# mp3guy/ElasticFusion

Measured on AMD Instinct MI355X. Metric: frames/s per GPU, 640x480 3-level ICP+fuse, higher is better.
Workload: dtype f32

## Files before the change

elasticfusion_amd/api.py:

```python
from __future__ import annotations

import ctypes as C
import os
import re

import numpy as np

_HERE = os.path.dirname(os.path.abspath(__file__))
LIB_PATH = os.environ.get("EF_HIP_LIB") or os.path.join(_HERE, "libefusion_hip.so")
_lib = None

c_f, c_i, c_u32, P = C.c_float, C.c_int, C.c_uint32, C.c_void_p


class EFError(RuntimeError):
    pass


class ef_config(C.Structure):
    _fields_ = [("width", c_i), ("height", c_i), ("fx", c_f), ("fy", c_f), ("cx", c_f), ("cy", c_f),
                ("time_delta", c_i), ("confidence", c_f), ("depth_cut", c_f), ("icp_weight", c_f),
                ("fast_odom", c_i), ("so3", c_i), ("frame_to_frame_rgb", c_i), ("pyramid", c_i), ("rgb_only", c_i),
                ("close_loops", c_i), ("max_surfels", c_u32), ("device", c_i), ("stream", P)]


class ef_intr(C.Structure):
    _fields_ = [("fx", c_f), ("fy", c_f), ("cx", c_f), ("cy", c_f)]


class ef_cam(C.Structure):
    _fields_ = [("cols", c_i), ("rows", c_i), ("fx", c_f), ("fy", c_f), ("cx", c_f), ("cy", c_f)]


class ef_gn_state(C.Structure):
    _fields_ = [("Rcurr", c_f * 9), ("tcurr", c_f * 3), ("resultRt", C.c_double * 16), ("krkinv", c_f * 9), ("kt", c_f * 3),
                ("lastRGBErrorLevel", c_f), ("rgb_broken", c_i)]


class ef_gn_update_args(C.Structure):
    _fields_ = [("sums", c_f * 58), ("prev", ef_gn_state), ("Rprev", c_f * 9), ("tprev", c_f * 3), ("count", c_i), ("sigma", c_i),
                ("icp", c_i), ("rgb", c_i), ("rgb_only", c_i), ("icp_weight", c_f), ("knext", ef_intr), ("level_changes", c_i),
                ("split_tail", c_i)]


class ef_model_maps_op(C.Structure):
    _fields_ = [("cols", c_i), ("rows", c_i), ("pred_vertex", P), ("pred_normal", P), ("fill_vertex", P), ("fill_normal", P), ("pred_image", P),
                ("fill_image", P), ("R", c_f * 9), ("t", c_f * 3), ("max_depth_rgb", c_f), ("camera_frame", c_i), ("force_fill_image", c_i),
                ("tally", c_i), ("dense_count", C.c_uint), ("dense_samples", c_i), ("vmap", P * 3), ("nmap", P * 3), ("depth0", P), ("last0", P),
                ("joint", c_i), ("raw", P), ("rgb3", P), ("depth_cut", c_f), ("filtered", P), ("metric", P), ("metric_filtered", P), ("next0", P)]


class ef_track_end_out(C.Structure):
    _fields_ = [("q", C.c_double * 4), ("t", C.c_double * 3), ("logged", C.c_double * 16), ("T_cw", c_f * 16), ("pose_f", c_f * 16),
                ("R_wc_f", c_f * 9), ("t_wc_f", c_f * 3), ("weighting", c_f)]


class ef_timing(C.Structure):
    _fields_ = [("name", C.c_char_p), ("ms", c_f)]


class ef_kernel_time(C.Structure):
    _fields_ = [("name", C.c_char_p), ("avg_us", c_f), ("launches", c_i), ("bytes_per_launch", C.c_double), ("bytes_per_launch_survey", C.c_double)]


class ef_tracker_plan(C.Structure):
    _fields_ = [("script", c_i), ("n_small", c_i), ("n_iter", c_i), ("levels", C.c_ulonglong), ("res_bytes", C.c_uint), ("res_budget", C.c_uint)]


class ef_render_params(C.Structure):
    _fields_ = [("width", c_i), ("height", c_i), ("fx", c_f), ("fy", c_f), ("cx", c_f), ("cy", c_f), ("T_wc", C.c_double * 16),
                ("max_depth", c_f), ("threshold", c_f), ("draw_unstable", c_i), ("color_type", c_i), ("draw_window", c_i),
                ("time", c_i), ("time_delta", c_i)]


class ef_register_params(C.Structure):
    _fields_ = [("max_dist", c_f), ("min_conf", c_f), ("min_normal_cos", c_f), ("max_iterations", c_i), ("min_pairs", c_i),
                ("stop_translation", C.c_double), ("stop_rotation", C.c_double)]


class ef_register_sums(C.Structure):
    _fields_ = [("A", C.c_double * 36), ("b", C.c_double * 6), ("e", C.c_double), ("pairs", c_u32), ("points", c_u32)]


class ef_register_result(C.Structure):
    _fields_ = [("status", c_i), ("iterations", c_i), ("pairs", c_u32), ("rms_first", C.c_double), ("rms_last", C.c_double),
                ("A", C.c_double * 36)]


class ef_map_selection(C.Structure):
    _fields_ = [("tests", c_u32), ("T_bw", C.c_double * 16), ("box_min", c_f * 3), ("box_max", c_f * 3), ("conf_min", c_f), ("conf_max", c_f),
                ("init_time_min", c_i), ("init_time_max", c_i), ("last_time_min", c_i), ("last_time_max", c_i), ("radius_min", c_f),
                ("radius_max", c_f), ("id_min", c_u32), ("id_max", c_u32), ("label_class", c_i), ("label_min_prob", c_f)]


class ef_insert_params(C.Structure):
    _fields_ = [("gate", c_i), ("min_separation", c_f), ("min_conf", c_f), ("min_normal_cos", c_f), ("init_time", c_i), ("last_time", c_i)]


class ef_insert_result(C.Structure):
    _fields_ = [("inserted", c_u32), ("duplicates", c_u32), ("skipped", c_u32), ("count_after", c_u32)]


class ef_fuse_params(C.Structure):
    _fields_ = [("min_separation", c_f), ("min_conf", c_f), ("min_normal_cos", c_f), ("append", c_i), ("init_time", c_i), ("last_time", c_i)]


class ef_fuse_result(C.Structure):
    _fields_ = [("fused", c_u32), ("absorbed", c_u32), ("weightless", c_u32), ("novel", c_u32), ("skipped", c_u32), ("inserted", c_u32),
                ("count_after", c_u32)]


class ef_thin_params(C.Structure):
    _fields_ = [("cell", c_f), ("keep", c_i)]


class ef_thin_result(C.Structure):
    _fields_ = [("participants", c_u32), ("cells", c_u32), ("removed", c_u32), ("count_after", c_u32)]


class ef_carve_params(C.Structure):
    _fields_ = [("width", c_i), ("height", c_i), ("fx", c_f), ("fy", c_f), ("cx", c_f), ("cy", c_f), ("min_depth", c_f), ("max_depth", c_f),
                ("margin", c_f), ("margin_quad", c_f), ("window", c_i), ("min_views", c_i), ("protect", c_i)]


class ef_carve_views(C.Structure):
    _fields_ = [("n", c_i), ("T_wc16", C.c_void_p), ("depth", C.c_void_p)]


class ef_carve_result(C.Structure):
    _fields_ = [("participants", c_u32), ("observed", c_u32), ("free_space", c_u32), ("protected_", c_u32), ("removed", c_u32),
                ("count_after", c_u32)]


class ef_outlier_params(C.Structure):
    _fields_ = [("mode", c_i), ("radius", c_f), ("cell", c_f), ("min_conf", c_f), ("min_neighbors", c_i), ("k", c_i), ("std_ratio", c_f),
                ("max_mean_dist", c_f), ("flag_sparse", c_i)]


class ef_outlier_result(C.Structure):
    _fields_ = [("sum", C.c_double), ("sum_sq", C.c_double), ("participants", c_u32), ("measured", c_u32), ("sparse", c_u32),
                ("outliers", c_u32), ("count_after", c_u32), ("threshold", c_f)]


class ef_component_params(C.Structure):
    _fields_ = [("radius", c_f), ("cell", c_f), ("min_conf", c_f), ("min_size", c_u32), ("max_size", c_u32)]


class ef_component_result(C.Structure):
    _fields_ = [("nodes", c_u32), ("components", c_u32), ("largest", c_u32), ("rejected_rows", c_u32), ("rejected_components", c_u32),
                ("count_after", c_u32), ("status", c_u32)]


CARVE_MAX_VIEWS = 32
COMPONENT_NONE = 0xFFFFFFFF
COMPONENTS_REJECTED, COMPONENTS_ACCEPTED = 0, 1
OUTLIER_RADIUS, OUTLIER_STATISTICAL = 0, 1
OUTLIER_SUM_LANES = 4096
THIN_KEEP_MAX_CONF, THIN_KEEP_NEWEST, THIN_KEEP_FIRST = 0, 1, 2
THIN_ROWS_REMOVED, THIN_ROWS_REPRESENTATIVES = 0, 1
INSERT_KEEP = -1
FUSE_SKIPPED, FUSE_NOVEL, FUSE_WEIGHTLESS, FUSE_ABSORBED, FUSE_FUSED, FUSE_INSERTED = 0, 1, 2, 3, 4, 5
ROW_NONE = 0xFFFFFFFF

SEL_BOX, SEL_CONF, SEL_INIT_TIME, SEL_LAST_TIME, SEL_RADIUS, SEL_ID, SEL_LABEL, SEL_INVERT = 0x01, 0x02, 0x04, 0x08, 0x10, 0x20, 0x40, 0x100

REG_CONVERGED, REG_MAX_ITERATIONS, REG_TOO_FEW_PAIRS, REG_DEGENERATE = 0, 1, 2, 3
REG_STATUS = {REG_CONVERGED: "CONVERGED", REG_MAX_ITERATIONS: "MAX_ITERATIONS", REG_TOO_FEW_PAIRS: "TOO_FEW_PAIRS", REG_DEGENERATE: "DEGENERATE"}


def _sums_dict(s: ef_register_sums) -> dict:
    return {"A": np.array(s.A, np.float64).reshape(6, 6), "b": np.array(s.b, np.float64), "e": float(s.e), "pairs": int(s.pairs),
            "points": int(s.points)}


def _sums_struct(sums) -> ef_register_sums:
    if isinstance(sums, ef_register_sums):
        return sums
    s = ef_register_sums()
    s.A[:] = np.ascontiguousarray(sums["A"], np.float64).reshape(36).tolist()
    s.b[:] = np.ascontiguousarray(sums["b"], np.float64).reshape(6).tolist()
    s.e = float(sums.get("e", 0.0))
    s.pairs = int(sums.get("pairs", 0))
    s.points = int(sums.get("points", 0))
    return s


def _pose16(T):
    if T is None:
        return None, None
    a = np.ascontiguousarray(T, np.float64).reshape(16)
    return a, _ptr(a)


def register_update(sums, T=None):
    s = _sums_struct(sums)
    keep, pT = _pose16(T)
    out = np.zeros(16, np.float64)
    xi = np.zeros(6, np.float64)
    rc = lib().ef_register_update(C.byref(s), pT, _ptr(out), _ptr(xi))
    if rc not in (0, REG_DEGENERATE):
        _chk(rc)
    return out.reshape(4, 4), xi, rc == REG_DEGENERATE
# ... 1189 lines not shown
        out = np.zeros((H, W, ch) if ch > 1 else (H, W), dt)
        _chk(lib().ef_get_image(self.h, which, _ptr(out), out.nbytes), self.h)
        return out

    def trackerBuffer(self, name: str, level: int = 0, tracker: int = 0) -> np.ndarray:
        which, dt, planes = self.TRACKER[name]
        w, h = self.cfg.width >> level, self.cfg.height >> level
        out = np.zeros((h * planes, w), dt)
        _chk(lib().ef_get_tracker_buffer_of(self.h, tracker, which, level, _ptr(out), out.nbytes), self.h)
        return out

    def enableTiming(self, on=True):
        _chk(lib().ef_enable_timing(self.h, int(on)), self.h)

    def timings(self) -> dict:
        arr = (ef_timing * 32)()
        n = c_i(0)
        _chk(lib().ef_get_timings(self.h, arr, 32, C.byref(n)), self.h)
        return {arr[i].name.decode(): arr[i].ms for i in range(n.value)}


class ops:
    @staticmethod
    def _f32(a):
        return np.ascontiguousarray(a, np.float32)

    @staticmethod
    def _image_op(name, src, dtype, scale, *scalars):
        h, w = src.shape[:2]
        shape = (h // scale, w // scale)
        s, d = DevBuf.from_array(src), DevBuf(shape[0] * shape[1] * np.dtype(dtype).itemsize)
        _chk(getattr(lib(), "ef_op_" + name)(s.p, w, h, *scalars, d.p, None))
        return d.to_array(dtype, shape)

    @staticmethod
    def pyr_down(src):
        return ops._image_op("pyr_down", src, np.uint16, 2)

    @staticmethod
    def create_vmap(depth, fx, fy, cx, cy, cutoff, init=None):
        h, w = depth.shape
        d = DevBuf.from_array(depth)
        v = DevBuf.from_array(np.zeros((3 * h, w), np.float32) if init is None else init)
        k = ef_intr(fx, fy, cx, cy)
        _chk(lib().ef_op_create_vmap(C.byref(k), d.p, w, h, cutoff, v.p, None))
        return v.to_array(np.float32, (3 * h, w))

    @staticmethod
    def create_nmap(vmap, init=None):
        h3, w = vmap.shape
        v = DevBuf.from_array(vmap)
        n = DevBuf.from_array(np.zeros((h3, w), np.float32) if init is None else init)
        _chk(lib().ef_op_create_nmap(v.p, w, h3 // 3, n.p, None))
        return n.to_array(np.float32, (h3, w))

    @staticmethod
    def transform_maps(vmap, nmap, R, t):
        h3, w = vmap.shape
        v, n = DevBuf.from_array(vmap), DevBuf.from_array(nmap)
        R9, t3 = ops._f32(R).reshape(9), ops._f32(t).reshape(3)
        _chk(lib().ef_op_transform_maps(v.p, n.p, w, h3 // 3, _ptr(R9), _ptr(t3), v.p, n.p, None))
        return v.to_array(np.float32, (h3, w)), n.to_array(np.float32, (h3, w))

    @staticmethod
    def copy_maps(vtex, ntex):
        h, w, _ = vtex.shape
        v4, n4 = DevBuf.from_array(ops._f32(vtex)), DevBuf.from_array(ops._f32(ntex))
        tmp, vm, nm = DevBuf(h * w * 16), DevBuf(h * w * 12), DevBuf(h * w * 12)
        _chk(lib().ef_op_copy_maps(v4.p, n4.p, w, h, tmp.p, vm.p, nm.p, None))
        return tmp.to_array(np.float32, (h, w, 4)), vm.to_array(np.float32, (3 * h, w)), nm.to_array(np.float32, (3 * h, w))

    @staticmethod
    def resize_map(src, normalize, init=None):
        h3, w = src.shape
        s = DevBuf.from_array(src)
        o = DevBuf.from_array(np.zeros((h3 // 2, w // 2), np.float32) if init is None else init)
        fn = lib().ef_op_resize_nmap if normalize else lib().ef_op_resize_vmap
        _chk(fn(s.p, w, h3 // 3, o.p, None))
        return o.to_array(np.float32, (h3 // 2, w // 2))

    @staticmethod
    def pyr_down_gauss_f(src):
        return ops._image_op("pyr_down_gauss_f", src, np.float32, 2)

    @staticmethod
    def pyr_down_uchar_gauss(src):
        return ops._image_op("pyr_down_uchar_gauss", src, np.uint8, 2)

    @staticmethod
    def vertices_to_depth(vmaps_tmp, cutoff):
        return ops._image_op("vertices_to_depth", ops._f32(vmaps_tmp), np.float32, 1, cutoff)

    @staticmethod
    def bgr_to_intensity(rgba):
        return ops._image_op("image_bgr_to_intensity", rgba, np.uint8, 1)

    @staticmethod
    def derivative_images(img):
        h, w = img.shape
        s, dx, dy = DevBuf.from_array(img), DevBuf(h * w * 2), DevBuf(h * w * 2)
        _chk(lib().ef_op_compute_derivative_images(s.p, w, h, dx.p, dy.p, None))
        return dx.to_array(np.int16, (h, w)), dy.to_array(np.int16, (h, w))

    @staticmethod
    def project_to_point_cloud(depth, fx, fy, cx, cy, level=0):
        h, w = depth.shape
        s, d = DevBuf.from_array(depth), DevBuf(h * w * 12)
        k = ef_intr(fx, fy, cx, cy)
        _chk(lib().ef_op_project_to_point_cloud(s.p, w, h, C.byref(k), level, d.p, None))
        return d.to_array(np.float32, (h, w, 3))

    @staticmethod
    def icp_step(Rcurr, tcurr, vmap_curr, nmap_curr, Rprev_inv, tprev, intr, vmap_g_prev, nmap_g_prev, distThres, angleThres):
        h3, w = vmap_curr.shape
        bufs = [DevBuf.from_array(a) for a in (vmap_curr, nmap_curr, vmap_g_prev, nmap_g_prev)]
        A, b, res = np.zeros((6, 6), np.float32), np.zeros(6, np.float32), np.zeros(2, np.float32)
        k = ef_intr(*intr)
        _chk(lib().ef_op_icp_step(_ptr(ops._f32(Rcurr).reshape(9)), _ptr(ops._f32(tcurr)), bufs[0].p, bufs[1].p,
                                  _ptr(ops._f32(Rprev_inv).reshape(9)), _ptr(ops._f32(tprev)), C.byref(k), bufs[2].p, bufs[3].p,
                                  distThres, angleThres, w, h3 // 3, _ptr(A), _ptr(b), _ptr(res), None))
        return A, b, res

    @staticmethod
    def rgb_residual(minScale, dIdx, dIdy, lastDepth, nextDepth, lastImage, nextImage, maxDepthDelta, kt, krkinv):
        h, w = nextImage.shape
        bufs = [DevBuf.from_array(a) for a in (dIdx, dIdy, lastDepth, nextDepth, lastImage, nextImage)]
        corres = DevBuf(h * w * 16)
        sigma, count = c_i(0), c_i(0)
        _chk(lib().ef_op_compute_rgb_residual(minScale, bufs[0].p, bufs[1].p, bufs[2].p, bufs[3].p, bufs[4].p, bufs[5].p, corres.p,
                                              maxDepthDelta, _ptr(ops._f32(kt)), _ptr(ops._f32(krkinv).reshape(9)), w, h,
                                              C.byref(sigma), C.byref(count), None))
        return corres.to_array(DATATERM, (h, w)), sigma.value, count.value

    @staticmethod
    def rgb_step(corres, sigma, cloud, fx, fy, dIdx, dIdy, sobelScale):
        h, w = corres.shape
        bufs = [DevBuf.from_array(a) for a in (corres, ops._f32(cloud), dIdx, dIdy)]
        A, b = np.zeros((6, 6), np.float32), np.zeros(6, np.float32)
        _chk(lib().ef_op_rgb_step(bufs[0].p, sigma, bufs[1].p, fx, fy, bufs[2].p, bufs[3].p, sobelScale, w, h,
                                  _ptr(A), _ptr(b), None))
        return A, b

    @staticmethod
    def so3_step(lastImage, nextImage, imageBasis, kinv, krlr):
        h, w = nextImage.shape
        li, ni = DevBuf.from_array(lastImage), DevBuf.from_array(nextImage)
        A, b, res = np.zeros((3, 3), np.float32), np.zeros(3, np.float32), np.zeros(2, np.float32)
        _chk(lib().ef_op_so3_step(li.p, ni.p, _ptr(ops._f32(imageBasis).reshape(9)), _ptr(ops._f32(kinv).reshape(9)),
                                  _ptr(ops._f32(krlr).reshape(9)), w, h, _ptr(A), _ptr(b), _ptr(res), None))
        return A, b, res

    @staticmethod
    def model_maps(pred_vertex, pred_normal, fill_vertex, fill_normal, R, t, maxDepthRGB=6.0, pred_image=None, fill_image=None, camera_frame=False,
                   force_fill_image=False, tally=False, dense_count=0, dense_samples=1, joint=False, raw=None, rgb=None, depth_cut=3.0, init=None):
        h, w, _ = pred_vertex.shape
        init = init or {}
        keep = [DevBuf.from_array(ops._f32(a)) for a in (pred_vertex, pred_normal, fill_vertex, fill_normal)]
        a = ef_model_maps_op()
        a.cols, a.rows = w, h
        a.pred_vertex, a.pred_normal, a.fill_vertex, a.fill_normal = (b.p for b in keep)
        if pred_image is not None:
            imgs = [DevBuf.from_array(np.ascontiguousarray(i, np.uint8)) for i in (pred_image, fill_image)]
            keep += imgs
            a.pred_image, a.fill_image = imgs[0].p, imgs[1].p
        a.R[:] = [float(v) for v in ops._f32(R).reshape(9)]
        a.t[:] = [float(v) for v in ops._f32(t).reshape(3)]
        a.max_depth_rgb = float(maxDepthRGB)
        a.camera_frame, a.force_fill_image, a.tally = int(camera_frame), int(force_fill_image), int(tally)
        a.dense_count, a.dense_samples = int(dense_count), int(dense_samples)
        spec = {}
        for l in range(3):
            spec[f"vmap{l}"] = spec[f"nmap{l}"] = (np.float32, (3 * (h >> l), w >> l))
        spec["depth0"], spec["last0"] = (np.float32, (h, w)), (np.uint8, (h, w))
        if joint:
            spec.update(filtered=(np.uint16, (h, w)), metric=(np.float32, (h, w)), metric_filtered=(np.float32, (h, w)), next0=(np.uint8, (h, w)))
        out = {}
        for name, (dt, shp) in spec.items():
            start = np.zeros(shp, dt) if name not in init else np.ascontiguousarray(init[name], dt)
            assert start.shape == shp, (name, start.shape, shp)
            out[name] = DevBuf.from_array(start)
        for l in range(3):
            a.vmap[l], a.nmap[l] = out[f"vmap{l}"].p, out[f"nmap{l}"].p
        a.depth0, a.last0 = out["depth0"].p, out["last0"].p
        if joint:
            fr = [DevBuf.from_array(np.ascontiguousarray(raw, np.uint16)), DevBuf.from_array(np.ascontiguousarray(rgb, np.uint8))]
            assert raw.shape == (h, w) and rgb.shape == (h, w, 3)
            keep += fr
            a.joint, a.raw, a.rgb3, a.depth_cut = 1, fr[0].p, fr[1].p, float(depth_cut)
            a.filtered, a.metric, a.metric_filtered, a.next0 = (out[n].p for n in ("filtered", "metric", "metric_filtered", "next0"))
        left = C.c_uint(0)
        _chk(lib().ef_op_model_maps(C.byref(a), C.byref(left), None))
        res = {name: out[name].to_array(*spec[name]) for name in spec}
        res["dense_count"] = int(left.value)
        return res

    @staticmethod
    def sobel_mask(nextImage, nextDepth):
        h, w = nextImage[0].shape
        img = [DevBuf.from_array(np.ascontiguousarray(a, np.uint8)) for a in nextImage]
        dep = [DevBuf.from_array(ops._f32(a)) for a in nextDepth]
        for l in range(3):
            assert nextImage[l].shape == nextDepth[l].shape == (h >> l, w >> l), (l, nextImage[l].shape, nextDepth[l].shape)
        outs = [[DevBuf((h >> l) * (w >> l) * sz, fill=0xA5) for l in range(3)] for sz in (2, 2, 1, 4)]
        arr = lambda bufs: (P * 3)(*[b.p for b in bufs])
        _chk(lib().ef_op_sobel_mask(arr(img), arr(dep), w, h, arr(outs[0]), arr(outs[1]), arr(outs[2]), arr(outs[3]), None))
        return tuple([b.to_array(dt, (h >> l, w >> l)) for l, b in enumerate(bufs)] for bufs, dt in zip(outs, (np.int16, np.int16, np.uint8, np.uint32)))

    @staticmethod
    def clean_deform(cam, T_wc, time, idx, vc, ct, nr, confThreshold, timeDelta, maxDepth, surfels, newUnstable, graph, depth, isFern=0):
        s = ops._f32(surfels).reshape(-1, 12)
        nu = ops._f32(newUnstable).reshape(-1, 12)
        g = ops._f32(graph).reshape(-1, 16)
        bufs = [DevBuf.from_array(a) for a in (idx, ops._f32(vc), ops._f32(ct), ops._f32(nr), g, ops._f32(depth))]
        sb, nb = DevBuf.from_array(s), DevBuf.from_array(nu if len(nu) else np.zeros((1, 12), np.float32))
        out = DevBuf((len(s) + len(nu) + 1) * 48)
        n = c_u32(0)
        _chk(lib().ef_op_clean_deform(C.byref(cam), _ptr(ops._T(T_wc)), time, bufs[0].p, bufs[1].p, bufs[2].p, bufs[3].p,
                                      confThreshold, timeDelta, maxDepth, sb.p, len(s), nb.p, len(nu),
                                      bufs[4].p, len(g), bufs[5].p, int(isFern), out.p, C.byref(n), None))
        return out.to_array(np.float32, (n.value, 12))

    LINALG = dict(ldlt6=0, ldlt3f=1, polar3=2, rodrigues=3, se3_inverse=4, se3_log_norm=5, scalar=6, ldlt6_wave=7, ldlt6_every_lane=8,
                  mat_to_quat=9, se3_mul=10, se3_castf=11, se3_inverse_f=12, m4_affine_inverse=13, ldlt_pivots=14, lu_inverse6=15)

    @staticmethod
    def linalg(which, vec, n_out):
        v = np.ascontiguousarray(np.asarray(vec, np.float64).reshape(-1))
        out = np.zeros(n_out, np.float64)
        _chk(lib().ef_op_linalg(ops.LINALG[which], _ptr(v), v.size, _ptr(out), n_out))
        return out

    GN_STATE = ("Rcurr", "tcurr", "resultRt", "krkinv", "kt", "lastRGBErrorLevel", "rgb_broken")

    @staticmethod
    def gn_update(sums, prev, Rprev, tprev, count, sigma, icp, rgb, rgbOnly, icpWeight, knext, level_changes, split_tail, lastA, lastb, stats):
        a = ef_gn_update_args()
        a.sums[:] = [float(v) for v in ops._f32(sums).reshape(58)]
        for name in ("Rcurr", "tcurr", "krkinv", "kt"):
            getattr(a.prev, name)[:] = [float(v) for v in ops._f32(prev[name]).reshape(-1)]
        a.prev.resultRt[:] = [float(v) for v in np.asarray(prev["resultRt"], np.float64).reshape(16)]
        a.prev.lastRGBErrorLevel, a.prev.rgb_broken = float(np.float32(prev["lastRGBErrorLevel"])), int(prev["rgb_broken"])
        a.Rprev[:] = [float(v) for v in ops._f32(Rprev).reshape(9)]
        a.tprev[:] = [float(v) for v in ops._f32(tprev).reshape(3)]
        a.count, a.sigma, a.icp, a.rgb, a.rgb_only = int(count), int(sigma), int(icp), int(rgb), int(rgbOnly)
        a.icp_weight, a.knext, a.level_changes, a.split_tail = float(icpWeight), ef_intr(*[float(v) for v in knext]), int(level_changes), int(split_tail)
        nxt = ef_gn_state()
        A = np.ascontiguousarray(np.asarray(lastA, np.float64).reshape(36)).copy()
        b = np.ascontiguousarray(np.asarray(lastb, np.float64).reshape(6)).copy()
        st = ops._f32(stats).reshape(4).copy()
        _chk(lib().ef_op_gn_update(C.byref(a), C.byref(nxt), _ptr(A), _ptr(b), _ptr(st)))
        out = {n: np.array(getattr(nxt, n)) for n in ("Rcurr", "tcurr", "resultRt", "krkinv", "kt")}
        out["lastRGBErrorLevel"], out["rgb_broken"] = np.float32(nxt.lastRGBErrorLevel), int(nxt.rgb_broken)
        return out, A, b, st

    @staticmethod
    def track_end_tail(Rcurr, tcurr, Rprev, tprev, q_prev, t_prev, rgb, weightMultiplier):
        o = ef_track_end_out()
        qp = np.ascontiguousarray(np.asarray(q_prev, np.float64).reshape(4))
        tp = np.ascontiguousarray(np.asarray(t_prev, np.float64).reshape(3))
        _chk(lib().ef_op_track_end_tail(_ptr(ops._f32(Rcurr).reshape(9)), _ptr(ops._f32(tcurr).reshape(3)), _ptr(ops._f32(Rprev).reshape(9)),
                                        _ptr(ops._f32(tprev).reshape(3)), _ptr(qp), _ptr(tp), int(rgb), weightMultiplier, C.byref(o)))
        out = {n: np.array(getattr(o, n)) for n in ("q", "t", "logged", "T_cw", "pose_f", "R_wc_f", "t_wc_f")}
        out["weighting"] = np.float32(o.weighting)
        return out

    @staticmethod
    def filter_depth(raw, maxD):
        return ops._image_op("filter_depth", raw, np.uint16, 1, maxD)

    @staticmethod
    def metricise_depth(d_in, maxD):
        return ops._image_op("metricise_depth", d_in, np.float32, 1, maxD)

    @staticmethod
    def seed_map(cam, rgb, dm, dmf, time, maxDepth):
        Pn = cam.cols * cam.rows
        bufs = [DevBuf.from_array(a) for a in (rgb, dm, dmf)]
        out = DevBuf(Pn * 48)
        n = c_u32(0)
        _chk(lib().ef_op_seed_map(C.byref(cam), bufs[0].p, bufs[1].p, bufs[2].p, time, maxDepth, out.p, C.byref(n), None))
        return out.to_array(np.float32, (n.value, 12))

    @staticmethod
    def _T(T):
        return np.ascontiguousarray(T, np.float64).reshape(16)

    @staticmethod
    def predict_indices(cam, T_wc, time, surfels, maxDepth, timeDelta):
        s = ops._f32(surfels).reshape(-1, 12)
        Pn = cam.cols * cam.rows
        sb = DevBuf.from_array(s)
        idx, vc, ct, nr = DevBuf(Pn * 4), DevBuf(Pn * 16), DevBuf(Pn * 16), DevBuf(Pn * 16)
        _chk(lib().ef_op_predict_indices(C.byref(cam), _ptr(ops._T(T_wc)), time, sb.p, len(s), maxDepth, timeDelta,
                                         idx.p, vc.p, ct.p, nr.p, None))
        shp = (cam.rows, cam.cols)
        return (idx.to_array(np.uint32, shp), vc.to_array(np.float32, shp + (4,)), ct.to_array(np.float32, shp + (4,)),
                nr.to_array(np.float32, shp + (4,)))

    @staticmethod
    def combined_predict(cam, T_wc, surfels, maxDepth, confThreshold, time, maxTime, timeDelta):
        s = ops._f32(surfels).reshape(-1, 12)
        Pn = cam.cols * cam.rows
        sb = DevBuf.from_array(s)
        img, vt, nm, tm = DevBuf(Pn * 4), DevBuf(Pn * 16), DevBuf(Pn * 16), DevBuf(Pn * 2)
        _chk(lib().ef_op_combined_predict(C.byref(cam), _ptr(ops._T(T_wc)), sb.p, len(s), maxDepth, confThreshold,
                                          time, maxTime, timeDelta, img.p, vt.p, nm.p, tm.p, None))
        shp = (cam.rows, cam.cols)
        return (img.to_array(np.uint8, shp + (4,)), vt.to_array(np.float32, shp + (4,)), nm.to_array(np.float32, shp + (4,)),
                tm.to_array(np.uint16, shp))

    @staticmethod
    def synthesize_depth(cam, T_wc, surfels, maxDepth, confThreshold, time, maxTime, timeDelta):
        s = ops._f32(surfels).reshape(-1, 12)
        Pn = cam.cols * cam.rows
        sb, d = DevBuf.from_array(s), DevBuf(Pn * 4)
        _chk(lib().ef_op_synthesize_depth(C.byref(cam), _ptr(ops._T(T_wc)), sb.p, len(s), maxDepth, confThreshold,
                                          time, maxTime, timeDelta, d.p, None))
        return d.to_array(np.float32, (cam.rows, cam.cols))

    @staticmethod
    def fill_in(cam, image, vertex, normal, depthFiltered, rgb, passthrough=0, passthroughImage=0):
        bufs = [DevBuf.from_array(a) for a in (image, ops._f32(vertex), ops._f32(normal), depthFiltered, rgb)]
        Pn = cam.cols * cam.rows
        fi, fv, fn = DevBuf(Pn * 4), DevBuf(Pn * 16), DevBuf(Pn * 16)
        _chk(lib().ef_op_fill_in(C.byref(cam), bufs[0].p, bufs[1].p, bufs[2].p, bufs[3].p, bufs[4].p, passthrough, passthroughImage,
                                 fi.p, fv.p, fn.p, None))
        shp = (cam.rows, cam.cols)
        return fi.to_array(np.uint8, shp + (4,)), fv.to_array(np.float32, shp + (4,)), fn.to_array(np.float32, shp + (4,))

    @staticmethod
    def dense_enough(cam, image):
        b = DevBuf.from_array(image)
        d = c_i(0)
        _chk(lib().ef_op_dense_enough(C.byref(cam), b.p, C.byref(d), None))
        return bool(d.value)

    @staticmethod
    def fuse(cam, T_wc, time, rgb, dm, dmf, idx, vc, ct, nr, maxDepth, weighting, surfels):
        s = ops._f32(surfels).reshape(-1, 12)
        bufs = [DevBuf.from_array(a) for a in (rgb, dm, dmf, idx, ops._f32(vc), ops._f32(ct), ops._f32(nr))]
        sb = DevBuf.from_array(s)
        nu = DevBuf((cam.cols // 2) * (cam.rows // 2) * 48)
# ... 17 lines not shown
```

elasticfusion_amd/csrc/ef_context.hip:

```cpp
#include <hip/hip_runtime.h>
#include <math.h>
#include <cmath>
#include <stdio.h>
#include <string.h>
#include <limits>
#include <string>
#include <thread>
#include <vector>

#include "../../include/ef_hip.h"
#include "ef_linalg_dev.hpp"
#include "ef_solve_dev.hpp"
#include "ef_map.hpp"
#include "ef_deform_solver.hpp"
#include "ef_track.hpp"

template void std::vector<int64_t>::push_back(const int64_t&);

namespace {

thread_local std::string g_create_error;

struct StageTimer {
  const char* name;
  hipEvent_t a, b;
  bool used;
};

struct DevBuf {
  uint8_t* p = nullptr;
  size_t bytes = 0;
  int reserve(ef_ctx* c, size_t need, const char* what, bool* grew = nullptr);
  void release() {
    if (p) (void)hipFree(p);
    p = nullptr;
    bytes = 0;
  }
  template <class T>
  T* as() const { return (T*)p; }
};
struct Carver {
  uint8_t* at;
  explicit Carver(const DevBuf& b) : at(b.p) {}
  template <class T>
  T* take(size_t count, size_t align = alignof(T)) {
    at = (uint8_t*)(((uintptr_t)at + align - 1) & ~(uintptr_t)(align - 1));
    T* r = (T*)at;
    at += count * sizeof(T);
    return r;
  }
  static size_t chunks(size_t rows) { return (size_t)efm::select_chunks((unsigned)rows) + 1; }
  static size_t scan_bytes(size_t rows) { return (2 * chunks(rows) + 4) * sizeof(uint32_t); }
  uint32_t* scan_words(size_t rows, efm::SelectScratch* sc, size_t align = alignof(uint32_t)) {
    const size_t k = chunks(rows);
    sc->chunk_count = take<uint32_t>(k, align);
    sc->chunk_offset = take<uint32_t>(k);
    return take<uint32_t>(4);
  }
};

struct FrameImages {
  uint8_t* rgb = nullptr;
  uint16_t *depth_raw = nullptr, *depth_filtered = nullptr;
  float *depth_metric = nullptr, *depth_metric_filtered = nullptr;
};
struct RingSlot {
  uint8_t *h_rgb = nullptr, *d_rgb = nullptr;
  uint16_t *h_depth = nullptr, *d_depth = nullptr;
  hipEvent_t ev_h2d = nullptr;
};
struct KernelSampler {
  std::vector<hipEvent_t> start, stop;
  eft::KernelProbe probe{nullptr, nullptr, 0, 0};
  int create(ef_ctx* c, int capacity);
  int average_us(ef_ctx* c, float* us) const;
  void release() {
    for (auto e : start) (void)hipEventDestroy(e);
    for (auto e : stop) (void)hipEventDestroy(e);
    *this = KernelSampler{};
  }
};

}

struct ef_ctx {
  ef_config cfg;
  hipStream_t stream = nullptr;
  bool own_stream = false;
  std::string err;
  efm::Cam cam;
  eft::Intr intr;
  const float maxDepthProcessed = 20.0f;
  FrameImages img, img_alt;
  hipStream_t in_stream = nullptr;
  hipEvent_t ev_input_done = nullptr, ev_track_done = nullptr;
  hipEvent_t ev_frame_done[2] = {nullptr, nullptr};
  int frame_parity = 0;
  int overlap_mode = 1;
  bool overlap = false;
  bool events_live = false;
  static constexpr int RING = 3;
  RingSlot ring[RING];
  hipStream_t copy_stream = nullptr;
  unsigned host_seq = 0;
  unsigned mark_value = 0;
  unsigned* h_consumed = nullptr;
  unsigned* d_consumed = nullptr;
  unsigned* h_abort = nullptr;
  unsigned* d_abort = nullptr;
  eft::Pyramid pyr{};
  eft::TrackState* st = nullptr;
  efm::IndexMaps im{};
  efm::PredictMaps pm{};
  efm::FillMaps fm{};
  unsigned long long* zbuf = nullptr;
  unsigned long long* zbuf_assoc = nullptr;
  unsigned long long* zbuf_clean = nullptr;
  float* im_T16 = nullptr;
  bool im_pending = false;
  int im_map = 0;
  efm::SurfelSoA maps[2]{};
  int cur = 0;
  efm::SurfelSoA shadow{};
  bool reference_download = false;
  uint32_t capacity = 0;
  uint32_t* winner = nullptr;
  efm::Candidates cand{};
  efm::CompactScratch cs{};
  int* overflow = nullptr;
  double* traj = nullptr;
  int traj_cap = 0;
  std::vector<int64_t> stamps;
  int tick = 1;
  std::vector<void*> allocs;
  bool tally_by_consumer = false;
  bool tally_pending = false;
  bool timing = false;
  std::vector<StageTimer> timers;
  float* graph_dev = nullptr;
  int graph_nodes = 0, graph_is_fern = 0;
  float* synth_depth = nullptr;
  float* rays = nullptr;
  int icp_count_thresh = 35000;
  float icp_err_thresh = 5e-05f, cov_thresh = 1e-05f;
  int deforms = 0;
  const float* bil_table = nullptr;
  eft::Pyramid pyr2{};
  eft::TrackState* st2 = nullptr;
  efm::PredictMaps old{};
  float* cons_dev = nullptr;
  float* h_cons = nullptr;
  eft::TrackState* h_states = nullptr;
  ef_loop_solver solver = nullptr;
  void* solver_user = nullptr;
  bool builtin_solver = false;
  int64_t last_deform_time = 0;
  float* nodes_dev = nullptr;
  std::vector<float> h_nodes;
  ef_local_loop loop{};
  std::vector<double> loop_constraints;
  std::vector<float> loop_graph;
  ef_closure* closure = nullptr;
  ef_global_loop gloop{};
  std::string fern_tracker_error;
  int fern_w = 0, fern_h = 0;
  uchar4* view_img_dev = nullptr;
  float4* view_vert_dev = nullptr;
  float4* view_norm_dev = nullptr;
  uint8_t* h_view = nullptr;
  eft::Pyramid pyr3{};
  eft::TrackState* st3 = nullptr;
  eft::Intr intr3{};
  float4* fern_maps_dev = nullptr;
  float* h_nodes_pinned = nullptr;
  int* fern_table_dev = nullptr;
  int fern_num = 0, fern_table_version = -1;
  uint8_t* fern_codes_dev = nullptr;
  uint8_t* h_codes = nullptr;
  uint8_t* h_codes_end = nullptr;
  uint8_t* h_view_end = nullptr;
  hipEvent_t ev_end_record = nullptr;
  bool end_pending = false, end_lost = false;
  int end_tick = 0;
  int n_nodes_host = 0;
  double h_pose[16] = {1, 0, 0, 0, 0, 1, 0, 0, 0, 0, 1, 0, 0, 0, 0, 1};
  bool reloc = false, lost = false, last_frame_recovery = false, tracking_ok = true;
  int tracking_count = 0;
  eft::TrackState h_reloc{};
  bool use_graph = false;
  bool track_only = false;
  bool no_resident = false;
  bool fused_step = false;
  int persistent = 1;
  struct TrackGraph { hipGraphExec_t exec = nullptr; const void* key = nullptr; eft::TrackParams tp{}; eft::TrackTail tail{}; eft::TrackerPlan plan{}; };
  TrackGraph tgraph[2];
  int ktime_every = 0;
  KernelSampler sample_step, sample_splat, sample_all;
  hipStream_t debug_stream = nullptr;
  DevBuf stage;
  struct RenderState { DevBuf zbuf; } render;
  struct LabelState {
    bool ids_on = false, ids_bad = false;
    unsigned* ids_state = nullptr;
    int C = 0, cur = 0;
    float* tab[2] = {};
    uint32_t* ids[2] = {};
    size_t rows = 0, bound = 0;
    size_t known = 0, known_frames = 0, ev_frames = 0;
    unsigned* count_h = nullptr;
    hipEvent_t ev = nullptr;
    bool ev_pending = false;
    DevBuf index;
  } labels;
  uint64_t map_gen = 1;
  struct QueryState {
    uint64_t gen = 0;
    float cell = EF_QUERY_DEFAULT_CELL, built_cell = 0.f;
    int lanes = 0;
    DevBuf sorted, rows;
    DevBuf cells;
    uint32_t nb = 0, n = 0;
  } query;
  struct RegisterState {
    DevBuf slabs;
    double* sums_h = nullptr;
  } reg;
  struct SelectState {
    DevBuf scratch;
    size_t rows = 0;
    uint64_t gen = 0;
    uint32_t count = 0;
  } sel;
  struct InsertState {
    DevBuf scratch;
    size_t rows = 0;
  } ins;
  struct ThinState {
    DevBuf scratch;
    size_t rows = 0;
  } thin;
  struct CarveState {
    DevBuf scratch;
    size_t rows = 0;
  } carve;
  struct OutlierState {
    DevBuf scratch;
    size_t rows = 0;
  } outlier;
  struct ComponentState {
    DevBuf scratch;
    size_t rows = 0;
  } components;
  struct FuseState {
    DevBuf scratch;
  } fuse;
};

namespace {

#define EF_HIP(ctx, expr)                                                                       \
  do {                                                                                          \
    hipError_t _e = (expr);                                                                     \
    if (_e != hipSuccess) {                                                                     \
      (ctx)->err = std::string(#expr) + ": " + hipGetErrorString(_e);                           \
      return EF_EHIP;                                                                           \
    }                                                                                           \
  } while (0)
// ... 788 lines not shown
```

elasticfusion_amd/csrc/ef_device.hpp:

```cpp
#pragma once
#include <hip/hip_runtime.h>
#include <stdint.h>
#include "ef_build.hpp"

#ifdef EF_NO_FMA
#define EF_FMA(a, b, c) ((a) * (b) + (c))
#else
#define EF_FMA(a, b, c) fmaf((a), (b), (c))
#endif

namespace ef {

struct f3 { float x, y, z; };

__device__ __forceinline__ float qnan() { return __int_as_float(0x7fffffff); }
__device__ __forceinline__ f3 operator-(f3 a, f3 b) { return {a.x - b.x, a.y - b.y, a.z - b.z}; }
__device__ __forceinline__ f3 operator+(f3 a, f3 b) { return {a.x + b.x, a.y + b.y, a.z + b.z}; }
__device__ __forceinline__ float dot(f3 a, f3 b) { return EF_FMA(a.z, b.z, EF_FMA(a.y, b.y, a.x * b.x)); }
__device__ __forceinline__ f3 cross(f3 a, f3 b) {
  return {EF_FMA(a.y, b.z, -(a.z * b.y)), EF_FMA(a.z, b.x, -(a.x * b.z)), EF_FMA(a.x, b.y, -(a.y * b.x))};
}
__device__ __forceinline__ float norm(f3 a) { return sqrtf(dot(a, a)); }
__device__ __forceinline__ f3 normalized(f3 a) {
  const float rn = 1.0f / sqrtf(dot(a, a));
  return {a.x * rn, a.y * rn, a.z * rn};
}
__device__ __forceinline__ uint8_t intensity_of(float c0, float c1, float c2) {
  const int value = (int)(c0 * 0.114f + c1 * 0.299f + c2 * 0.587f);
  return (uint8_t)value;
}
struct m33 { f3 r[3]; };
__device__ __forceinline__ f3 mul(const m33& m, f3 a) { return {dot(m.r[0], a), dot(m.r[1], a), dot(m.r[2], a)}; }
__device__ __forceinline__ m33 m33_load(const float* p) {
  return m33{{{p[0], p[1], p[2]}, {p[3], p[4], p[5]}, {p[6], p[7], p[8]}}};
}
struct rt34 { m33 R; f3 t; };
__device__ __forceinline__ rt34 rt34_load16(const float* M) {
  return rt34{{{{M[0], M[1], M[2]}, {M[4], M[5], M[6]}, {M[8], M[9], M[10]}}}, {M[3], M[7], M[11]}};
}
__device__ __forceinline__ f3 xform(const rt34& T, f3 p) { return mul(T.R, p) + T.t; }

__device__ __forceinline__ int f2i_rn(float x) {
  float r = (x != x) ? 0.0f : rintf(x);
  r = fminf(fmaxf(r, -2147483648.0f), 2147483520.0f);
  return (int)r;
}

__host__ __device__ inline float ef_next_up(float a) { unsigned u; __builtin_memcpy(&u, &a, 4); ++u; __builtin_memcpy(&a, &u, 4); return a; }
__host__ __device__ inline float ef_next_down(float a) { unsigned u; __builtin_memcpy(&u, &a, 4); --u; __builtin_memcpy(&a, &u, 4); return a; }
__host__ __device__ inline float sq_le_max(float T) {
  if (!(T >= 0.0f)) return -1.0f;
  if (T > 3.4028234664e38f) return T;
  float a = T * T;
  if (a > 3.4028234664e38f) a = 3.4028234664e38f;
  for (int i = 0; i < 8 && a > 0.0f && !(__builtin_sqrtf(a) <= T); ++i) a = ef_next_down(a);
  for (int i = 0; i < 8 && a < 3.4028234664e38f && __builtin_sqrtf(ef_next_up(a)) <= T; ++i) a = ef_next_up(a);
  return a;
}
__host__ __device__ inline float sq_lt_max(float T) {
  if (!(T > 0.0f)) return -1.0f;
  float a = T > 3.4028234664e38f ? 3.4028234664e38f : T * T;
  if (a > 3.4028234664e38f) a = 3.4028234664e38f;
  for (int i = 0; i < 8 && a > 0.0f && !(__builtin_sqrtf(a) < T); ++i) a = ef_next_down(a);
  for (int i = 0; i < 8 && a < 3.4028234664e38f && __builtin_sqrtf(ef_next_up(a)) < T; ++i) a = ef_next_up(a);
  return a;
}

__device__ __forceinline__ float ef_expf(float x) {
  if (x < -87.0f) return 0.0f;
  const float n = rintf(x * 1.44269504088896341f);
  float r = fmaf(n, -0.693359375f, x);
  r = fmaf(n, 2.12194440e-4f, r);
  float p = 1.9875691500e-4f;
  p = fmaf(p, r, 1.3981999507e-3f);
  p = fmaf(p, r, 8.3334519073e-3f);
  p = fmaf(p, r, 4.1665795894e-2f);
  p = fmaf(p, r, 1.6666665459e-1f);
  p = fmaf(p, r, 5.0000001201e-1f);
  const float e = fmaf(p, r * r, r) + 1.0f;
  return ldexpf(e, (int)n);
}

__device__ __forceinline__ int clampi(int v, int lo, int hi) { return v < lo ? lo : (v > hi ? hi : v); }

struct DataTerm {
  short zero_x, zero_y;
  short one_x, one_y;
  float diff;
  unsigned char valid;
  unsigned char pad[3];
};
static_assert(sizeof(DataTerm) == 16, "DataTerm must be 16 bytes");

template <int K, int BLOCK>
__device__ __forceinline__ void block_reduce_store(const float (&acc)[K], float* lds, float* out) {
  static_assert(K <= 32 && BLOCK % 64 == 0, "shape");
  constexpr int STR = BLOCK + 1;
  constexpr int SEG = BLOCK / 32;
  const int t = threadIdx.x;
#pragma unroll
  for (int k = 0; k < K; ++k) lds[k * STR + t] = acc[k];
  __syncthreads();
  const int v = t & 31, g = t >> 5;
  float s = 0.f;
  if (v < K) {
    const float* row = lds + v * STR + g * 32;
#pragma unroll
    for (int i = 0; i < 32; ++i) s += row[i];
  }
  __syncthreads();
  lds[g * 32 + v] = s;
  __syncthreads();
  if (t < K) {
    float r = 0.f;
#pragma unroll
    for (int gg = 0; gg < SEG; ++gg) r += lds[gg * 32 + t];
    out[t] = r;
  }
}
template <int K, int BLOCK>
constexpr int block_reduce_lds_floats() { return K * (BLOCK + 1); }

template <int BLOCK>
__device__ __forceinline__ void block_reduce_atomic_int2(int a, int b, int* lds, int* out2) {
  const int t = threadIdx.x;
  for (int off = 32; off > 0; off >>= 1) {
    a += __shfl_down(a, off, 64);
    b += __shfl_down(b, off, 64);
  }
  if ((t & 63) == 0) { lds[(t >> 6) * 2] = a; lds[(t >> 6) * 2 + 1] = b; }
  __syncthreads();
  if (t == 0) {
    int sa = 0, sb = 0;
    for (int w = 0; w < BLOCK / 64; ++w) { sa += lds[w * 2]; sb += lds[w * 2 + 1]; }
    if (sa) atomicAdd(out2, sa);
    if (sb) atomicAdd(out2 + 1, sb);
  }
}

}
```

elasticfusion_amd/csrc/ef_host_frame.inc:

```
namespace {
int do_predict(ef_ctx* c, bool count_dense = true) {
  efm::combined_predict(c->cam, c->st->T_cw, c->maps[c->cur], &c->st->map_counts[c->cur], c->maxDepthProcessed, c->cfg.confidence,
                        c->last_frame_recovery ? 0 : c->tick, c->tick, c->cfg.time_delta, c->zbuf, c->pm, c->fm, c->img.depth_filtered, c->img.rgb,
                        c->cfg.frame_to_frame_rgb != 0, (count_dense && !c->tally_by_consumer) ? &c->st->dense_count : nullptr, c->stream, nullptr, 0u,
                        (count_dense && c->mark_value) ? c->d_consumed : nullptr, c->mark_value, c->rays);
  if (count_dense) c->mark_value = 0;
  if (count_dense && c->tally_by_consumer) c->tally_pending = true;
  if (c->lost) efm::fill_in(c->cam, c->pm, c->img.depth_filtered, c->img.rgb, true, true, c->fm, c->stream);
  return EF_OK;
}
bool reloc_covariance_ok(const eft::TrackState& h) {
  double cov[36];
  efl::lu_inverse<double, 6>(h.lastA, cov);
  for (int i = 0; i < 6; ++i)
    if (cov[i * 6 + i] > 1e-04) return false;
  return true;
}
struct FramePlan {
  const ef_ctx* c; hipMemcpyKind kind; bool pose_given;
  bool overlap = c->overlap && !c->timing && c->in_stream != nullptr;
  hipStream_t sb = overlap ? c->in_stream : c->stream;
  bool want_events = c->overlap && c->in_stream != nullptr;
  int overlap_mode = (c->overlap_mode == 2 && c->persistent == 1 && !c->use_graph) ? 1 : c->overlap_mode;
  bool frame_done_event = want_events && c->overlap_mode == 2;
  bool track_this = c->tick > 1 && !pose_given;
  bool fold_copies = kind == hipMemcpyDeviceToDevice && track_this;
  bool joint_inputs = track_this && !overlap && !c->timing;
  bool sample = c->ktime_every > 0 && (c->tick % c->ktime_every) == 0;
  bool replay = c->use_graph && !sample && !c->timing;
#ifdef EF_KEEP_INDEX_RESOLVE
  bool keyed = false;
#else
  bool keyed = !c->timing && !c->reference_download && !c->cfg.close_loops;
#endif
  bool defer_merge = !c->timing;
};
int input_stage(ef_ctx* c, const FramePlan& f, const uint8_t* rgb_src, const uint16_t* depth_src, hipEvent_t images_ready, eft::FramePreprocess* fp) {
  const int W = c->cam.cols, H = c->cam.rows;
  hipStream_t sb = f.sb;
  if (f.overlap && !c->events_live) EF_HIP(c, hipStreamSynchronize(c->stream));
  std::swap(c->img, c->img_alt);
  c->frame_parity ^= 1;
  if (f.overlap) EF_HIP(c, hipStreamWaitEvent(sb, f.overlap_mode == 2 ? c->ev_frame_done[c->frame_parity] : c->ev_track_done, 0));
  if (images_ready) EF_HIP(c, hipStreamWaitEvent(sb, images_ready, 0));
  if (!f.fold_copies) {
    EF_HIP(c, hipMemcpyAsync(c->img.rgb, rgb_src, (size_t)W * H * 3, f.kind, sb));
    EF_HIP(c, hipMemcpyAsync(c->img.depth_raw, depth_src, (size_t)W * H * 2, f.kind, sb));
  }
  *fp = eft::FramePreprocess{f.fold_copies ? depth_src : c->img.depth_raw, c->cfg.depth_cut, c->bil_table, c->img.depth_filtered, c->img.depth_metric,
                             c->img.depth_metric_filtered, f.fold_copies ? rgb_src : c->img.rgb, f.fold_copies ? c->img.rgb : nullptr};
  timer_begin(c, "Preprocess");
  if (!f.joint_inputs && !efm::preprocess_depth(fp->raw, W, H, fp->maxD, fp->filtered, fp->metric, fp->metric_filtered, sb, 0u,
                                                f.track_this ? fp->rgb3 : nullptr, c->pyr.nextImage[0], fp->rgb_keep, fp->table)) {
    c->err = "bilateral weight table missing on this device";
    return EF_EHIP;
  }
  timer_end(c, "Preprocess");
  if (f.overlap && f.overlap_mode == 2) EF_HIP(c, hipStreamWaitEvent(sb, c->ev_track_done, 0));
  if (f.track_this && f.overlap)
    eft::build_pyramids_frame_side(c->pyr, c->img.depth_filtered, c->intr, c->maxDepthProcessed, sb);
  if (f.overlap) EF_HIP(c, hipEventRecord(c->ev_input_done, sb));
  return EF_OK;
}
int first_frame(ef_ctx* c, const FramePlan& f, int log_slot) {
  hipStream_t s = c->stream;
  if (f.overlap) EF_HIP(c, hipStreamWaitEvent(s, c->ev_input_done, 0));
  timer_begin(c, "feedbackBuffers");
  efm::seed_map(c->cam, c->img.rgb, c->img.depth_metric, c->img.depth_metric_filtered, c->tick, c->maxDepthProcessed, c->maps[c->cur],
                &c->st->map_counts[c->cur], c->cs, s);
  eft::init_first_rgb(c->pyr, c->img.rgb, s);
  if (log_slot >= 0) eft::log_pose(c->st, c->traj, log_slot, s);
  if (f.want_events) EF_HIP(c, hipEventRecord(c->ev_track_done, s));
  timer_end(c, "feedbackBuffers");
  return EF_OK;
}
int track_replayed(ef_ctx* c, const eft::TrackParams& tp, eft::TrackTail* tail) {
  hipStream_t s = c->stream;
  const void* key = c->pyr.nextImage[0];
  ef_ctx::TrackGraph* g = nullptr;
  for (auto& cand : c->tgraph)
    if (cand.exec && cand.key == key && !memcmp(&cand.tp, &tp, sizeof(tp))) g = &cand;
  if (!g) {
    g = (c->tgraph[0].exec && c->tgraph[0].key != key) ? &c->tgraph[1] : &c->tgraph[0];
    if (g->exec) { (void)hipGraphExecDestroy(g->exec); g->exec = nullptr; }
    eft::track_prepare(c->pyr, tp, s);
    eft::Pyramid pyr_copy = c->pyr;
    hipGraph_t graph = nullptr;
    EF_HIP(c, hipStreamBeginCapture(s, hipStreamCaptureModeThreadLocal));
    g->tail = eft::track(pyr_copy, c->st, c->intr, tp, s, nullptr);
    g->plan = pyr_copy.plan;
    hipError_t ce = hipStreamEndCapture(s, &graph);
    if (ce == hipSuccess) ce = hipGraphInstantiate(&g->exec, graph, nullptr, nullptr, 0);
    if (graph) (void)hipGraphDestroy(graph);
    if (ce != hipSuccess) {
      g->exec = nullptr;
      c->err = std::string("hipGraph capture of the tracker: ") + hipGetErrorString(ce);
      return EF_EHIP;
    }
    g->key = key;
    memcpy(&g->tp, &tp, sizeof(tp));
  }
  EF_HIP(c, hipGraphLaunch(g->exec, s));
  eft::track_swap(c->pyr, tp);
  c->pyr.plan = g->plan;
  *tail = g->tail;
  return EF_OK;
}
int track_frame(ef_ctx* c, const FramePlan& f, const eft::FramePreprocess& fp, float weightMultiplier, int log_slot) {
  hipStream_t s = c->stream;
  eft::TrackParams tp = track_params(c);
  tp.rgbOnly = c->cfg.rgb_only != 0; tp.pyramid = c->cfg.pyramid != 0; tp.fastOdom = c->cfg.fast_odom != 0; tp.so3 = c->cfg.so3 != 0;
  tp.icpWeight = c->cfg.icp_weight;
  const bool rgb = tp.rgbOnly || tp.icpWeight < 100;
  timer_begin(c, "odomInit");
  eft::init_icp_model(c->pyr, (const float*)c->pm.vertex, (const float*)c->pm.normal, (const float*)c->fm.vertex,
                      (const float*)c->fm.normal, c->st, 6.0f , s, (const uint8_t*)c->pm.image,
                      (const uint8_t*)c->fm.image, c->cfg.frame_to_frame_rgb != 0, f.joint_inputs ? &fp : nullptr, c->tally_pending);
  c->tally_pending = false;
  if (f.overlap) {
    eft::build_pyramids_model_side(c->pyr, s);
    EF_HIP(c, hipStreamWaitEvent(s, c->ev_input_done, 0));
  } else {
    eft::build_pyramids(c->pyr, c->img.depth_filtered, c->intr, c->maxDepthProcessed, s, rgb);
  }
  if (rgb && f.overlap) eft::init_rgb_sobel(c->pyr, s);
  timer_end(c, "odomInit");
  timer_begin(c, "odom");
  eft::TrackTail tail{};
  if (f.replay) {
    tp.persistent = 0;
    EF_TRY(track_replayed(c, tp, &tail));
  } else {
    tail = eft::track(c->pyr, c->st, c->intr, tp, s, f.sample ? &c->sample_step.probe : nullptr,
                      f.sample && c->sample_all.probe.start ? &c->sample_all.probe : nullptr);
  }
  eft::track_end(c->st, tail, rgb, weightMultiplier, log_slot >= 0 ? c->traj : nullptr, log_slot, s, eft::tracker_abort_word(c->pyr), c->d_abort);
  timer_end(c, "odom");
  return EF_OK;
}
int reloc_verdict(ef_ctx* c) {
  c->tracking_ok = true;
  if (!c->reloc) return EF_OK;
  EF_TRY(read_state(c, c->st, &c->h_reloc));
  c->tracking_ok = c->h_reloc.lastICPError < 1e-04;
  if (!c->lost) {
    if (!reloc_covariance_ok(c->h_reloc)) c->tracking_ok = false;
    if (!c->tracking_ok) {
      if (++c->tracking_count > 10) c->lost = true;
    } else {
      c->tracking_count = 0;
    }
  } else if (c->last_frame_recovery) {
    if (!reloc_covariance_ok(c->h_reloc)) c->tracking_ok = false;
    if (c->tracking_ok) {
      c->lost = false;
      c->tracking_count = 0;
    }
    c->last_frame_recovery = false;
  }
  return EF_OK;
}
int close_loops(ef_ctx* c, int log_slot) {
  int fern_graph = 0;
  if (c->closure) {
    timer_begin(c, "globalLoop");
    do_predict(c, false);
    c->last_frame_recovery = false;
    const int r = global_loop_closure(c, log_slot, &fern_graph);
    timer_end(c, "globalLoop");
    if (r != EF_OK) return r;
  }
  if (c->lost || fern_graph) {
    memset(&c->loop, 0, sizeof(c->loop));
    return EF_OK;
  }
  timer_begin(c, "localLoop");
  const int r = local_loop_closure(c, log_slot, c->closure != nullptr);
  timer_end(c, "localLoop");
  return r;
  return EF_OK;
}
void fuse_frame(ef_ctx* c, const FramePlan& f) {
  hipStream_t s = c->stream;
  const bool keyed = f.keyed, sample_splat = f.sample && c->sample_splat.probe.start;
  timer_begin(c, "indexMap");
  efm::IndexMaps im_assoc = c->im;
  im_assoc.color_time = nullptr;
  const efm::KeyedIndex key_assoc{c->zbuf_assoc, c->st->T_cw, c->maps[c->cur]}, key_clean{c->zbuf_clean, c->st->T_cw, c->maps[c->cur]};
  efm::predict_indices(c->cam, c->st->T_cw, c->tick, c->maps[c->cur], &c->st->map_counts[c->cur], c->maxDepthProcessed, c->cfg.time_delta,
                       keyed ? c->zbuf_assoc : c->zbuf, im_assoc, s, sample_splat ? &c->sample_splat.probe : nullptr, nullptr, nullptr, !keyed);
  timer_end(c, "indexMap");
  timer_begin(c, "Fuse::Data+Update");
  efm::fuse(c->cam, c->st->pose_f, c->tick, c->img.rgb, c->img.depth_metric, c->img.depth_metric_filtered, c->im, c->maxDepthProcessed,
            &c->st->weighting, c->maps[c->cur], &c->st->map_counts[c->cur], c->cand, c->winner, s, f.defer_merge,
            keyed ? &key_assoc : nullptr, keyed ? c->zbuf_clean : nullptr);
  if (c->reference_download && !f.defer_merge) efm::copy_map(c->maps[c->cur], &c->st->map_counts[c->cur], c->shadow, s);
  timer_end(c, "Fuse::Data+Update");
  timer_begin(c, "indexMap2");
  efm::predict_indices(c->cam, c->st->T_cw, c->tick, c->maps[c->cur], &c->st->map_counts[c->cur], c->maxDepthProcessed, c->cfg.time_delta,
                       keyed ? c->zbuf_clean : c->zbuf, c->im, s, nullptr, f.defer_merge ? &c->cand : nullptr, c->winner, !keyed);
  c->im_pending = keyed;
  c->im_map = c->cur;
  if (c->reference_download && f.defer_merge) efm::copy_map(c->maps[c->cur], &c->st->map_counts[c->cur], c->shadow, s);
  timer_end(c, "indexMap2");
  efm::Deformation def{c->graph_dev, c->graph_nodes, c->synth_depth, c->graph_is_fern, c->maxDepthProcessed};
  if (c->graph_nodes > 0 && !c->graph_is_fern)
    efm::synthesize_depth(c->cam, c->st->T_cw, c->maps[c->cur], &c->st->map_counts[c->cur], c->maxDepthProcessed, c->cfg.confidence, c->tick,
                          c->tick - c->cfg.time_delta, 65535, c->zbuf, c->synth_depth, s, c->rays);
  timer_begin(c, "Fuse::Copy");
  efm::clean(c->cam, c->st->T_cw, c->tick, c->im, c->cfg.confidence, c->cfg.time_delta, c->maps[c->cur], &c->st->map_counts[c->cur], c->cand,
             c->winner, c->maps[c->cur ^ 1], &c->st->map_counts[c->cur ^ 1], c->capacity, c->cs, c->overflow, s,
             c->graph_nodes > 0 ? &def : nullptr, keyed ? &key_clean : nullptr, keyed ? c->zbuf_assoc : nullptr, keyed ? c->im_T16 : nullptr);
  c->cur ^= 1;
  timer_end(c, "Fuse::Copy");
}
int end_of_frame(ef_ctx* c, const FramePlan& f) {
  timer_begin(c, "IndexMap::ACTIVE");
  do_predict(c);
  timer_end(c, "IndexMap::ACTIVE");
  if (c->closure) {
    timer_begin(c, "ferns");
    int r = flush_end_record(c);
    if (r == EF_OK) r = enqueue_end_record(c);
    timer_end(c, "ferns");
    if (r != EF_OK) return r;
  }
  if (f.frame_done_event) EF_HIP(c, hipEventRecord(c->ev_frame_done[c->frame_parity], c->stream));
  c->events_live = f.want_events;
  if (!c->lost) c->tick++;
  EF_HIP(c, hipGetLastError());
  return EF_OK;
}
int process_frame(ef_ctx* c, const uint8_t* rgb_src, const uint16_t* depth_src, hipMemcpyKind kind, int64_t timestamp,
                  float weightMultiplier, const double* in_T_wc, hipEvent_t images_ready = nullptr) {
  ++c->map_gen;
  if ((c->h_abort && (c->h_abort[0] | c->h_abort[1] | c->h_abort[2])) || c->pyr.sticky_abort || c->pyr2.sticky_abort || c->pyr3.sticky_abort) {
    c->err = "a persistent tracker launch of an earlier frame timed out waiting for another workgroup after its whole grid had reported in (a protocol "
             "failure, not a busy chip: that case runs on one workgroup, ef_get_tracker_fallbacks): the poses and the map since then are invalid; "
             "recreate the context (ef_set_persistent_tracker(ctx, 0) selects the launch-per-step script)";
    return EF_EHIP;
  }
  const FramePlan f{c, kind, in_T_wc != nullptr};
  eft::FramePreprocess fp;
  EF_TRY(input_stage(c, f, rgb_src, depth_src, images_ready, &fp));
  if ((int)c->stamps.size() >= c->traj_cap) EF_TRY(grow_trajectory(c));
  const int log_slot = (int)c->stamps.size();
  c->stamps.push_back(timestamp);
  if (c->tick == 1) {
    EF_TRY(first_frame(c, f, log_slot));
  } else {
    if (!in_T_wc) {
      EF_TRY(track_frame(c, f, fp, weightMultiplier, log_slot));
      EF_TRY(reloc_verdict(c));
    } else {
      c->tracking_ok = true;
      if (f.overlap) EF_HIP(c, hipStreamWaitEvent(c->stream, c->ev_input_done, 0));
      eft::pose_injected(c->st, in_T_wc, true, weightMultiplier, true, log_slot >= 0 ? c->traj : nullptr, log_slot, c->stream);
    }
    if (f.want_events) EF_HIP(c, hipEventRecord(c->ev_track_done, c->stream));
    if (c->cfg.close_loops) EF_TRY(close_loops(c, log_slot));
    if (!c->cfg.rgb_only && c->tracking_ok && !c->lost && !c->track_only) fuse_frame(c, f);
    c->graph_nodes = 0;
  }
  return end_of_frame(c, f);
}
}

extern "C" {

int ef_process_frame(ef_ctx* c, const uint8_t* rgb, const uint16_t* depth, int64_t timestamp, float wm, const double* T) {
  if (!c || !rgb || !depth) return EF_EINVAL;
  DeviceGuard dg_(c);
  const size_t P = (size_t)c->cam.cols * c->cam.rows;
  const RingSlot& slot = c->ring[c->host_seq % ef_ctx::RING];
  if (c->host_seq >= (unsigned)ef_ctx::RING) {
    const unsigned need = c->host_seq - ef_ctx::RING + 1u;
    volatile unsigned* seen = c->h_consumed;
    int spins = 0;
    while ((int)(*seen - need) < 0) {
      if (++spins > 20000) {
        EF_HIP(c, hipStreamSynchronize(c->stream));
        break;
      }
      if (spins > 64) std::this_thread::yield();
    }
  }
  memcpy(slot.h_rgb, rgb, P * 3);
  memcpy(slot.h_depth, depth, P * 2);
  EF_HIP(c, hipMemcpyAsync(slot.d_depth, slot.h_depth, P * 2, hipMemcpyHostToDevice, c->copy_stream));
  EF_HIP(c, hipMemcpyAsync(slot.d_rgb, slot.h_rgb, P * 3, hipMemcpyHostToDevice, c->copy_stream));
  EF_HIP(c, hipEventRecord(slot.ev_h2d, c->copy_stream));
  c->mark_value = c->host_seq + 1u;
  c->host_seq++;
  return process_frame(c, slot.d_rgb, slot.d_depth, hipMemcpyDeviceToDevice, timestamp, wm, T, slot.ev_h2d);
}
int ef_process_frame_dev(ef_ctx* c, const uint8_t* rgb_dev, const uint16_t* depth_dev, int64_t timestamp, float wm, const double* T) {
  if (!c || !rgb_dev || !depth_dev) return EF_EINVAL;
  DeviceGuard dg_(c);
  return process_frame(c, rgb_dev, depth_dev, hipMemcpyDeviceToDevice, timestamp, wm, T);
}
int ef_predict(ef_ctx* c) {
  if (!c) return EF_EINVAL;
  DeviceGuard dg_(c);
  EF_HIP(c, hipMemsetAsync(&c->st->dense_count, 0, sizeof(unsigned), c->stream));
  return do_predict(c);
}

}
```

elasticfusion_amd/csrc/ef_host_inspect.inc:

```
namespace {
struct ImageRef { const void* src; int elem; bool resizable; };
ImageRef image_ref(const ef_ctx* c, int which) {
  switch (which) {
    case EF_IMG_DEPTH_FILTERED: return {c->img.depth_filtered, 2, false};
    case EF_IMG_DEPTH_METRIC: return {c->img.depth_metric, 4, false};
    case EF_IMG_DEPTH_METRIC_FILTERED: return {c->img.depth_metric_filtered, 4, false};
    case EF_IMG_PREDICT_IMAGE: return {c->pm.image, 4, true};
    case EF_IMG_PREDICT_VERTEX: return {c->pm.vertex, 16, true};
    case EF_IMG_PREDICT_NORMAL: return {c->pm.normal, 16, true};
    case EF_IMG_PREDICT_TIME: return {c->pm.time, 2, true};
    case EF_IMG_FILL_IMAGE: return {c->fm.image, 4, true};
    case EF_IMG_FILL_VERTEX: return {c->fm.vertex, 16, true};
    case EF_IMG_FILL_NORMAL: return {c->fm.normal, 16, true};
    case EF_IMG_INDEX: return {c->im.index, 4, false};
    case EF_IMG_VERT_CONF: return {c->im.vert_conf, 16, false};
    case EF_IMG_COLOR_TIME: return {c->im.color_time, 16, false};
    case EF_IMG_NORM_RAD: return {c->im.norm_rad, 16, false};
    case EF_IMG_OLD_IMAGE: return {c->old.image, 4, true};
    case EF_IMG_OLD_VERTEX: return {c->old.vertex, 16, true};
    case EF_IMG_OLD_NORMAL: return {c->old.normal, 16, true};
    case EF_IMG_OLD_TIME: return {c->old.time, 2, true};
    default: return {nullptr, 0, false};
  }
}
// ... 89 lines not shown
      }
    }
  }
  if (stamps) for (int i = 0; i < n; ++i) stamps[i] = c->stamps[i];
  *n_frames = n;
  return EF_OK;
}
int ef_get_pose_qt(ef_ctx* c, double* q4_t3) {
  if (!c || !q4_t3) return EF_EINVAL;
  DeviceGuard dg_(c);
  eft::TrackState h;
  EF_TRY(read_state(c, c->st, &h));
  for (int i = 0; i < 4; ++i) q4_t3[i] = h.q[i];
  for (int i = 0; i < 3; ++i) q4_t3[4 + i] = h.t[i];
  return EF_OK;
}
int ef_get_relocalisation(ef_ctx* c, ef_reloc_state* out) {
  if (!c || !out) return EF_EINVAL;
  out->lost = c->lost; out->tracking_ok = c->tracking_ok; out->tracking_count = c->tracking_count; out->last_frame_recovery = c->last_frame_recovery;
  return EF_OK;
}
int ef_get_global_loop(ef_ctx* c, ef_global_loop* info) {
  if (!c || !info) return EF_EINVAL;
  *info = c->gloop;
  return EF_OK;
}
ef_closure* ef_get_closure(ef_ctx* c) {
  if (!c) return nullptr;
  DeviceGuard dg_(c);
  (void)flush_end_record(c);
  return c->closure;
}
int ef_get_local_loop(ef_ctx* c, ef_local_loop* info, double* constraints, int max_constraints, int* n_out) {
  if (!c || !info) return EF_EINVAL;
  *info = c->loop;
  int n = c->loop.n_constraints < max_constraints ? c->loop.n_constraints : max_constraints;
  if (!constraints) n = 0;
  if (n > 0) memcpy(constraints, c->loop_constraints.data(), (size_t)n * 8 * sizeof(double));
  if (n_out) *n_out = n;
  return EF_OK;
}
int ef_sample_graph(ef_ctx* c, float* nodes4, int max_nodes, int* n_out) {
  if (!c || !nodes4 || !n_out || max_nodes <= 0) return EF_EINVAL;
  DeviceGuard dg_(c);
  float* dev = nullptr;
  EF_HIP(c, hipMalloc((void**)&dev, ((size_t)max_nodes * 4 + 4) * sizeof(float)));
  unsigned* n_dev = (unsigned*)(dev + (size_t)max_nodes * 4);
  efm::sample_graph(c->maps[c->cur], &c->st->map_counts[c->cur], 5000, max_nodes, dev, n_dev, c->stream);
  unsigned n = 0;
  hipError_t e = hipMemcpyAsync(&n, n_dev, sizeof(n), hipMemcpyDeviceToHost, c->stream);
  if (e == hipSuccess) e = hipStreamSynchronize(c->stream);
  if (e == hipSuccess && n > 0) e = hipMemcpy(nodes4, dev, (size_t)n * 4 * sizeof(float), hipMemcpyDeviceToHost);
  (void)hipFree(dev);
  EF_HIP(c, e);
  *n_out = (int)n;
  return EF_OK;
}
int ef_map_count(ef_ctx* c, uint32_t* count) {
  if (!c || !count) return EF_EINVAL;
  DeviceGuard dg_(c);
  return read_count(c, count);
}
int ef_map_download(ef_ctx* c, float* surfels, uint32_t max_surfels, uint32_t* count) {
  if (!c || !count) return EF_EINVAL;
  DeviceGuard dg_(c);
  if (c->labels.ids_on) {
    const int ri = ids_prepare(c, "ef_map_download");
    if (ri != EF_OK) return ri;
  }
  uint32_t n = 0;
  int r = ef_map_count(c, &n);
  if (r != EF_OK) return r;
  if (n > max_surfels) n = max_surfels;
  *count = n;
  if (!surfels || !n) return EF_OK;
  float* tmp = nullptr;
  EF_HIP(c, hipMalloc((void**)&tmp, (size_t)n * 48));
  efm::soa_to_aos(c->reference_download ? c->shadow : c->maps[c->cur], n, tmp, c->stream);
  hipError_t e = hipMemcpyAsync(surfels, tmp, (size_t)n * 48, hipMemcpyDeviceToHost, c->stream);
  if (e == hipSuccess) e = hipStreamSynchronize(c->stream);
  (void)hipFree(tmp);
  EF_HIP(c, e);
  return EF_OK;
}
int ef_write_freiburg(const char* path, const double* T_wc16_array, const int64_t* timestamps, int n) {
  if (!path || (n > 0 && (!T_wc16_array || !timestamps))) return EF_EINVAL;
  FILE* f = fopen(path, "w");
  if (!f) return EF_EINVAL;
  for (int i = 0; i < n; ++i) {
    const efl::SE3 S = efl::se3_from_matrix(T_wc16_array + (size_t)i * 16);
    fprintf(f, "%.6f %g %g %g %g %g %g %g\n", (double)timestamps[i] / 1000000.0, S.t[0], S.t[1], S.t[2], S.q[0], S.q[1], S.q[2], S.q[3]);
  }
  fclose(f);
  return EF_OK;
}
int ef_write_ply(const char* path, const float* surfels, uint32_t count, float confidence_threshold) {
  if (!path || (count > 0 && !surfels)) return EF_EINVAL;
  uint32_t valid = 0;
  for (uint32_t i = 0; i < count; ++i) valid += surfels[(size_t)i * 12 + 3] > confidence_threshold;
  FILE* f = fopen(path, "wb");
  if (!f) return EF_EINVAL;
  fprintf(f, "ply\nformat binary_little_endian 1.0\nelement vertex %u\nproperty float x\nproperty float y\nproperty float z\n"
             "property uchar red\nproperty uchar green\nproperty uchar blue\nproperty float nx\nproperty float ny\nproperty float nz\n"
             "property float radius\nend_header\n", valid);
  for (uint32_t i = 0; i < count; ++i) {
    const float* s = surfels + (size_t)i * 12;
    if (!(s[3] > confidence_threshold)) continue;
    const int col = (int)s[4];
    const unsigned char rgbc[3] = {(unsigned char)((col >> 16) & 0xFF), (unsigned char)((col >> 8) & 0xFF), (unsigned char)(col & 0xFF)};
    const float nr[4] = {s[8] * -1, s[9] * -1, s[10] * -1, s[11]};
    fwrite(s, sizeof(float), 3, f);
    fwrite(rgbc, 1, 3, f);
    fwrite(nr, sizeof(float), 4, f);
  }
  fclose(f);
  return EF_OK;
}
int ef_save_freiburg(ef_ctx* c, const char* path) {
  if (!c || !path) return EF_EINVAL;
  DeviceGuard dg_(c);
  const int n = (int)c->stamps.size();
  std::vector<double> T((size_t)n * 16);
  int got = 0;
  int r = ef_get_trajectory(c, T.data(), nullptr, n, &got);
  if (r != EF_OK) return r;
  r = ef_write_freiburg(path, T.data(), c->stamps.data(), got);
  if (r != EF_OK) c->err = std::string("cannot open ") + path;
  return r;
}
int ef_save_ply(ef_ctx* c, const char* path) {
  if (!c || !path) return EF_EINVAL;
  DeviceGuard dg_(c);
  uint32_t n = 0;
  int r = ef_map_count(c, &n);
  if (r != EF_OK) return r;
  std::vector<float> m((size_t)n * 12);
  r = ef_map_download(c, m.data(), n, &n);
  if (r != EF_OK) return r;
  r = ef_write_ply(path, m.data(), n, c->cfg.confidence);
  if (r != EF_OK) c->err = std::string("cannot open ") + path;
  return r;
}

static void im_materialise(ef_ctx* c) {
  if (!c->im_pending) return;
  efm::resolve_indices(c->cam, c->im_T16, c->maps[c->im_map], c->zbuf_clean, c->im, c->stream);
  c->im_pending = false;
}
int ef_get_image(ef_ctx* c, int which, void* dst, size_t bytes) {
  if (!c || !dst) return EF_EINVAL;
  DeviceGuard dg_(c);
  const size_t P = (size_t)c->cam.cols * c->cam.rows;
  if (which >= EF_IMG_INDEX && which <= EF_IMG_NORM_RAD) im_materialise(c);
  const ImageRef im = image_ref(c, which);
  if (!im.elem) { c->err = "ef_get_image: unknown image"; return EF_EINVAL; }
  const void* src = im.src;
  const size_t need = P * (size_t)im.elem;
  if (!src) { c->err = "ef_get_image: this image only exists in a close_loops context"; return EF_ESTATE; }
  if (bytes < need) { c->err = "ef_get_image: destination too small"; return EF_EINVAL; }
  void* tmp = nullptr;
  if (c->im.colmajor && which >= EF_IMG_INDEX && which <= EF_IMG_NORM_RAD) {
    EF_HIP(c, hipMalloc(&tmp, need));
    const int W = c->cam.cols, H = c->cam.rows;
    const dim3 g((unsigned)((P + 255) / 256));
    if (which == EF_IMG_INDEX) hipLaunchKernelGGL(k_to_rowmajor<uint32_t>, g, dim3(256), 0, c->stream, (const uint32_t*)src, W, H, (uint32_t*)tmp);
    else hipLaunchKernelGGL(k_to_rowmajor<float4>, g, dim3(256), 0, c->stream, (const float4*)src, W, H, (float4*)tmp);
    src = tmp;
  }
  hipError_t e = hipMemcpyAsync(dst, src, need, hipMemcpyDeviceToHost, c->stream);
  if (e == hipSuccess) e = hipStreamSynchronize(c->stream);
  if (tmp) (void)hipFree(tmp);
  EF_HIP(c, e);
  return EF_OK;
}
int ef_get_image_resized(ef_ctx* c, int which, int factor, void* dst, size_t bytes) {
  if (!c || !dst || factor < 1) return EF_EINVAL;
  DeviceGuard dg_(c);
  const int W = c->cam.cols, H = c->cam.rows, dw = W / factor, dh = H / factor;
  const ImageRef im = image_ref(c, which);
  if (!im.resizable) { c->err = "ef_get_image_resized: a predicted, fill-in or inactive-prediction image"; return EF_EINVAL; }
  const void* src = im.src;
  const int elem = im.elem;
  if (!src) { c->err = "ef_get_image_resized: this image only exists in a close_loops context"; return EF_ESTATE; }
  const size_t need = (size_t)dw * dh * elem;
  if (dw == 0 || dh == 0 || bytes < need) { c->err = "ef_get_image_resized: destination too small"; return EF_EINVAL; }
  void* tmp = nullptr;
  EF_HIP(c, hipMalloc(&tmp, need));
  const dim3 g((unsigned)((dw * dh + 255) / 256));
  if (elem == 16) hipLaunchKernelGGL(k_resize_nearest<float4>, g, dim3(256), 0, c->stream, (const float4*)src, W, dw, dh, factor, (float4*)tmp);
  else if (elem == 4) hipLaunchKernelGGL(k_resize_nearest<uint32_t>, g, dim3(256), 0, c->stream, (const uint32_t*)src, W, dw, dh, factor, (uint32_t*)tmp);
  else hipLaunchKernelGGL(k_resize_nearest<uint16_t>, g, dim3(256), 0, c->stream, (const uint16_t*)src, W, dw, dh, factor, (uint16_t*)tmp);
  hipError_t e = hipMemcpyAsync(dst, tmp, need, hipMemcpyDeviceToHost, c->stream);
  if (e == hipSuccess) e = hipStreamSynchronize(c->stream);
  (void)hipFree(tmp);
  EF_HIP(c, e);
  return EF_OK;
}
int ef_get_tracker_buffer(ef_ctx* c, int which, int level, void* dst, size_t bytes) { return ef_get_tracker_buffer_of(c, 0, which, level, dst, bytes); }
int ef_get_tracker_buffer_of(ef_ctx* c, int tracker, int which, int level, void* dst, size_t bytes) {
  if (!c || !dst || level < 0 || level >= eft::NUM_PYRS || tracker < 0 || tracker > 1) return EF_EINVAL;
  DeviceGuard dg_(c);
  const size_t n = (size_t)(c->cam.cols >> level) * (c->cam.rows >> level);
  const void* src = nullptr;
  size_t need = 0;
  const eft::Pyramid& p = tracker == 0 ? c->pyr : c->pyr2;
  if (!p.partials) { c->err = "ef_get_tracker_buffer_of: the model-to-model tracker only exists in a close_loops context"; return EF_ESTATE; }
  switch (which) {
    case 0: src = p.vmap_curr[level]; need = n * 12; break;
    case 1: src = p.nmap_curr[level]; need = n * 12; break;
    case 2: src = p.vmap_g_prev[level]; need = n * 12; break;
    case 3: src = p.nmap_g_prev[level]; need = n * 12; break;
    case 4: src = p.lastDepth[level]; need = n * 4; break;
    case 5: src = p.nextDepth[level]; need = n * 4; break;
    case 6: src = p.lastImage[level]; need = n; break;
    case 7: src = p.nextImage[level]; need = n; break;
    case 8: src = p.lastNextImage[level]; need = n; break;
    case 9: src = p.dIdx[level]; need = n * 2; break;
    case 10: src = p.dIdy[level]; need = n * 2; break;
    case 11: src = (level == 0 && tracker == 0) ? c->img.depth_filtered : p.depth_tmp[level]; need = n * 2; break;
    case 12: src = p.rgbMask[level]; need = n; break;
    case 13: src = p.corres[level]; need = n * 4; break;
    default: c->err = "ef_get_tracker_buffer: unknown buffer"; return EF_EINVAL;
  }
  if (bytes < need) { c->err = "ef_get_tracker_buffer: destination too small"; return EF_EINVAL; }
  EF_HIP(c, hipMemcpyAsync(dst, src, need, hipMemcpyDeviceToHost, c->stream));
  EF_HIP(c, hipStreamSynchronize(c->stream));
  return EF_OK;
}

int ef_enable_timing(ef_ctx* c, int on) { if (!c) return EF_EINVAL; c->timing = on != 0; return EF_OK; }
int ef_get_timings(ef_ctx* c, ef_timing* out, int max, int* n) {
  if (!c || !n) return EF_EINVAL;
  DeviceGuard dg_(c);
  EF_HIP(c, hipStreamSynchronize(c->stream));
  int k = 0;
  for (auto& t : c->timers) {
    if (!t.used || k >= max) continue;
    float ms = 0.f;
    if (hipEventElapsedTime(&ms, t.a, t.b) != hipSuccess) ms = -1.f;
    if (out) { out[k].name = t.name; out[k].ms = ms; }
    ++k;
  }
  *n = k;
  return EF_OK;
}

int ef_kernel_timing(ef_ctx* c, int every_n_frames) {
  if (!c || every_n_frames < 0) return EF_EINVAL;
  DeviceGuard dg_(c);
  EF_HIP(c, hipStreamSynchronize(c->stream));
  c->ktime_every = every_n_frames;
  KernelSampler* const all[3] = {&c->sample_all, &c->sample_splat, &c->sample_step};
  const int capacity[3] = {1024, 1024, 4096};
  for (int i = 0; i < 3; ++i) {
    all[i]->probe.used = 0;
    if (every_n_frames > 0) EF_TRY(all[i]->create(c, capacity[i]));
  }
  return EF_OK;
}
int ef_get_kernel_timing(ef_ctx* c, ef_kernel_time* out) {
  if (!c || !out) return EF_EINVAL;
  DeviceGuard dg_(c);
  EF_TRY(c->sample_step.average_us(c, &out->avg_us));
  const bool icp = !c->cfg.rgb_only && c->cfg.icp_weight > 0, rgb = c->cfg.rgb_only || c->cfg.icp_weight < 100;
#ifdef EF_FAST_ORDER
  out->name = "k_se3_accum_fast (level 0 of the launch-per-step script: icpStep + rgbStep Jacobian rows + fast-order sums)";
#else
  out->name = "k_se3_accum (level 0: icpStep + rgbStep Jacobian rows + reference-order sums)";
#endif
  out->launches = c->sample_step.probe.used;
  out->bytes_per_launch = (double)c->cam.cols * c->cam.rows * ((icp ? 48.0 : 0.0) + (rgb ? 4.0 : 0.0));
  out->bytes_per_launch_survey = (double)c->cam.cols * c->cam.rows * (icp ? 48.0 : 0.0);
  return EF_OK;
}

int ef_get_tracker_timing(ef_ctx* c, ef_kernel_time* out) {
  if (!c || !out) return EF_EINVAL;
  DeviceGuard dg_(c);
  EF_TRY(c->sample_all.average_us(c, &out->avg_us));
  const bool icp = !c->cfg.rgb_only && c->cfg.icp_weight > 0, rgb = c->cfg.rgb_only || c->cfg.icp_weight < 100;
#ifdef EF_FAST_ORDER
  out->name = "k_track_fast (the whole tracker as one persistent launch: SO(3) loop + every ICP+RGB iteration of every level + the update steps)";
#else
  out->name = "k_track_ref (the whole tracker as one persistent launch, reference summation order: SO(3) loop + every ICP+RGB iteration of every level + the update steps)";
#endif
  out->launches = c->sample_all.probe.used;
  const int its[3] = {c->cfg.fast_odom ? 3 : 10, c->cfg.pyramid ? 5 : 0, c->cfg.pyramid ? 4 : 0};
  double visits = 0;
  for (int l = 0; l < 3; ++l) visits += (double)its[l] * (double)(c->cam.cols >> l) * (double)(c->cam.rows >> l);
  out->bytes_per_launch = visits * ((icp ? 48.0 : 0.0) + (rgb ? 4.0 : 0.0));
  out->bytes_per_launch_survey = visits * (icp ? 48.0 : 0.0);
  return EF_OK;
}

int ef_get_splat_timing(ef_ctx* c, ef_kernel_time* out) {
  if (!c || !out) return EF_EINVAL;
  DeviceGuard dg_(c);
  EF_TRY(c->sample_splat.average_us(c, &out->avg_us));
  unsigned count = 0;
  EF_HIP(c, hipMemcpy(&count, &c->st->map_counts[c->cur], sizeof(count), hipMemcpyDeviceToHost));
  out->name = "k_index_splat (IndexMap::predictIndices: per-surfel transform + project + 64-bit atomicMin z-buffer)";
  out->launches = c->sample_splat.probe.used;
  out->bytes_per_launch = 40.0 * (double)count;
  out->bytes_per_launch_survey = 48.0 * (double)count;
  return EF_OK;
}
// ... 3 lines not shown
```

elasticfusion_amd/csrc/ef_host_ops.inc:

```
extern "C" {

__global__ void k_calib_empty() {}
__global__ void __launch_bounds__(256) k_calib_stream(const float4* __restrict__ src, float4* __restrict__ dst, int n) {
  for (int i = blockIdx.x * blockDim.x + threadIdx.x; i < n; i += gridDim.x * blockDim.x) dst[i] = src[i];
}
int ef_dev_calibrate(void* stream, float* empty_us, float* stream16mb_us) {
  if (!empty_us || !stream16mb_us) return EF_EINVAL;
  hipStream_t s = (hipStream_t)stream;
  const int n = 1 << 20, reps = 200;
  float4 *a = nullptr, *b = nullptr;
  hipEvent_t e0 = nullptr, e1 = nullptr;
  int rc = EF_EHIP;
  float ms = 0;
  if (hipMalloc((void**)&a, (size_t)n * sizeof(float4)) != hipSuccess || hipMalloc((void**)&b, (size_t)n * sizeof(float4)) != hipSuccess) { rc = EF_ENOMEM; goto done; }
  if (hipMemsetAsync(a, 0, (size_t)n * sizeof(float4), s) != hipSuccess) goto done;
  if (hipEventCreate(&e0) != hipSuccess || hipEventCreate(&e1) != hipSuccess) goto done;
  for (int pass = 0; pass < 2; ++pass) {
    if (hipEventRecord(e0, s) != hipSuccess) goto done;
    for (int i = 0; i < reps; ++i) hipLaunchKernelGGL(k_calib_empty, dim3(256), dim3(256), 0, s);
    if (hipEventRecord(e1, s) != hipSuccess || hipEventSynchronize(e1) != hipSuccess || hipEventElapsedTime(&ms, e0, e1) != hipSuccess) goto done;
    *empty_us = 1e3f * ms / reps;
    if (hipEventRecord(e0, s) != hipSuccess) goto done;
    for (int i = 0; i < reps; ++i) hipLaunchKernelGGL(k_calib_stream, dim3(2048), dim3(256), 0, s, (const float4*)a, b, n);
    if (hipEventRecord(e1, s) != hipSuccess || hipEventSynchronize(e1) != hipSuccess || hipEventElapsedTime(&ms, e0, e1) != hipSuccess) goto done;
// ... 23 lines not shown
    if (_e != hipSuccess) { g_create_error = hipGetErrorString(_e); return EF_EHIP; } \
    return EF_OK;                                                          \
  } while (0)
#define OP_SYNC(s)                                                         \
  do {                                                                     \
    hipError_t _e = hipStreamSynchronize((hipStream_t)(s));                \
    if (_e == hipSuccess) _e = hipGetLastError();                          \
    if (_e != hipSuccess) { g_create_error = hipGetErrorString(_e); return EF_EHIP; } \
  } while (0)

int ef_op_pyr_down(const uint16_t* src, int sc, int sr, uint16_t* dst, void* s) { eft::pyr_down_u16(src, sc, sr, dst, (hipStream_t)s); OP_TAIL(s); }
int ef_op_create_vmap(const ef_intr* k, const uint16_t* depth, int cols, int rows, float cutoff, float* vmap, void* s) {
  eft::create_vmap(depth, cols, rows, eft::Intr{k->fx, k->fy, k->cx, k->cy}, cutoff, vmap, (hipStream_t)s);
  OP_TAIL(s);
}
int ef_op_create_nmap(const float* vmap, int cols, int rows, float* nmap, void* s) { eft::create_nmap(vmap, cols, rows, nmap, (hipStream_t)s); OP_TAIL(s); }
int ef_op_transform_maps(const float* vs, const float* ns, int cols, int rows, const float* R9, const float* t3, float* vd, float* nd, void* s) {
  float* rt = nullptr;
  if (hipMalloc((void**)&rt, 12 * sizeof(float)) != hipSuccess) return EF_ENOMEM;
  float h[12];
  memcpy(h, R9, 36);
  memcpy(h + 9, t3, 12);
  (void)hipMemcpyAsync(rt, h, sizeof(h), hipMemcpyHostToDevice, (hipStream_t)s);
  eft::transform_maps(vs, ns, cols, rows, rt, rt + 9, vd, nd, (hipStream_t)s);
  (void)hipStreamSynchronize((hipStream_t)s);
  (void)hipFree(rt);
  OP_TAIL(s);
}
int ef_op_copy_maps(const float* v4, const float* n4, int cols, int rows, float* tmp, float* vd, float* nd, void* s) {
  eft::copy_maps(v4, n4, cols, rows, tmp, vd, nd, (hipStream_t)s);
  OP_TAIL(s);
}
int ef_op_resize_vmap(const float* in, int sc, int sr, float* out, void* s) { eft::resize_map(in, sc, sr, out, false, (hipStream_t)s); OP_TAIL(s); }
int ef_op_resize_nmap(const float* in, int sc, int sr, float* out, void* s) { eft::resize_map(in, sc, sr, out, true, (hipStream_t)s); OP_TAIL(s); }
int ef_op_pyr_down_gauss_f(const float* src, int sc, int sr, float* dst, void* s) { eft::pyr_down_gauss_f(src, sc, sr, dst, (hipStream_t)s); OP_TAIL(s); }
int ef_op_pyr_down_uchar_gauss(const uint8_t* src, int sc, int sr, uint8_t* dst, void* s) { eft::pyr_down_uchar_gauss(src, sc, sr, dst, (hipStream_t)s); OP_TAIL(s); }
int ef_op_vertices_to_depth(const float* tmp, int cols, int rows, float cutoff, float* dst, void* s) { eft::vertices_to_depth(tmp, cols, rows, cutoff, dst, (hipStream_t)s); OP_TAIL(s); }
int ef_op_image_bgr_to_intensity(const uint8_t* rgba, int cols, int rows, uint8_t* dst, void* s) { eft::bgr_to_intensity(rgba, 4, cols, rows, dst, (hipStream_t)s); OP_TAIL(s); }
int ef_op_compute_derivative_images(const uint8_t* src, int cols, int rows, int16_t* dx, int16_t* dy, void* s) {
  eft::derivative_images(src, cols, rows, dx, dy, (hipStream_t)s);
  OP_TAIL(s);
}
int ef_op_project_to_point_cloud(const float* depth, int cols, int rows, const ef_intr* k0, int level, float* cloud, void* s) {
  eft::project_to_point_cloud(depth, cols, rows, eft::intr_level(eft::Intr{k0->fx, k0->fy, k0->cx, k0->cy}, level), cloud, (hipStream_t)s);
  OP_TAIL(s);
}

static int op_scratch(float** partials, float** out, int nfloats_out) {
  if (hipMalloc((void**)partials, (size_t)eft::OP_SCRATCH_FLOATS * sizeof(float)) != hipSuccess) return EF_ENOMEM;
  if (hipMalloc((void**)out, nfloats_out * sizeof(float)) != hipSuccess) { (void)hipFree(*partials); return EF_ENOMEM; }
  return EF_OK;
}
static void unpack29_host(const float* h, float* A, float* b) {
  int shift = 0;
  for (int i = 0; i < 6; ++i)
    for (int j = i; j < 7; ++j) {
      const float v = h[shift++];
      if (j == 6) b[i] = v;
      else A[j * 6 + i] = A[i * 6 + j] = v;
    }
}
int ef_op_icp_step(const float* Rc, const float* tc, const float* vc, const float* nc, const float* Rpi, const float* tp, const ef_intr* k,
                   const float* vg, const float* ng, float dist, float ang, int cols, int rows, float* A, float* b, float* res, void* s) {
  if (cols <= 0 || rows <= 0 || cols > 2048 || rows > 2048) return EF_EINVAL;
  eft::IcpArgs a;
  memcpy(a.Rcurr, Rc, 36); memcpy(a.tcurr, tc, 12); memcpy(a.Rprev_inv, Rpi, 36); memcpy(a.tprev, tp, 12);
  a.k = eft::Intr{k->fx, k->fy, k->cx, k->cy};
  a.distThres = dist; a.angleThres = ang;
  float *partials, *out;
  int r = op_scratch(&partials, &out, 32);
  if (r != EF_OK) return r;
  eft::icp_step_op(a, vc, nc, vg, ng, cols, rows, partials, out, (hipStream_t)s);
  float h[32];
  (void)hipMemcpyAsync(h, out, 29 * sizeof(float), hipMemcpyDeviceToHost, (hipStream_t)s);
  hipError_t e = hipStreamSynchronize((hipStream_t)s);
  (void)hipFree(partials); (void)hipFree(out);
  if (e != hipSuccess) { g_create_error = hipGetErrorString(e); return EF_EHIP; }
  unpack29_host(h, A, b);
  res[0] = h[27]; res[1] = h[28];
  return EF_OK;
}
int ef_op_compute_rgb_residual(float minScale, const int16_t* dIdx, const int16_t* dIdy, const float* lastDepth, const float* nextDepth,
                               const uint8_t* lastImage, const uint8_t* nextImage, void* corres, float maxDepthDelta, const float* kt,
                               const float* krkinv, int cols, int rows, int* sigma, int* count, void* s) {
  eft::RgbResidualArgs a;
  a.minScale = minScale; a.maxDepthDelta = maxDepthDelta;
  memcpy(a.kt, kt, 12); memcpy(a.krkinv, krkinv, 36);
  int* out;
  if (hipMalloc((void**)&out, 2 * sizeof(int)) != hipSuccess) return EF_ENOMEM;
  eft::rgb_residual_op(a, dIdx, dIdy, lastDepth, nextDepth, lastImage, nextImage, corres, cols, rows, out, (hipStream_t)s);
  int h[2] = {0, 0};
  hipError_t e = hipMemcpy(h, out, sizeof(h), hipMemcpyDeviceToHost);
  (void)hipFree(out);
  if (e != hipSuccess) { g_create_error = hipGetErrorString(e); return EF_EHIP; }
  *count = h[0];
  *sigma = h[1];
  return EF_OK;
}
int ef_op_rgb_step(const void* corres, float sigma, const float* cloud, float fx, float fy, const int16_t* dIdx, const int16_t* dIdy,
                   float sobelScale, int cols, int rows, float* A, float* b, void* s) {
  float *partials, *out;
  int r = op_scratch(&partials, &out, 32);
  if (r != EF_OK) return r;
  eft::rgb_step_op(corres, sigma, cloud, fx, fy, dIdx, dIdy, sobelScale, cols, rows, partials, out, (hipStream_t)s);
  float h[32];
  (void)hipMemcpyAsync(h, out, 29 * sizeof(float), hipMemcpyDeviceToHost, (hipStream_t)s);
  hipError_t e = hipStreamSynchronize((hipStream_t)s);
  (void)hipFree(partials); (void)hipFree(out);
  if (e != hipSuccess) { g_create_error = hipGetErrorString(e); return EF_EHIP; }
  unpack29_host(h, A, b);
  return EF_OK;
}
int ef_op_so3_step(const uint8_t* lastImage, const uint8_t* nextImage, const float* ib, const float* kinv, const float* krlr, int cols,
                   int rows, float* A, float* b, float* res, void* s) {
  eft::So3Args a;
  memcpy(a.imageBasis, ib, 36); memcpy(a.kinv, kinv, 36); memcpy(a.krlr, krlr, 36);
  float *partials, *out;
  int r = op_scratch(&partials, &out, 16);
  if (r != EF_OK) return r;
  eft::so3_step_op(a, lastImage, nextImage, cols, rows, partials, out, (hipStream_t)s);
  float h[11];
  (void)hipMemcpyAsync(h, out, sizeof(h), hipMemcpyDeviceToHost, (hipStream_t)s);
  hipError_t e = hipStreamSynchronize((hipStream_t)s);
  (void)hipFree(partials); (void)hipFree(out);
  if (e != hipSuccess) { g_create_error = hipGetErrorString(e); return EF_EHIP; }
  int shift = 0;
  for (int i = 0; i < 3; ++i)
    for (int j = i; j < 4; ++j) {
      const float v = h[shift++];
      if (j == 3) b[i] = v;
      else A[j * 3 + i] = A[i * 3 + j] = v;
    }
  res[0] = h[9]; res[1] = h[10];
  return EF_OK;
}

int ef_op_model_maps(const ef_model_maps_op* a, unsigned* dense_count_left, void* s) {
  if (!a || !dense_count_left || a->cols <= 0 || a->rows <= 0 || a->cols > 2048 || a->rows > 2048 || (a->cols & 3) || (a->rows & 3)) return EF_EINVAL;
  if (!a->pred_vertex || !a->pred_normal || !a->fill_vertex || !a->fill_normal || !a->depth0) return EF_EINVAL;
  if ((a->pred_image == nullptr) != (a->fill_image == nullptr) || (a->pred_image && !a->last0)) return EF_EINVAL;
  for (int i = 0; i < eft::NUM_PYRS; ++i)
    if (!a->vmap[i] || !a->nmap[i]) return EF_EINVAL;
  if (a->joint && (!a->raw || !a->rgb3 || !a->filtered || !a->metric || !a->metric_filtered || !a->next0)) return EF_EINVAL;
  eft::ModelMapsOp o{};
  o.cols = a->cols; o.rows = a->rows;
  o.pred_vertex = a->pred_vertex; o.pred_normal = a->pred_normal; o.fill_vertex = a->fill_vertex; o.fill_normal = a->fill_normal;
  o.pred_image = a->pred_image; o.fill_image = a->fill_image;
  memcpy(o.R, a->R, 36); memcpy(o.t, a->t, 12);
  o.maxDepthRGB = a->max_depth_rgb;
  o.camera_frame = a->camera_frame != 0; o.force_fill_image = a->force_fill_image != 0; o.tally = a->tally != 0;
  o.dense_count = a->dense_count; o.dense_samples = a->dense_samples;
  for (int i = 0; i < eft::NUM_PYRS; ++i) { o.vmap[i] = a->vmap[i]; o.nmap[i] = a->nmap[i]; }
  o.depth0 = a->depth0; o.last0 = a->last0;
  eft::FramePreprocess fp{};
  if (a->joint) {
    fp = eft::FramePreprocess{a->raw, a->depth_cut, efm::bilateral_table(), a->filtered, a->metric, a->metric_filtered, a->rgb3, nullptr};
    if (!fp.table) { g_create_error = "bilateral weight table missing on this device"; return EF_EHIP; }
    o.with = &fp; o.next0 = a->next0;
  }
  const hipError_t e = (hipError_t)eft::model_maps_op(o, dense_count_left, (hipStream_t)s);
  if (e != hipSuccess) { g_create_error = hipGetErrorString(e); return e == hipErrorOutOfMemory ? EF_ENOMEM : EF_EHIP; }
  return EF_OK;
}
int ef_op_sobel_mask(const uint8_t* const* nextImage, const float* const* nextDepth, int cols, int rows, int16_t* const* dIdx, int16_t* const* dIdy,
                     uint8_t* const* mask, uint32_t* const* corres, void* s) {
  if (!nextImage || !nextDepth || !dIdx || !dIdy || !mask || !corres || cols <= 0 || rows <= 0 || cols > 2048 || rows > 2048) return EF_EINVAL;
  eft::SobelMaskOp o{};
  o.cols = cols; o.rows = rows;
  for (int i = 0; i < eft::NUM_PYRS; ++i) {
    if (!nextImage[i] || !nextDepth[i] || !dIdx[i] || !dIdy[i] || !mask[i] || !corres[i]) return EF_EINVAL;
    o.nextImage[i] = nextImage[i]; o.nextDepth[i] = nextDepth[i]; o.dIdx[i] = dIdx[i]; o.dIdy[i] = dIdy[i]; o.mask[i] = mask[i]; o.corres[i] = corres[i];
  }
  eft::sobel_mask_op(o, (hipStream_t)s);
  const hipError_t le = hipGetLastError();
  if (le != hipSuccess) { g_create_error = hipGetErrorString(le); return EF_EHIP; }
  OP_SYNC(s);
  return EF_OK;
}

}
namespace {
__global__ void k_linalg_probe(int which, const double* __restrict__ in, double* __restrict__ out) {
  if (which == EF_LINALG_LDLT6_WAVE || which == EF_LINALG_LDLT6_EVERY_LANE) {
    __shared__ efs::SolveScratch S;
    const int lane = threadIdx.x;
    if (lane < 6) S.b[lane] = in[36 + lane];
    efs::wave_sync();
    if (which == EF_LINALG_LDLT6_WAVE) efs::ldlt6_wave(in[lane < 36 ? lane : 0], S);
    else efs::ldlt6_every_lane(in[lane < 36 ? lane : 0], S);
    if (lane < 6) out[lane] = S.x[lane];
    return;
  }
  if (threadIdx.x != 0) return;
  switch (which) {
    case EF_LINALG_LDLT6: efl::ldlt_solve<double, 6>(in, in + 36, out); break;
    case EF_LINALG_LDLT3F: {
      float A[9], b[3], x[3];
      for (int i = 0; i < 9; ++i) A[i] = (float)in[i];
      for (int i = 0; i < 3; ++i) b[i] = (float)in[9 + i];
      efl::ldlt_solve<float, 3>(A, b, x);
      for (int i = 0; i < 3; ++i) out[i] = (double)x[i];
      break;
    }
    case EF_LINALG_POLAR3: efl::polar3(in, out); break;
    case EF_LINALG_RODRIGUES: efl::rodrigues(in, out); break;
    case EF_LINALG_SE3_INVERSE: efl::se3_matrix(efl::se3_inverse(efl::se3_from_matrix(in)), out); break;
    case EF_LINALG_SE3_LOG_NORM: out[0] = efl::se3_log_norm(efl::se3_from_matrix(in)); break;
    case EF_LINALG_SCALAR:
      out[0] = sqrt(in[0]); out[1] = in[0] / in[1]; out[2] = sin(in[0]); out[3] = cos(in[0]); out[4] = atan2(in[0], in[1]);
      break;
    case EF_LINALG_MAT_TO_QUAT: {
      efl::mat_to_quat(in, out);
      efl::SE3 T;
      efl::se3_set_rotation(T, in);
      for (int i = 0; i < 4; ++i) out[4 + i] = T.q[i];
      break;
    }
    case EF_LINALG_SE3_MUL: {
      const efl::SE3 T = efl::se3_mul(efl::se3_from_matrix(in), efl::se3_from_matrix(in + 16));
      for (int i = 0; i < 4; ++i) out[i] = T.q[i];
      for (int i = 0; i < 3; ++i) out[4 + i] = T.t[i];
      break;
    }
    case EF_LINALG_SE3_CASTF:
    case EF_LINALG_SE3_INVERSE_F: {
      float M[16];
      if (which == EF_LINALG_SE3_CASTF) efl::se3_castf_matrix(efl::se3_from_matrix(in), M);
      else efl::se3_inverse_matrix_f(efl::se3_from_matrix(in), M);
      for (int i = 0; i < 16; ++i) out[i] = (double)M[i];
      break;
    }
    case EF_LINALG_M4_AFFINE_INVERSE: efl::m4_affine_inverse(in, out); break;
    case EF_LINALG_LDLT_PIVOTS: efl::ldlt_pivots<double, 6>(in, out); break;
    case EF_LINALG_LU_INVERSE6: efl::lu_inverse<double, 6>(in, out); break;
    default: break;
  }
}
}
extern "C" {
int ef_op_linalg(int which, const double* in, int n_in, double* out, int n_out) {
  if (!in || !out || n_in <= 0 || n_out <= 0 || n_in > 64 || n_out > 64 || which < 0 || which > EF_LINALG_LU_INVERSE6) return EF_EINVAL;
  double* d;
  if (hipMalloc((void**)&d, 128 * sizeof(double)) != hipSuccess) return EF_ENOMEM;
  (void)hipMemset(d, 0, 128 * sizeof(double));
  (void)hipMemcpy(d, in, n_in * sizeof(double), hipMemcpyHostToDevice);
  hipLaunchKernelGGL(k_linalg_probe, dim3(1), dim3(64), 0, 0, which, (const double*)d, d + 64);
  hipError_t e = hipMemcpy(out, d + 64, n_out * sizeof(double), hipMemcpyDeviceToHost);
  (void)hipFree(d);
  if (e != hipSuccess) { g_create_error = hipGetErrorString(e); return EF_EHIP; }
  return EF_OK;
}

static_assert(sizeof(ef_gn_state) == sizeof(eft::GNState), "ef_gn_state is eft::GNState");
int ef_op_gn_update(const ef_gn_update_args* in, ef_gn_state* next, double* lastA36, double* lastb6, float* stats4) {
  if (!in || !next || !lastA36 || !lastb6 || !stats4 || !(in->icp || in->rgb)) return EF_EINVAL;
  eft::GnUpdateProbe p;
  memcpy(p.sums, in->sums, sizeof(p.sums));
  memcpy(&p.prev, &in->prev, sizeof(p.prev));
  memcpy(p.Rprev, in->Rprev, 36); memcpy(p.tprev, in->tprev, 12);
  p.count = in->count; p.sigma = in->sigma;
  p.icp = in->icp != 0; p.rgb = in->rgb != 0; p.rgbOnly = in->rgb_only != 0;
  p.icpWeight = in->icp_weight;
  p.knext = eft::Intr{in->knext.fx, in->knext.fy, in->knext.cx, in->knext.cy};
  p.level_changes = in->level_changes != 0;
  p.split_tail = in->split_tail != 0;
  const hipError_t e = (hipError_t)eft::gn_update_op(p, (eft::GNState*)next, lastA36, lastb6, stats4);
  if (e != hipSuccess) { g_create_error = hipGetErrorString(e); return e == hipErrorOutOfMemory ? EF_ENOMEM : EF_EHIP; }
  return EF_OK;
}
int ef_op_track_end_tail(const float* Rcurr9, const float* tcurr3, const float* Rprev9, const float* tprev3, const double* q_prev4,
                         const double* t_prev3, int rgb, float weight_multiplier, ef_track_end_out* out) {
  if (!Rcurr9 || !tcurr3 || !Rprev9 || !tprev3 || !q_prev4 || !t_prev3 || !out) return EF_EINVAL;
  eft::TrackState* st = new eft::TrackState();
  memcpy(st->Rprev, Rprev9, 36); memcpy(st->tprev, tprev3, 12);
  memcpy(st->q_prev, q_prev4, 32); memcpy(st->t_prev, t_prev3, 24);
  float pose[12];
  memcpy(pose, Rcurr9, 36); memcpy(pose + 9, tcurr3, 12);
  const hipError_t e = (hipError_t)eft::track_end_tail_op(st, pose, rgb != 0, weight_multiplier, out->logged);
  if (e == hipSuccess) {
    memcpy(out->q, st->q, 32); memcpy(out->t, st->t, 24);
    memcpy(out->T_cw, st->T_cw, 64); memcpy(out->pose_f, st->pose_f, 64);
    memcpy(out->R_wc_f, st->R_wc_f, 36); memcpy(out->t_wc_f, st->t_wc_f, 12);
    out->weighting = st->weighting;
  }
  delete st;
  if (e != hipSuccess) { g_create_error = hipGetErrorString(e); return e == hipErrorOutOfMemory ? EF_ENOMEM : EF_EHIP; }
  return EF_OK;
}

int ef_op_filter_depth(const uint16_t* raw, int cols, int rows, float maxD, uint16_t* filtered, void* s) {
  if (!efm::filter_depth(raw, cols, rows, maxD, filtered, (hipStream_t)s)) return EF_EHIP;
  OP_TAIL(s);
}
int ef_op_metricise_depth(const uint16_t* in, int cols, int rows, float maxD, float* out, void* s) {
  efm::metricise_depth(in, cols, rows, maxD, out, (hipStream_t)s);
  OP_TAIL(s);
}

}
namespace {
struct OpMap {
  std::vector<void*> allocs;
  template <typename T>
  T* alloc(size_t n, int fill = 0) {
    void* p = nullptr;
    if (hipMalloc(&p, (n ? n : 1) * sizeof(T)) != hipSuccess) return nullptr;
// ... 220 lines not shown
```

elasticfusion_amd/csrc/ef_map_kernels.hip:

```cpp
#include "ef_device.hpp"
#include <stdlib.h>
#include <mutex>
#include <hip/hip_ext.h>
#include "ef_map.hpp"
#include "ef_zkey.hpp"
#include "ef_unionfind.hpp"

using namespace ef;

namespace efm {

namespace {

inline int ceil_div(int a, int b) { return (a + b - 1) / b; }
constexpr int SURFEL_GRID = 1024;
constexpr int BLK = 256;
constexpr int CLEAN_GRID = 4096;
static_assert(CLEAN_ROW == BLK, "clean kernels run one element per thread");
static_assert(CLEAN_GRID % 8 == 0, "xcd_row");

__device__ __forceinline__ unsigned long long zkey(float z, uint32_t id) { return ((unsigned long long)depth_key(z) << 32) | id; }
__device__ __forceinline__ unsigned xcd_block() {
  const unsigned g = gridDim.x, x = blockIdx.x & 7u, slot = blockIdx.x >> 3;
  return x * (g >> 3) + (x < (g & 7u) ? x : (g & 7u)) + slot;
// ... 272 lines not shown
                                                      unsigned long long* zbuf, int colmajor, Candidates cand, const uint32_t* __restrict__ winner) {
  const rt34 T = rt34_load16(T16);
  const unsigned count = *count_dev;
  const float ftime = (float)time, ftd = (float)timeDelta;
  for (unsigned id = blockIdx.x * blockDim.x + threadIdx.x; id < count; id += gridDim.x * blockDim.x) {
    float4 pc = map.pos_conf[id];
    float4 ct = map.col_time[id];
    if (MERGE) {
      const uint32_t r = winner[id];
      if (r != WINNER_EMPTY) merge_surfel(cand, (int)r, id, map, time, pc, ct);
    }
    const f3 p = xform(T, f3{pc.x, pc.y, pc.z});
    if (p.z > maxDepth || p.z < 0 || ftime - ct.w > ftd) continue;
    const float u = ((cam.fx * p.x) / p.z) + cam.cx;
    const float v = ((cam.fy * p.y) / p.z) + cam.cy;
    const float xn = (u - (float)cam.cols * 0.5f) / ((float)cam.cols * 0.5f), yn = (v - (float)cam.rows * 0.5f) / ((float)cam.rows * 0.5f);
    const double xw = ((double)xn + 1.0) * 0.5 * (double)cam.cols, yw = ((double)yn + 1.0) * 0.5 * (double)cam.rows;
    if (!(xw >= 0 && xw < cam.cols && yw >= 0 && yw < cam.rows)) continue;
    const int px = (int)floor(xw), py = (int)floor(yw);
    atomicMin(&zbuf[colmajor ? px * cam.rows + py : py * cam.cols + px], zkey(p.z, id));
  }
}
__device__ __forceinline__ float4 index_texel_vert_conf(const rt34& T, float4 pc) {
  const f3 p = xform(T, f3{pc.x, pc.y, pc.z});
  return make_float4(p.x, p.y, p.z, pc.w);
}
__device__ __forceinline__ float4 index_texel_norm_rad(const rt34& T, float4 nr) {
  const f3 n = normalized(mul(T.R, f3{nr.x, nr.y, nr.z}));
  return make_float4(n.x, n.y, n.z, nr.w);
}
template <bool CLEAR>
__global__ void __launch_bounds__(BLK) k_index_resolve(const Cam cam, const float* __restrict__ T16, SurfelSoA map,
                                                        unsigned long long* zbuf, IndexMaps out) {
  const int pi = blockIdx.x * blockDim.x + threadIdx.x;
  if (pi >= cam.cols * cam.rows) return;
  const unsigned long long key = zbuf[pi];
  if (key == ZBUF_EMPTY) {
    out.index[pi] = 0u;
    out.vert_conf[pi] = make_float4(0, 0, 0, 0);
    if (out.color_time) out.color_time[pi] = make_float4(0, 0, 0, 0);
    out.norm_rad[pi] = make_float4(0, 0, 0, 0);
    return;
  }
  if (CLEAR) zbuf[pi] = ZBUF_EMPTY;
  const uint32_t id = (uint32_t)key;
  const rt34 T = rt34_load16(T16);
  const float4 pc = map.pos_conf[id];
  const float4 nr = map.nrm_rad[id];
  out.index[pi] = id;
  out.vert_conf[pi] = index_texel_vert_conf(T, pc);
  if (out.color_time) out.color_time[pi] = map.col_time[id];
  out.norm_rad[pi] = index_texel_norm_rad(T, nr);
}

struct Sprite {
  f3 p, n;
  float rad, conf;
  float u, v, hs;
  bool ok;
};
__device__ __forceinline__ float glmin(float x, float y) { return y < x ? y : x; }
__device__ __forceinline__ float glmax(float x, float y) { return x < y ? y : x; }
__device__ __forceinline__ Sprite make_sprite(const Cam& cam, const rt34& T, float4 pc, float4 ct, float4 nr, float maxDepth,
                                              float confThreshold, float ftime, float fmaxTime, float ftd) {
  Sprite S;
  S.ok = false;
  S.p = xform(T, f3{pc.x, pc.y, pc.z});
  if (S.p.z > maxDepth || S.p.z < 0 || pc.w < confThreshold || ftime - ct.w > ftd || ct.w > fmaxTime) return S;
  S.n = normalized(mul(T.R, f3{nr.x, nr.y, nr.z}));
  S.rad = nr.w;
  S.conf = pc.w;
  const f3 t1 = normalized(f3{S.n.y - S.n.z, -S.n.x, S.n.x});
  const f3 x1{(t1.x * S.rad) * 1.41421356f, (t1.y * S.rad) * 1.41421356f, (t1.z * S.rad) * 1.41421356f};
  const f3 y1 = cross(S.n, x1);
  const float fx = cam.fx, fy = cam.fy, cx = cam.cx, cy = cam.cy;
  const f3 a = S.p + x1, b = S.p + y1, c = S.p - y1, d = S.p - x1;
  const float q1x = ((fx * a.x) / a.z) + cx, q1y = ((fy * a.y) / a.z) + cy;
  const float q2x = ((fx * b.x) / b.z) + cx, q2y = ((fy * b.y) / b.z) + cy;
  const float q3x = ((fx * c.x) / c.z) + cx, q3y = ((fy * c.y) / c.z) + cy;
  const float q4x = ((fx * d.x) / d.z) + cx, q4y = ((fy * d.y) / d.z) + cy;
  const float xmin = glmin(q1x, glmin(q2x, glmin(q3x, q4x))), xmax = glmax(q1x, glmax(q2x, glmax(q3x, q4x)));
  const float ymin = glmin(q1y, glmin(q2y, glmin(q3y, q4y))), ymax = glmax(q1y, glmax(q2y, glmax(q3y, q4y)));
  float size = glmax(0.f, glmax(fabsf(xmax - xmin), fabsf(ymax - ymin)));
  size = fminf(fmaxf(size, 1.0f), 2047.0f);
  S.u = ((fx * S.p.x) / S.p.z) + cx;
  S.v = ((fy * S.p.y) / S.p.z) + cy;
  if (!(S.u >= 0 && S.u < (float)cam.cols && S.v >= 0 && S.v < (float)cam.rows)) return S;
  S.hs = size * 0.5f;
  S.ok = true;
  return S;
}
__device__ __forceinline__ f3 pixel_ray(const Cam& cam, int px, int py) {
  const float fcx = (float)px + 0.5f, fcy = (float)py + 0.5f;
  return normalized(f3{(fcx - cam.cx) / cam.fx, (fcy - cam.cy) / cam.fy, 1.0f});
}
__device__ __forceinline__ bool sprite_fragment_ray(const f3& Sp, const f3& Sn, float rad, float psn, const f3& l, float& z) {
  const float k = psn / dot(l, Sn);
  const f3 cp{k * l.x, k * l.y, k * l.z};
  const f3 diff = cp - Sp;
  if (!(dot(diff, diff) <= rad * rad)) return false;
  z = cp.z;
  return true;
}
__device__ __forceinline__ bool sprite_fragment(const Cam& cam, const Sprite& S, int px, int py, float& z) {
  return sprite_fragment_ray(S.p, S.n, S.rad, dot(S.p, S.n), pixel_ray(cam, px, py), z);
}
__global__ void k_ray_table(const Cam cam, float4* __restrict__ rays) {
  const int i = blockIdx.x * blockDim.x + threadIdx.x;
  if (i >= cam.cols * cam.rows) return;
  const int px = i / cam.rows, py = i - px * cam.rows;
  const f3 l = pixel_ray(cam, px, py);
  rays[i] = make_float4(l.x, l.y, l.z, 0.f);
}
constexpr int SPLAT_LANES = 4;
constexpr int SPLAT_GRID = SURFEL_GRID * SPLAT_LANES;
template <bool LUT>
__global__ void __launch_bounds__(BLK) k_surface_splat(const Cam cam, const float* __restrict__ T16, SurfelSoA map,
                                                        const unsigned* __restrict__ count_dev, float maxDepth, float confThreshold,
                                                        int time, int maxTime, int timeDelta, unsigned long long* zbuf,
                                                        unsigned* consumed_mark, unsigned consumed_value, const float4* __restrict__ rays) {
  if (consumed_mark && blockIdx.x == 0 && threadIdx.x == 0)
    __hip_atomic_store(consumed_mark, consumed_value, __ATOMIC_RELAXED, __HIP_MEMORY_SCOPE_SYSTEM);
  const rt34 T = rt34_load16(T16);
  const unsigned count = *count_dev;
  const unsigned sub = threadIdx.x % SPLAT_LANES;
  const unsigned stride = gridDim.x * blockDim.x / SPLAT_LANES;
  for (unsigned id = (blockIdx.x * blockDim.x + threadIdx.x) / SPLAT_LANES; id < count; id += stride) {
    const float4 pc = map.pos_conf[id];
    if (pc.w < confThreshold) continue;
    const float4 ct = map.col_time[id];
    const float4 nr = map.nrm_rad[id];
    const Sprite S = make_sprite(cam, T, pc, ct, nr, maxDepth, confThreshold, (float)time, (float)maxTime, (float)timeDelta);
    if (!S.ok) continue;
    const int px0 = max(0, (int)ceilf(S.u - S.hs - 0.5f)), px1 = min(cam.cols - 1, (int)ceilf(S.u + S.hs - 0.5f) - 1);
    const int py0 = max(0, (int)ceilf(S.v - S.hs - 0.5f)), py1 = min(cam.rows - 1, (int)ceilf(S.v + S.hs - 0.5f) - 1);
    const int hgt = py1 - py0 + 1, nfrag = (px1 - px0 + 1) * hgt;
    const float psn = dot(S.p, S.n);
    for (int f = (int)sub; f < nfrag; f += SPLAT_LANES) {
      const int fx = f / hgt, py = py0 + (f - fx * hgt), px = px0 + fx;
      const int zi = px * cam.rows + py;
      f3 l;
      if (LUT) { const float4 r = rays[zi]; l = f3{r.x, r.y, r.z}; }
      else l = pixel_ray(cam, px, py);
      float z;
      if (!sprite_fragment_ray(S.p, S.n, S.rad, psn, l, z)) continue;
      if (z != z) continue;
      unsigned long long* cell = &zbuf[zi];
      const unsigned long long key = zkey(z, id);
      atomicMin(cell, key);
    }
  }
}

__device__ __forceinline__ f3 fill_vertex_at(const uint16_t* __restrict__ d, const Cam& cam, int sx, int sy, int x, int y, float inv_fx,
                                             float inv_fy) {
  const float z = (float)d[clampi(sy, 0, cam.rows - 1) * cam.cols + clampi(sx, 0, cam.cols - 1)] / 1000.0f;
  return {((float)x - cam.cx) * z * inv_fx, ((float)y - cam.cy) * z * inv_fy, z};
}
__device__ __forceinline__ void fill_in_px(const Cam& cam, int x, int y, uchar4 si, float4 sv, float4 sn,
                                           const uint16_t* __restrict__ depth_filtered, const uint8_t* __restrict__ rgb3, bool passthrough,
                                           bool passthroughImage, FillMaps out) {
  const int pi = y * cam.cols + x;
  const float inv_fx = 1.0f / cam.fx, inv_fy = 1.0f / cam.fy;
  if (sv.z == 0 || passthrough) {
    const f3 v = fill_vertex_at(depth_filtered, cam, x, y, x, y, inv_fx, inv_fy);
    out.vertex[pi] = make_float4(v.x, v.y, v.z, 1.f);
  } else {
    out.vertex[pi] = sv;
  }
  if (sn.z == 0 || passthrough) {
    const f3 v = fill_vertex_at(depth_filtered, cam, x, y, x, y, inv_fx, inv_fy);
    const f3 vx = fill_vertex_at(depth_filtered, cam, x + 1, y, x + 1, y, inv_fx, inv_fy);
    const f3 vy = fill_vertex_at(depth_filtered, cam, x, y + 1, x, y + 1, inv_fx, inv_fy);
    const f3 nn = normalized(cross(vx - v, vy - v));
    out.normal[pi] = make_float4(nn.x, nn.y, nn.z, 1.f);
  } else {
    out.normal[pi] = sn;
  }
  if ((si.x == 0 && si.y == 0 && si.z == 0) || passthroughImage) {
    out.image[pi] = make_uchar4(rgb3[(size_t)pi * 3], rgb3[(size_t)pi * 3 + 1], rgb3[(size_t)pi * 3 + 2], 255);
  } else {
    out.image[pi] = si;
  }
}
__device__ __forceinline__ void dense_sample(const Cam& cam, int x, int y, uchar4 si, unsigned* counter) {
  if (counter && x % 20 == 10 && y % 20 == 10 && x / 20 < cam.cols / 20 && y / 20 < cam.rows / 20)
    if (si.x > 0 && si.y > 0 && si.z > 0) atomicAdd(counter, 1u);
}

template <bool FUSE_FILL>
__global__ void __launch_bounds__(BLK) k_surface_resolve(const Cam cam, const float* __restrict__ T16, SurfelSoA map, float maxDepth,
                                                          float confThreshold, int time, int maxTime, int timeDelta,
                                                          unsigned long long* zbuf, PredictMaps out, FillMaps fill,
                                                          const uint16_t* __restrict__ depth_filtered, const uint8_t* __restrict__ rgb3,
                                                          bool passthroughImage, unsigned* dense_counter, unsigned* nonempty_flag,
                                                          unsigned nonempty_value) {
  const int lane = threadIdx.x & 63, wave = threadIdx.x >> 6;
  const int px = blockIdx.x * 16 + (wave & 1) * 8 + (lane >> 3), py = blockIdx.y * 16 + (wave >> 1) * 8 + (lane & 7);
  if (px >= cam.cols || py >= cam.rows) return;
  const int pi = py * cam.cols + px, zi = px * cam.rows + py;
  const unsigned long long key = zbuf[zi];
  uchar4 im = make_uchar4(0, 0, 0, 0);
  float4 vt = make_float4(0, 0, 0, 0), nm = make_float4(0, 0, 0, 0);
  uint16_t tm = 0;
  if (key != ZBUF_EMPTY) {
    if (nonempty_flag) *nonempty_flag = nonempty_value;
    zbuf[zi] = ZBUF_EMPTY;
    const uint32_t id = (uint32_t)key;
    const rt34 T = rt34_load16(T16);
    const float4 pc = map.pos_conf[id], ct = map.col_time[id], nr = map.nrm_rad[id];
    const Sprite S = make_sprite(cam, T, pc, ct, nr, maxDepth, confThreshold, (float)time, (float)maxTime, (float)timeDelta);
    float z = 0.f;
    sprite_fragment(cam, S, px, py, z);
    const f3 col = decodeColor(ct.x);
    im = make_uchar4((uint8_t)roundf(col.x * 255.0f), (uint8_t)roundf(col.y * 255.0f), (uint8_t)roundf(col.z * 255.0f), 255);
    const float fcx = (float)px + 0.5f, fcy = (float)py + 0.5f;
    vt = make_float4((fcx - cam.cx) * z * (1.f / cam.fx), (fcy - cam.cy) * z * (1.f / cam.fy), z, pc.w);
    nm = make_float4(S.n.x, S.n.y, S.n.z, nr.w);
    tm = (uint16_t)(unsigned)ct.z;
  }
  out.image[pi] = im;
  out.vertex[pi] = vt;
  out.normal[pi] = nm;
  out.time[pi] = tm;
  if (FUSE_FILL) {
    fill_in_px(cam, px, py, im, vt, nm, depth_filtered, rgb3, false, passthroughImage, fill);
    dense_sample(cam, px, py, im, dense_counter);
  }
}
__global__ void __launch_bounds__(BLK) k_depth_resolve(const Cam cam, const float* __restrict__ T16, SurfelSoA map, float maxDepth,
                                                        float confThreshold, int time, int maxTime, int timeDelta, unsigned long long* zbuf,
                                                        float* __restrict__ depth) {
  const int cols = cam.cols, rows = cam.rows;
  const int pi = blockIdx.x * blockDim.x + threadIdx.x;
  if (pi >= cols * rows) return;
  const int py = pi / cols, px = pi - py * cols, zi = px * rows + py;
  const unsigned long long key = zbuf[zi];
  float z = 0.f;
  if (key != ZBUF_EMPTY) {
    zbuf[zi] = ZBUF_EMPTY;
    z = depth_of_key((uint32_t)(key >> 32));
    if (z == 0.f) {
      const uint32_t id = (uint32_t)key;
      const rt34 T = rt34_load16(T16);
      const Sprite S = make_sprite(cam, T, map.pos_conf[id], map.col_time[id], map.nrm_rad[id], maxDepth, confThreshold, (float)time,
                                   (float)maxTime, (float)timeDelta);
      sprite_fragment(cam, S, px, py, z);
    }
  }
  depth[pi] = z;
}
__global__ void __launch_bounds__(BLK) k_fill_in(const Cam cam, PredictMaps pred, const uint16_t* __restrict__ depth_filtered,
                                                  const uint8_t* __restrict__ rgb3, bool passthrough, bool passthroughImage, FillMaps out) {
  const int pi = blockIdx.x * blockDim.x + threadIdx.x;
  if (pi >= cam.cols * cam.rows) return;
  const int py = pi / cam.cols, px = pi - py * cam.cols;
  fill_in_px(cam, px, py, pred.image[pi], pred.vertex[pi], pred.normal[pi], depth_filtered, rgb3, passthrough, passthroughImage, out);
}
__global__ void k_dense_count(const Cam cam, const uchar4* __restrict__ image, unsigned* counter) {
  const int dc = cam.cols / 20, dr = cam.rows / 20;
  const int i = blockIdx.x * blockDim.x + threadIdx.x;
  if (i >= dc * dr) return;
  const int b = i / dc, a = i - b * dc;
  const uchar4 t = image[(20 * b + 10) * cam.cols + (20 * a + 10)];
  if (t.x > 0 && t.y > 0 && t.z > 0) atomicAdd(counter, 1u);
}

struct FuseArgs {
  Cam cam;
  const float* pose16;
  int time;
  const uint8_t* rgb3;
  const float* dm;
  const float* dmf;
  IndexMaps im;
  float maxDepth;
  const float* weighting;
  KeyedIndex key;
  unsigned long long* zclear;
};
constexpr int ASSOC_LANES = 4;
constexpr int ASSOC_SLOTS = (9 + ASSOC_LANES - 1) / ASSOC_LANES;
static_assert(ASSOC_LANES == 1 || ASSOC_LANES == 2 || ASSOC_LANES == 4 || ASSOC_LANES == 8, "a wavefront holds whole pixels; the combine knows offsets 1, 2, 4");
template <int OFF>
__device__ __forceinline__ uint32_t assoc_lane_down(uint32_t v) {
  static_assert(OFF == 1 || OFF == 2 || OFF == 4, "");
  constexpr int ctrl = OFF == 1 ? 0xF5  : OFF == 2 ? 0xEE  : 0x104 ;
  return (uint32_t)__builtin_amdgcn_update_dpp(0, (int)v, ctrl, 0xF, 0xF, true);
}
template <int OFF>
__device__ __forceinline__ void assoc_combine(float& bestDist, uint32_t& best) {
  const float d = __uint_as_float(assoc_lane_down<OFF>(__float_as_uint(bestDist)));
  const uint32_t id = assoc_lane_down<OFF>(best);
  if (d < bestDist) {
    bestDist = d;
    best = id;
  }
}
template <bool KEYED>
__global__ void __launch_bounds__(BLK) k_associate(const FuseArgs A, Candidates cand, uint32_t* winner, int colwalk) {
  const Cam cam = A.cam;
  const int qc = cam.cols / 2, qr = cam.rows / 2;
  const int t = (int)(xcd_block() * blockDim.x + threadIdx.x);
  if (KEYED && A.zclear)
    for (int i = t, P = cam.cols * cam.rows, step = (int)(gridDim.x * blockDim.x); i < P; i += step) A.zclear[i] = ZBUF_EMPTY;
  const int q = t / ASSOC_LANES, sub = t % ASSOC_LANES;
  if (q >= qc * qr) return;
  const int seg_len = 9 / ASSOC_LANES + (sub < 9 % ASSOC_LANES ? 1 : 0);
  const int seg_first = sub * (9 / ASSOC_LANES) + (sub < 9 % ASSOC_LANES ? sub : 9 % ASSOC_LANES);
  const int qy = colwalk ? q % qr : q / qc, qx = colwalk ? q / qr : q - (q / qc) * qc;
  const int par = A.time % 2;
  const int i = 2 * qx + par, j = 2 * qy + par;
  const int r = qx * qr + qy;
  float4 c_col = make_float4(0, 0, 0, 0);
  if (i < cam.cols && j < cam.rows) {
    const float cx = cam.cx, cy = cam.cy;
    const float inv_fx = (float)(1.0 / (double)cam.fx), inv_fy = (float)(1.0 / (double)cam.fy);
    const DepthF DR{A.dm, cam.cols, cam.rows}, DF{A.dmf, cam.cols, cam.rows};
    const float x = pix_coord(i, cam.cols), y = pix_coord(j, cam.rows);
    const float ftime = (float)A.time;
    const f3 vPosLocal = getVertexF(DR, i, j, x, y, cx, cy, inv_fx, inv_fy);
    const bool sel = ((int)x % 2 == (int)ftime % 2 && (int)y % 2 == (int)ftime % 2);
    const bool nb = !(DR.at(i - 1, j) == 0 || DR.at(i, j - 1) == 0 || DR.at(i + 1, j) == 0 || DR.at(i, j + 1) == 0);
    const float zf_c = DF.at(i, j), zf_xf = DF.at(i + 1, j), zf_xb = DF.at(i - 1, j), zf_yf = DF.at(i, j + 1), zf_yb = DF.at(i, j - 1);
    const uint8_t* c = A.rgb3 + (size_t)(j * cam.cols + i) * 3;
    const uint8_t c0 = c[0], c1 = c[1], c2 = c[2];
    const float weighting = *A.weighting;
    uint32_t idxs[ASSOC_SLOTS];
    float4 vcs[ASSOC_SLOTS], nrs[ASSOC_SLOTS];
    uint2 keys[ASSOC_SLOTS];
#pragma unroll
    for (int m = 0; m < ASSOC_SLOTS; ++m) {
      const int k = m < seg_len ? seg_first + m : 8;
      const int a3 = (k >= 3) + (k >= 6), b3 = k - 3 * a3;
      const int tx = clampi(i + a3 - 1, 0, cam.cols - 1), ty = clampi(j + b3 - 1, 0, cam.rows - 1);
      const int ti = im_texel(A.im, cam, tx, ty);
      if (KEYED) {
        keys[m] = reinterpret_cast<const uint2*>(A.key.keys)[ti];
      } else {
        const uint32_t id = A.im.index[ti];
        idxs[m] = m < seg_len ? id : 0U;
        vcs[m] = A.im.vert_conf[ti];
        nrs[m] = A.im.norm_rad[ti];
      }
    }
    const rt34 pose = rt34_load16(A.pose16);
    if (sel && nb && vPosLocal.z > 0 && vPosLocal.z <= A.maxDepth) {
      auto vtx = [&](float z, float xx, float yy) { return f3{(xx - cx) * z * inv_fx, (yy - cy) * z * inv_fy, z}; };
      const f3 vPosition_f = vtx(zf_c, x, y);
      const f3 xf = vtx(zf_xf, x + 1, y), xb = vtx(zf_xb, x - 1, y), yf = vtx(zf_yf, x, y + 1), yb = vtx(zf_yb, x, y - 1);
      const f3 del_x = half_sum(xb, vPosition_f) - half_sum(xf, vPosition_f);
      const f3 del_y = half_sum(yb, vPosition_f) - half_sum(yf, vPosition_f);
      const f3 vNormLocal = normalized(cross(del_x, del_y));
      uint32_t best = 0;
      float bestDist = 1000;
      const float xl = (x - cx) * inv_fx, yl = (y - cy) * inv_fy;
      const float lambda = sqrtf(xl * xl + yl * yl + 1);
      const f3 ray{xl, yl, 1};
      const float lenRay = sqrtf(dot(ray, ray));
      const float lenN = sqrtf(dot(vNormLocal, vNormLocal));
      const rt34 Tcw = rt34_load16(KEYED ? A.key.T_cw16_dev : A.pose16);
      if (KEYED) {
#pragma unroll
        for (int m = 0; m < ASSOC_SLOTS; ++m) {
          const uint32_t id = keys[m].x;
          float vcz = depth_of_key(keys[m].y);
          asm volatile("" : "+v"(vcz));
          const bool tap = m < seg_len && (id & keys[m].y) != 0xFFFFFFFFu  && id > 0U && fabsf((vcz * lambda) - (vPosLocal.z * lambda)) < 0.05f;
          idxs[m] = tap ? id : 0U;
        }
#pragma unroll
        for (int m = 0; m < ASSOC_SLOTS; ++m) {
          vcs[m] = A.key.map.pos_conf[idxs[m]];
          nrs[m] = A.key.map.nrm_rad[idxs[m]];
        }
      }
#pragma unroll
      for (int m = 0; m < ASSOC_SLOTS; ++m) {
        const uint32_t current = idxs[m];
        if (current > 0U) {
          const float4 vc = KEYED ? index_texel_vert_conf(Tcw, vcs[m]) : vcs[m];
// ... 674 lines not shown
```

elasticfusion_amd/csrc/ef_track.hpp:

```cpp
#pragma once
#include <hip/hip_runtime.h>
#include <stdint.h>

#include "ef_build.hpp"

namespace eft {

constexpr int NUM_PYRS = 3;
constexpr int REDUCE_BLOCK = 256;
constexpr int VTHREADS = 16384;
constexpr int VWARPS = VTHREADS / 32;
constexpr int RGB_SLOTS = 64;
constexpr int SE3_ACCS = 29;
constexpr int SO3_ACCS = 11;
constexpr int SE3_PAIRS = VWARPS / 2;
constexpr int PARTIAL_FLOATS = 2 * SE3_ACCS * SE3_PAIRS > SO3_ACCS * VWARPS ? 2 * SE3_ACCS * SE3_PAIRS : SO3_ACCS * VWARPS;
constexpr int PT_WGS = 128, PT_BLOCK = 512, PT_MAX_ITER = 16, PT_MAX_PIXELS = 8 * VTHREADS, PT_SYNC_FLOATS = 1024;
constexpr int PARTIAL_ALLOC_FLOATS = (2 * PARTIAL_FLOATS + PT_SYNC_FLOATS) > 196608 ? (2 * PARTIAL_FLOATS + PT_SYNC_FLOATS) : 196608;
constexpr int FT_EPOCHS = 64;

struct Intr { float fx, fy, cx, cy; };
__host__ __device__ inline Intr intr_level(const Intr& k, int level) {
  const int div = 1 << level;
  return Intr{k.fx / div, k.fy / div, k.cx / div, k.cy / div};
// ... 1 lines not shown

struct GNState {
  float Rcurr[9], tcurr[3];
  double resultRt[16];
  float krkinv[9], kt[3];
  float lastRGBErrorLevel;
  int rgb_broken;
};

struct TrackState {
  double q[4];
  double t[3];
  double q_prev[4];
  double t_prev[3];
  float Rprev[9], tprev[3], Rprev_inv[9];
  GNState gn[2];
  int rgb_slots[2][RGB_SLOTS][16];
  float lastICPError, lastICPCount, lastRGBError, lastRGBCount, lastSO3Error, lastSO3Count;
  double lastA[36], lastb[6];
  int so3_iterations;
  double so3_resultR[9], so3_lastResultR[9];
  float so3_R_lr[9];
  float so3_mats[27];
  float so3_lastError, so3_lastCount;
  int so3_done;
  unsigned so3_ticket;
  float weighting;
  unsigned dense_count;
  int dense_samples;
  int tick;
  unsigned long long step_rec[16];
  unsigned call_seq;
  unsigned step_timeout;
  unsigned long long dbg_clock[16];
  unsigned map_counts[2];
  unsigned model_view_stamp;
  float T_cw[16];
  float pose_f[16];
  float R_wc_f[9], t_wc_f[3];
};

struct TrackerPlan {
  int script = 0;
  int n_small = 0;
  int n_iter = 0;
  unsigned long long levels = 0;
  unsigned res_bytes = 0;
  unsigned res_budget = 0;
};

struct Pyramid {
  int width, height;
  uint16_t* depth_tmp[NUM_PYRS];
  float* vmap_curr[NUM_PYRS];
  float* nmap_curr[NUM_PYRS];
  float* vmap_g_prev[NUM_PYRS];
  float* nmap_g_prev[NUM_PYRS];
  float* lastDepth[NUM_PYRS];
  float* nextDepth[NUM_PYRS];
  uint8_t* lastImage[NUM_PYRS];
  uint8_t* nextImage[NUM_PYRS];
  uint8_t* lastNextImage[NUM_PYRS];
  int16_t* dIdx[NUM_PYRS];
  int16_t* dIdy[NUM_PYRS];
  uint32_t* corres[NUM_PYRS];
  uint8_t* rgbMask[NUM_PYRS];
  float* partials;
  unsigned epoch = 1;
  int last_mode = 0;
  unsigned sticky_abort = 0, fallbacks_base = 0;
  TrackerPlan plan;
  int W(int l) const { return width >> l; }
  int H(int l) const { return height >> l; }
};

struct KernelProbe {
  hipEvent_t* start;
  hipEvent_t* stop;
  int capacity;
  int used;
};

struct TrackParams {
  bool rgbOnly, pyramid, fastOdom, so3;
  float icpWeight;
  float distThres, angleThres;
  int fused_step = 0;
  int persistent = 1;
  const unsigned* empty_model_flag = nullptr;
  unsigned empty_model_value = 0;
  int no_resident = 0;
};
static_assert(sizeof(TrackParams) == 4 + 4 + 8 + 4 + 4 + 8 + 4 + 4, "TrackParams has no padding bytes (it is compared with memcmp)");

void pyr_down_u16(const uint16_t* src, int scols, int srows, uint16_t* dst, hipStream_t s);
void create_vmap(const uint16_t* depth, int cols, int rows, Intr k, float cutoff, float* vmap, hipStream_t s);
void create_nmap(const float* vmap, int cols, int rows, float* nmap, hipStream_t s);
void transform_maps(const float* vsrc, const float* nsrc, int cols, int rows, const float* R9_dev, const float* t3_dev,
                    float* vdst, float* ndst, hipStream_t s);
void copy_maps(const float* vtex, const float* ntex, int cols, int rows, float* vmaps_tmp, float* vmap, float* nmap, hipStream_t s);
void resize_map(const float* in, int scols, int srows, float* out, bool normalize, hipStream_t s);
void pyr_down_gauss_f(const float* src, int scols, int srows, float* dst, hipStream_t s);
void pyr_down_uchar_gauss(const uint8_t* src, int scols, int srows, uint8_t* dst, hipStream_t s);
void vertices_to_depth(const float* vmaps_tmp, int cols, int rows, float cutoff, float* dst, hipStream_t s);
void bgr_to_intensity(const uint8_t* src, int channels, int cols, int rows, uint8_t* dst, hipStream_t s);
void derivative_images(const uint8_t* src, int cols, int rows, int16_t* dx, int16_t* dy, hipStream_t s);
void project_to_point_cloud(const float* depth, int cols, int rows, Intr k, float* cloud, hipStream_t s);

struct IcpArgs {
  float Rcurr[9], tcurr[3], Rprev_inv[9], tprev[3];
  Intr k;
  float distThres, angleThres;
};
constexpr int OP_SCRATCH_FLOATS = SE3_ACCS * VWARPS + 64;
void icp_step_op(const IcpArgs& a, const float* vmap_curr, const float* nmap_curr, const float* vmap_g_prev,
                 const float* nmap_g_prev, int cols, int rows, float* scratch, float* out29_dev, hipStream_t s);
struct RgbResidualArgs {
  float minScale, maxDepthDelta;
  float kt[3], krkinv[9];
};
void rgb_residual_op(const RgbResidualArgs& a, const int16_t* dIdx, const int16_t* dIdy, const float* lastDepth,
                     const float* nextDepth, const uint8_t* lastImage, const uint8_t* nextImage, void* corres, int cols,
                     int rows, int* out2_dev, hipStream_t s);
void rgb_step_op(const void* corres, float sigma, const float* cloud, float fx, float fy, const int16_t* dIdx,
                 const int16_t* dIdy, float sobelScale, int cols, int rows, float* scratch, float* out29_dev, hipStream_t s);
struct So3Args { float imageBasis[9], kinv[9], krlr[9]; };
void so3_step_op(const So3Args& a, const uint8_t* lastImage, const uint8_t* nextImage, int cols, int rows, float* scratch,
                 float* out11_dev, hipStream_t s);

struct GnUpdateProbe {
  float sums[2 * SE3_ACCS];
  GNState prev;
  float Rprev[9], tprev[3];
  int count, sigma;
  bool icp, rgb, rgbOnly;
  float icpWeight;
  Intr knext;
  bool level_changes;
  bool split_tail;
};
int gn_update_op(const GnUpdateProbe& p, GNState* next_host, double* lastA36, double* lastb6, float* stats4);
int track_end_tail_op(TrackState* st_host, const float* pose12, bool rgb, float weightMultiplier, double* logged16);

struct FramePreprocess {
  const uint16_t* raw;
  float maxD;
  const float* table;
  uint16_t* filtered;
  float* metric;
  float* metric_filtered;
  const uint8_t* rgb3;
  uint8_t* rgb_keep;
};
void init_icp_model(const Pyramid& p, const float* pred_vertex, const float* pred_normal, const float* fill_vertex,
                    const float* fill_normal, const TrackState* st, float maxDepthRGB, hipStream_t s, const uint8_t* pred_image_rgba = nullptr,
                    const uint8_t* fill_image_rgba = nullptr, bool frameToFrameRGB = false, const FramePreprocess* with = nullptr,
                    bool tally = false );
void init_icp_maps(const Pyramid& p, const float* vertex4, const float* normal4, const uint8_t* image_rgba, const TrackState* st,
                   float maxDepthRGB, hipStream_t s);
void build_pyramids(const Pyramid& p, const uint16_t* depth_filtered, Intr k, float cutoff, hipStream_t s, bool with_sobel);
void build_pyramids_frame_side(const Pyramid& p, const uint16_t* depth_filtered, Intr k, float cutoff, hipStream_t s);
void build_pyramids_model_side(const Pyramid& p, hipStream_t s);
void init_rgb_sobel(const Pyramid& p, hipStream_t s);
void init_model_pair(const Pyramid& p, const float* model_vertex4, const float* model_normal4, const uint8_t* model_image_rgba,
                     const float* cur_vertex4, const float* cur_normal4, const uint8_t* cur_image_rgba, const TrackState* st, float maxDepthRGB,
                     hipStream_t s);
struct ModelMapsOp {
  int cols, rows;
  const float *pred_vertex, *pred_normal, *fill_vertex, *fill_normal;
  const uint8_t *pred_image, *fill_image;
  float R[9], t[3], maxDepthRGB;
  bool camera_frame, force_fill_image, tally;
  unsigned dense_count;
  int dense_samples;
  float* vmap[NUM_PYRS];
  float* nmap[NUM_PYRS];
  float* depth0;
  uint8_t* last0;
  const FramePreprocess* with;
  uint8_t* next0;
};
int model_maps_op(const ModelMapsOp& o, unsigned* dense_count_left, hipStream_t s);
struct SobelMaskOp {
  int cols, rows;
  const uint8_t* nextImage[NUM_PYRS];
  const float* nextDepth[NUM_PYRS];
  int16_t* dIdx[NUM_PYRS];
  int16_t* dIdy[NUM_PYRS];
  uint8_t* mask[NUM_PYRS];
  uint32_t* corres[NUM_PYRS];
};
void sobel_mask_op(const SobelMaskOp& o, hipStream_t s);
void init_first_rgb(const Pyramid& p, const uint8_t* rgb3, hipStream_t s);
struct TrackTail {
  int cur, slots;
  bool has_head, icp, rgb, rgbOnly;
  float icpWeight;
  Intr k0;
  const float* pairs;
  int ng = 0;
  bool merged_end = false;
  unsigned epoch = 0;
  float* partials = nullptr;
};
TrackTail track(Pyramid& p, TrackState* st, Intr k, const TrackParams& tp, hipStream_t s, KernelProbe* probe = nullptr,
                KernelProbe* probe_all = nullptr);
int tracker_aborted(const Pyramid& p, hipStream_t s);
void track_prepare(Pyramid& p, const TrackParams& tp, hipStream_t s);
int tracker_fallbacks(const Pyramid& p, hipStream_t s);
void persistent_chain_forget(hipStream_t s);
int tracker_small_clocks(const Pyramid& p, unsigned long long* out32, hipStream_t s);
void track_swap(Pyramid& p, const TrackParams& tp);
void track_end(TrackState* st, const TrackTail& tail, bool rgb, float weightMultiplier, double* traj, int slot, hipStream_t s,
               const unsigned* abort_word = nullptr, unsigned* abort_report = nullptr);
unsigned* tracker_abort_word(const Pyramid& p);
void pose_injected(TrackState* st, const double* T_wc16, bool save_prev, float weightMultiplier, bool with_weighting, double* traj,
                   int slot, hipStream_t s);
void log_pose(const TrackState* st, double* traj, int slot, hipStream_t s);
void pose_restored(TrackState* st, const double* q4, const double* t3, hipStream_t s);
void copy_pose(TrackState* dst, const TrackState* src, hipStream_t s);
void adopt_pose(TrackState* st, const TrackState* est, double* traj, int slot, hipStream_t s);
void sample_constraints(const float* vertex4, const uint16_t* old_time, int cols, int rows, int step, float* out4, hipStream_t s);

}
```

elasticfusion_amd/csrc/ef_track_host_inputs.inc:

```
namespace {
inline dim3 model_maps_grid(const Pyramid& p) {
  return dim3(ceil_div(p.W(0), 64), ceil_div(p.H(0) / 4, 4));
}
ModelMapsArgs model_maps_args(const Pyramid& p, bool model_side, const float* vertex, const float* normal, float maxDepthRGB) {
  ModelMapsArgs A{};
  A.pred_vertex = A.fill_vertex = (const float4*)vertex;
  A.pred_normal = A.fill_normal = (const float4*)normal;
  for (int i = 0; i < NUM_PYRS; ++i) {
    A.vmap[i] = model_side ? p.vmap_g_prev[i] : p.vmap_curr[i];
    A.nmap[i] = model_side ? p.nmap_g_prev[i] : p.nmap_curr[i];
  }
  A.depth0 = model_side ? p.lastDepth[0] : p.nextDepth[0];
  A.cols = p.W(0); A.rows = p.H(0);
  A.maxDepthRGB = maxDepthRGB;
  A.camera_frame = !model_side;
  return A;
}
struct PyrJob { const void* src; void* dst; int type; };
enum { PYR_U16 = 0, PYR_F32 = 1, PYR_U8 = 2 };
void launch_pyr_step(const Pyramid& p, int i, std::initializer_list<PyrJob> jobs, hipStream_t s) {
  PyrJobs J{};
  int n = 0;
  for (const PyrJob& j : jobs) { J.src[n] = j.src; J.dst[n] = j.dst; J.type[n] = j.type; ++n; }
  J.scols = p.W(i); J.srows = p.H(i);
  dim3 g = tile_grid(p.W(i + 1), p.H(i + 1));
  g.z = n;
  hipLaunchKernelGGL(k_pyr_down_multi, g, tile_block(), 0, s, J);
}
inline const uint16_t* frame_depth(const Pyramid& p, const uint16_t* depth_filtered, int i) { return i == 0 ? depth_filtered : p.depth_tmp[i]; }

SobelLevels sobel_levels_of(const Pyramid& p) {
  SobelLevels L;
  const float minGrad[NUM_PYRS] = {5, 3, 1};
  const float sobelScale = 1.0f / 8.0f;
  for (int i = 0; i < NUM_PYRS; ++i) {
    L.src[i] = p.nextImage[i]; L.dx[i] = p.dIdx[i]; L.dy[i] = p.dIdy[i];
    L.nextDepth[i] = p.nextDepth[i]; L.mask[i] = p.rgbMask[i]; L.corres[i] = p.corres[i];
    L.minScale[i] = (float)(pow((double)minGrad[i], 2.0) / pow((double)sobelScale, 2.0));
    L.cols[i] = p.W(i); L.rows[i] = p.H(i);
  }
  return L;
}
void build_vn_levels(const Pyramid& p, const uint16_t* depth_filtered, Intr k, float cutoff, bool with_sobel, hipStream_t s) {
  VNLevels L;
  for (int i = 0; i < NUM_PYRS; ++i) {
    L.depth[i] = frame_depth(p, depth_filtered, i);
    L.vmap[i] = p.vmap_curr[i];
    L.nmap[i] = p.nmap_curr[i];
    L.cols[i] = p.W(i);
    L.rows[i] = p.H(i);
    L.k[i] = intr_level(k, i);
  }
  L.cutoff = cutoff;
  dim3 g = tile_grid(p.W(0), p.H(0));
  if (with_sobel) {
    g.z = 2 * NUM_PYRS;
    hipLaunchKernelGGL(k_vn_sobel_levels, g, tile_block(), 0, s, L, sobel_levels_of(p));
    return;
  }
  g.z = NUM_PYRS;
  hipLaunchKernelGGL(k_vmap_nmap_levels, g, tile_block(), 0, s, L);
}
ModelMapsArgs model_maps_choice_args(const Pyramid& p, bool model_side, const float* pred_vertex, const float* pred_normal, const float* fill_vertex,
                                     const float* fill_normal, const TrackState* st, float maxDepthRGB, const uint8_t* pred_image_rgba,
                                     const uint8_t* fill_image_rgba, bool frameToFrameRGB, bool tally) {
  ModelMapsArgs A = model_maps_args(p, model_side, pred_vertex, pred_normal, maxDepthRGB);
  A.fill_vertex = (const float4*)fill_vertex; A.fill_normal = (const float4*)fill_normal;
  A.pred_image = pred_image_rgba; A.fill_image = fill_image_rgba; A.force_fill_image = frameToFrameRGB;
  A.tally_image = (tally && pred_image_rgba) ? pred_image_rgba : nullptr;
  A.tally_out = const_cast<unsigned*>(&st->dense_count);
  A.last0 = pred_image_rgba ? p.lastImage[0] : nullptr;
  return A;
}
void launch_model_maps(const Pyramid& p, const ModelMapsArgs& A, const TrackState* st, const FramePreprocess* with, hipStream_t s) {
  const dim3 mg = model_maps_grid(p);
  if (with) {
    PreArgs P{};
    P.raw = with->raw; P.cols = p.W(0); P.rows = p.H(0); P.maxv = (unsigned)(with->maxD * 1000.0f); P.table = with->table;
    P.filtered = with->filtered; P.metric = with->metric; P.metric_filtered = with->metric_filtered;
    P.rgb3 = with->rgb3; P.next0 = p.nextImage[0]; P.rgb_keep = with->rgb_keep;
    P.tiles_x = (P.cols + pre::PRE_TW - 1) / pre::PRE_TW;
    P.tiles = P.tiles_x * ((P.rows + pre::PRE_TH - 1) / pre::PRE_TH);
    P.mm_x = (int)mg.x;
    hipLaunchKernelGGL(k_frame_inputs, dim3(P.tiles + (int)(mg.x * mg.y)), dim3(64, 4), 0, s, P, A, st);
    return;
  }
  hipLaunchKernelGGL(k_model_maps, mg, dim3(64, 4), 0, s, A, st);
}
}

void init_icp_model(const Pyramid& p, const float* pred_vertex, const float* pred_normal, const float* fill_vertex,
                    const float* fill_normal, const TrackState* st, float maxDepthRGB, hipStream_t s, const uint8_t* pred_image_rgba,
                    const uint8_t* fill_image_rgba, bool frameToFrameRGB, const FramePreprocess* with, bool tally) {
  launch_model_maps(p, model_maps_choice_args(p, true, pred_vertex, pred_normal, fill_vertex, fill_normal, st, maxDepthRGB, pred_image_rgba,
                                               fill_image_rgba, frameToFrameRGB, tally), st, with, s);
}
int model_maps_op(const ModelMapsOp& o, unsigned* dense_count_left, hipStream_t s) {
  Pyramid p{};
  p.width = o.cols; p.height = o.rows;
  for (int i = 0; i < NUM_PYRS; ++i) {
    p.vmap_g_prev[i] = p.vmap_curr[i] = o.vmap[i];
    p.nmap_g_prev[i] = p.nmap_curr[i] = o.nmap[i];
  }
  p.lastDepth[0] = p.nextDepth[0] = o.depth0;
  p.lastImage[0] = o.last0;
  p.nextImage[0] = o.next0;
  TrackState* h = new TrackState();
  for (int i = 0; i < 9; ++i) h->R_wc_f[i] = o.R[i];
  for (int i = 0; i < 3; ++i) h->t_wc_f[i] = o.t[i];
  h->dense_count = o.dense_count;
  h->dense_samples = o.dense_samples;
  TrackState* st = nullptr;
  hipError_t e = hipMalloc((void**)&st, sizeof(TrackState));
  if (e == hipSuccess) e = hipMemcpy(st, h, sizeof(TrackState), hipMemcpyHostToDevice);
  if (e == hipSuccess) {
    launch_model_maps(p, model_maps_choice_args(p, !o.camera_frame, o.pred_vertex, o.pred_normal, o.fill_vertex, o.fill_normal, st, o.maxDepthRGB,
                                                 o.pred_image, o.fill_image, o.force_fill_image, o.tally), st, o.with, s);
    e = hipGetLastError();
  }
  if (e == hipSuccess) e = hipStreamSynchronize(s);
  if (e == hipSuccess) e = hipMemcpy(dense_count_left, &st->dense_count, sizeof(unsigned), hipMemcpyDeviceToHost);
  if (st) (void)hipFree(st);
  delete h;
  return (int)e;
}
void init_icp_maps(const Pyramid& p, const float* vertex, const float* normal, const uint8_t* image_rgba, const TrackState* st,
                   float maxDepthRGB, hipStream_t s) {
  hipLaunchKernelGGL(k_model_maps, model_maps_grid(p), dim3(64, 4), 0, s, model_maps_args(p, false, vertex, normal, maxDepthRGB), st);
  const int n = p.W(0) * p.H(0);
  for (int i = 0; i + 1 < NUM_PYRS; ++i) pyr_down_gauss_f(p.nextDepth[i], p.W(i), p.H(i), p.nextDepth[i + 1], s);
  hipLaunchKernelGGL(k_model_intensity, dim3(ceil_div(n, 256)), dim3(256), 0, s, image_rgba, image_rgba, true, st, n, p.nextImage[0]);
  for (int i = 0; i + 1 < NUM_PYRS; ++i) pyr_down_uchar_gauss(p.nextImage[i], p.W(i), p.H(i), p.nextImage[i + 1], s);
}
void init_model_pair(const Pyramid& p, const float* model_vertex, const float* model_normal, const uint8_t* model_image_rgba, const float* cur_vertex,
                     const float* cur_normal, const uint8_t* cur_image_rgba, const TrackState* st, float maxDepthRGB, hipStream_t s) {
  hipLaunchKernelGGL(k_model_maps, model_maps_grid(p), dim3(64, 4), 0, s, model_maps_args(p, true, model_vertex, model_normal, maxDepthRGB), st);
  hipLaunchKernelGGL(k_model_maps, model_maps_grid(p), dim3(64, 4), 0, s, model_maps_args(p, false, cur_vertex, cur_normal, maxDepthRGB), st);
  const int n = p.W(0) * p.H(0);
  hipLaunchKernelGGL(k_rgba_intensity_pair, dim3(ceil_div(n, 256), 2), dim3(256), 0, s, model_image_rgba, cur_image_rgba, n, p.lastImage[0], p.nextImage[0]);
  for (int i = 0; i + 1 < NUM_PYRS; ++i)
    launch_pyr_step(p, i, {{p.lastDepth[i], p.lastDepth[i + 1], PYR_F32}, {p.nextDepth[i], p.nextDepth[i + 1], PYR_F32},
                           {p.lastImage[i], p.lastImage[i + 1], PYR_U8}, {p.nextImage[i], p.nextImage[i + 1], PYR_U8}}, s);
}
void build_pyramids(const Pyramid& p, const uint16_t* depth_filtered, Intr k, float cutoff, hipStream_t s, bool with_sobel) {
  for (int i = 0; i + 1 < NUM_PYRS; ++i)
    launch_pyr_step(p, i, {{frame_depth(p, depth_filtered, i), p.depth_tmp[i + 1], PYR_U16}, {p.lastDepth[i], p.lastDepth[i + 1], PYR_F32},
                           {p.lastImage[i], p.lastImage[i + 1], PYR_U8}, {p.nextImage[i], p.nextImage[i + 1], PYR_U8}}, s);
  build_vn_levels(p, depth_filtered, k, cutoff, with_sobel, s);
}
void build_pyramids_frame_side(const Pyramid& p, const uint16_t* depth_filtered, Intr k, float cutoff, hipStream_t s) {
  for (int i = 0; i + 1 < NUM_PYRS; ++i)
    launch_pyr_step(p, i, {{frame_depth(p, depth_filtered, i), p.depth_tmp[i + 1], PYR_U16}, {p.nextImage[i], p.nextImage[i + 1], PYR_U8}}, s);
  build_vn_levels(p, depth_filtered, k, cutoff, false, s);
}
void build_pyramids_model_side(const Pyramid& p, hipStream_t s) {
  for (int i = 0; i + 1 < NUM_PYRS; ++i)
    launch_pyr_step(p, i, {{p.lastDepth[i], p.lastDepth[i + 1], PYR_F32}, {p.lastImage[i], p.lastImage[i + 1], PYR_U8}}, s);
}
void init_rgb_sobel(const Pyramid& p, hipStream_t s) {
  dim3 g = tile_grid(p.W(0), p.H(0));
  g.z = NUM_PYRS;
  hipLaunchKernelGGL(k_sobel_levels, g, tile_block(), 0, s, sobel_levels_of(p));
}
void sobel_mask_op(const SobelMaskOp& o, hipStream_t s) {
  Pyramid p{};
  p.width = o.cols; p.height = o.rows;
  for (int i = 0; i < NUM_PYRS; ++i) {
    p.nextImage[i] = const_cast<uint8_t*>(o.nextImage[i]); p.nextDepth[i] = const_cast<float*>(o.nextDepth[i]);
    p.dIdx[i] = o.dIdx[i]; p.dIdy[i] = o.dIdy[i]; p.rgbMask[i] = o.mask[i]; p.corres[i] = o.corres[i];
  }
  init_rgb_sobel(p, s);
}

void init_first_rgb(const Pyramid& p, const uint8_t* rgb3, hipStream_t s) {
  bgr_to_intensity(rgb3, 3, p.W(0), p.H(0), p.lastNextImage[0], s);
  for (int i = 0; i + 1 < NUM_PYRS; ++i) pyr_down_uchar_gauss(p.lastNextImage[i], p.W(i), p.H(i), p.lastNextImage[i + 1], s);
}
```

elasticfusion_amd/csrc/ef_track_kernels.hip:

```cpp
#include "ef_device.hpp"
#include "ef_linalg_dev.hpp"
#include "ef_solve_dev.hpp"
#include <stddef.h>
#include <initializer_list>
#include <mutex>
#include <type_traits>
#include <hip/hip_ext.h>
#include "ef_track.hpp"

using namespace ef;

namespace eft {

namespace {

constexpr int TILE_X = 64, TILE_Y = 4;

inline dim3 tile_grid(int cols, int rows) { return dim3((cols + TILE_X - 1) / TILE_X, (rows + TILE_Y - 1) / TILE_Y); }
inline dim3 tile_block() { return dim3(TILE_X, TILE_Y); }


__device__ __forceinline__ void pyr_down_u16_px(const uint16_t* __restrict__ src, int scols, int srows, uint16_t* __restrict__ dst, int x, int y) {
  const int dcols = scols / 2;
  const int D = 5;
// ... 286 lines not shown
__global__ void k_rgba_intensity_pair(const uint8_t* __restrict__ last_rgba, const uint8_t* __restrict__ next_rgba, int n, uint8_t* __restrict__ last0,
                                      uint8_t* __restrict__ next0) {
  const int i = blockIdx.x * blockDim.x + threadIdx.x;
  if (i >= n) return;
  const uchar4 c = ((const uchar4*)(blockIdx.y == 0 ? last_rgba : next_rgba))[i];
  (blockIdx.y == 0 ? last0 : next0)[i] = intensity_of((float)c.x, (float)c.y, (float)c.z);
}

__device__ __forceinline__ float sobel_gsx(int k) {
  const float a = 0.52201f, b = 0.79451f;
  return k == 8 ? -a : k == 7 ? 0.00000f : k == 6 ? a : k == 5 ? -b : k == 4 ? -0.00000f : k == 3 ? b : k == 2 ? -a : k == 1 ? 0.00000f : a;
}
__device__ __forceinline__ float sobel_gsy(int k) {
  const float a = 0.52201f, b = 0.79451f;
  return k == 8 ? -a : k == 7 ? -b : k == 6 ? -a : (k >= 3) ? 0.00000f : k == 2 ? a : k == 1 ? b : a;
}
__device__ __forceinline__ void sobel_taps(const float (&v)[3][3], int cols, int rows, int x, int y, int16_t& dx, int16_t& dy) {
  const float gsx[9] = {0.52201f, 0.00000f, -0.52201f, 0.79451f, -0.00000f, -0.79451f, 0.52201f, 0.00000f, -0.52201f};
  const float gsy[9] = {0.52201f, 0.79451f, 0.52201f, 0.00000f, 0.00000f, 0.00000f, -0.52201f, -0.79451f, -0.52201f};
  float dxVal = 0, dyVal = 0;
  if (x >= 1 && y >= 1 && x <= cols - 2 && y <= rows - 2) {
    int k = 8;
#pragma unroll
    for (int dj = 0; dj < 3; ++dj)
#pragma unroll
      for (int di = 0; di < 3; ++di) {
        dxVal += v[dj][di] * gsx[k];
        dyVal += v[dj][di] * gsy[k];
        --k;
      }
  } else {
    const int jlo = max(y - 1, 0), ilo = max(x - 1, 0), ni = min(x + 1, cols - 1) - ilo + 1;
#pragma unroll
    for (int dj = 0; dj < 3; ++dj)
#pragma unroll
      for (int di = 0; di < 3; ++di) {
        const int j = y - 1 + dj, i = x - 1 + di;
        if (j >= 0 && j <= rows - 1 && i >= 0 && i <= cols - 1) {
          const int k = 8 - ((j - jlo) * ni + (i - ilo));
          dxVal += v[dj][di] * sobel_gsx(k);
          dyVal += v[dj][di] * sobel_gsy(k);
        }
      }
  }
  dx = (int16_t)(int)dxVal;
  dy = (int16_t)(int)dyVal;
}
__device__ __forceinline__ void sobel_px(const uint8_t* __restrict__ src, int cols, int rows, int x, int y, int16_t* dx, int16_t* dy) {
  float v[3][3];
#pragma unroll
  for (int dj = 0; dj < 3; ++dj)
#pragma unroll
    for (int di = 0; di < 3; ++di) v[dj][di] = (float)src[min(max(y - 1 + dj, 0), rows - 1) * cols + min(max(x - 1 + di, 0), cols - 1)];
  int16_t ox, oy;
  sobel_taps(v, cols, rows, x, y, ox, oy);
  dx[y * cols + x] = ox;
  dy[y * cols + x] = oy;
}
__global__ void k_sobel(const uint8_t* __restrict__ src, int cols, int rows, int16_t* __restrict__ dx, int16_t* __restrict__ dy) {
  const int x = blockIdx.x * blockDim.x + threadIdx.x, y = blockIdx.y * blockDim.y + threadIdx.y;
  if (x >= cols || y >= rows) return;
  sobel_px(src, cols, rows, x, y, dx, dy);
}
__device__ __forceinline__ uint32_t pack_corres(int u0, int v0, int idiff) {
  return 0x80000000u | ((uint32_t)(idiff + 255) << 22) | ((uint32_t)v0 << 11) | (uint32_t)u0;
}
struct SobelLevels {
  const uint8_t* src[NUM_PYRS];
  int16_t* dx[NUM_PYRS];
  int16_t* dy[NUM_PYRS];
  const float* nextDepth[NUM_PYRS];
  uint8_t* mask[NUM_PYRS];
  uint32_t* corres[NUM_PYRS];
  float minScale[NUM_PYRS];
  int cols[NUM_PYRS], rows[NUM_PYRS];
};
__device__ __forceinline__ void sobel_mask_px(const SobelLevels& L, int l, int x, int y) {
  const int cols = L.cols[l], rows = L.rows[l];
  if (x >= cols || y >= rows) return;
  const uint8_t* __restrict__ img = L.src[l];
  const int k = y * cols + x;
  int w[4][4];
#pragma unroll
  for (int a = 0; a < 4; ++a)
#pragma unroll
    for (int b = 0; b < 4; ++b) w[a][b] = img[min(max(y - 2 + a, 0), rows - 1) * cols + min(max(x - 2 + b, 0), cols - 1)];
  const float nd = L.nextDepth[l][k];
  float v[3][3];
#pragma unroll
  for (int dj = 0; dj < 3; ++dj)
#pragma unroll
    for (int di = 0; di < 3; ++di) v[dj][di] = (float)w[dj + 1][di + 1];
  int16_t sx, sy;
  sobel_taps(v, cols, rows, x, y, sx, sy);
  L.dx[l][k] = sx;
  L.dy[l][k] = sy;
  bool ok = (x < cols - 5 && y < rows - 1);
#pragma unroll
  for (int a = 0; a < 4; ++a)
#pragma unroll
    for (int b = 0; b < 4; ++b) {
      const int u = y - 2 + a, vv = x - 2 + b;
      if (u >= 0 && u < rows && vv >= 0 && vv < cols) ok = ok && (w[a][b] > 0);
    }
  if (ok) {
    const int valx = sx, valy = sy;
    const float mTwo = (float)((valx * valx) + (valy * valy));
    ok = mTwo >= L.minScale[l] && !isnan(nd);
  }
  L.mask[l][k] = ok ? 1 : 0;
  L.corres[l][k] = 0u;
}
__global__ void k_sobel_levels(const SobelLevels L) {
  sobel_mask_px(L, blockIdx.z, blockIdx.x * blockDim.x + threadIdx.x, blockIdx.y * blockDim.y + threadIdx.y);
}
__global__ void k_vn_sobel_levels(const VNLevels V, const SobelLevels S) {
  const int z = blockIdx.z, x = blockIdx.x * blockDim.x + threadIdx.x, y = blockIdx.y * blockDim.y + threadIdx.y;
  if (z < NUM_PYRS) vmap_nmap_px(V, z, x, y);
  else sobel_mask_px(S, z - NUM_PYRS, x, y);
}

__device__ __forceinline__ f3 project_point(int x, int y, float z, float invFx, float invFy, float cx, float cy) {
  return {(float)((x - cx) * z * invFx), (float)((y - cy) * z * invFy), z};
}
__global__ void k_project_points(const float* __restrict__ depth, int cols, int rows, float invFx, float invFy, float cx,
                                 float cy, float* __restrict__ cloud) {
  const int x = blockIdx.x * blockDim.x + threadIdx.x, y = blockIdx.y * blockDim.y + threadIdx.y;
  if (x >= cols || y >= rows) return;
  const f3 p = project_point(x, y, depth[y * cols + x], invFx, invFy, cx, cy);
  float* c = cloud + (size_t)(y * cols + x) * 3;
  c[0] = p.x; c[1] = p.y; c[2] = p.z;
}

__device__ __forceinline__ bool use_fill_in(const TrackState* __restrict__ st) {
  return !((float)st->dense_count / (float)st->dense_samples > 0.75f);
}
struct ModelMapsArgs {
  const float4* pred_vertex;
  const float4* pred_normal;
  const float4* fill_vertex;
  const float4* fill_normal;
  float* vmap[NUM_PYRS];
  float* nmap[NUM_PYRS];
  float* depth0;
  int cols, rows;
  float maxDepthRGB;
  bool camera_frame;
  const uint8_t* pred_image;
  const uint8_t* fill_image;
  bool force_fill_image;
  uint8_t* last0;
  const uint8_t* tally_image;
  unsigned* tally_out;
};
__device__ __forceinline__ bool model_maps_use_fill(const ModelMapsArgs& A, const TrackState* __restrict__ st, bool first_wg) {
  if (!A.tally_image) return use_fill_in(st);
  __shared__ unsigned tally_s[4];
  const int t = (int)(threadIdx.y * blockDim.x + threadIdx.x);
  const int dc = A.cols / 20, dr = A.rows / 20;
  unsigned cnt = 0;
  for (int i = t; i < dc * dr; i += 256) {
    const int b = i / dc, a = i - b * dc;
    const uchar4 px = ((const uchar4*)A.tally_image)[(20 * b + 10) * A.cols + (20 * a + 10)];
    cnt += (px.x > 0 && px.y > 0 && px.z > 0) ? 1u : 0u;
  }
#pragma unroll
  for (int off = 32; off > 0; off >>= 1) cnt += __shfl_down(cnt, off, 64);
  if ((t & 63) == 0) tally_s[t >> 6] = cnt;
  __syncthreads();
  const unsigned total = tally_s[0] + tally_s[1] + tally_s[2] + tally_s[3];
  if (first_wg && t == 0) *A.tally_out = total;
  return !((float)total / (float)st->dense_samples > 0.75f);
}
template <bool ALL_PLANES>
__device__ __forceinline__ void store_planar(float* m, int cols, int rows, int x, int y, bool valid, f3 v) {
  if (valid) {
    m[(y + rows) * cols + x] = v.y;
    m[(y + 2 * rows) * cols + x] = v.z;
    m[y * cols + x] = v.x;
  } else {
    m[y * cols + x] = qnan();
    if (ALL_PLANES) {
      m[(y + rows) * cols + x] = qnan();
      m[(y + 2 * rows) * cols + x] = qnan();
    }
  }
}
__device__ __forceinline__ float qx1(float x) { return __int_as_float(__builtin_amdgcn_mov_dpp(__float_as_int(x), 0xB1, 0xF, 0xF, true)); }
__device__ __forceinline__ float qx2(float x) { return __int_as_float(__builtin_amdgcn_mov_dpp(__float_as_int(x), 0x4E, 0xF, 0xF, true)); }
__device__ __forceinline__ f3 qx1(f3 v) { return f3{qx1(v.x), qx1(v.y), qx1(v.z)}; }
__device__ __forceinline__ f3 qx2(f3 v) { return f3{qx2(v.x), qx2(v.y), qx2(v.z)}; }
__device__ __forceinline__ f3 box4(f3 a, f3 b, f3 c, f3 d) {
  return f3{(a.x + b.x + c.x + d.x) / 4, (a.y + b.y + c.y + d.y) / 4, (a.z + b.z + c.z + d.z) / 4};
}
__device__ __forceinline__ void model_maps_lane(const ModelMapsArgs& A, const TrackState* __restrict__ st, int gx, int by, bool fill) {
  const int cols = A.cols, rows = A.rows;
  if (gx >= cols || by * 4 >= rows) return;
  const int j = gx & 3, bx = gx >> 2;
  const bool even = (j & 1) == 0, leftpair = j < 2;
  const float4* __restrict__ vsrc = fill ? A.fill_vertex : A.pred_vertex;
  const float4* __restrict__ nsrc = fill ? A.fill_normal : A.pred_normal;
  const m33 R = m33_load(st->R_wc_f);
  const f3 t{st->t_wc_f[0], st->t_wc_f[1], st->t_wc_f[2]};
  const bool cf = A.camera_frame;
  const int c1 = cols / 2, r1 = rows / 2, c2 = cols / 4, r2 = rows / 4;
  float4 vs[4], ns[4];
#pragma unroll
  for (int r = 0; r < 4; ++r) {
    vs[r] = vsrc[(by * 4 + r) * cols + gx];
    ns[r] = nsrc[(by * 4 + r) * cols + gx];
  }
  if (A.last0) {
    const uchar4* __restrict__ isrc = (const uchar4*)((A.force_fill_image || fill) ? A.fill_image : A.pred_image);
    uchar4 cs[4];
#pragma unroll
    for (int r = 0; r < 4; ++r) cs[r] = isrc[(by * 4 + r) * cols + gx];
#pragma unroll
    for (int r = 0; r < 4; ++r) A.last0[(by * 4 + r) * cols + gx] = intensity_of((float)cs[r].x, (float)cs[r].y, (float)cs[r].z);
  }
  f3 v0[4], n0[4];
#pragma unroll
  for (int r = 0; r < 4; ++r) {
    const int y = by * 4 + r;
    const bool ok = !(vs[r].z == 0);
    v0[r] = {vs[r].x, vs[r].y, vs[r].z};
    n0[r] = {ns[r].x, ns[r].y, ns[r].z};
    A.depth0[y * cols + gx] = (vs[r].z > A.maxDepthRGB || vs[r].z <= 0) ? qnan() : vs[r].z;
    const bool nok = ok && !isnan(ns[r].x);
    if (cf) {
      store_planar<true>(A.vmap[0], cols, rows, gx, y, ok, v0[r]);
      store_planar<true>(A.nmap[0], cols, rows, gx, y, ok, n0[r]);
    } else {
      store_planar<true>(A.vmap[0], cols, rows, gx, y, ok && !isnan(vs[r].x), mul(R, v0[r]) + t);
      store_planar<true>(A.nmap[0], cols, rows, gx, y, nok, mul(R, n0[r]));
    }
  }
  f3 v1[2], n1[2];
  bool v1ok[2], n1ok[2];
#pragma unroll
  for (int qy = 0; qy < 2; ++qy) {
    const f3 pv0 = qx1(v0[2 * qy]), pv1 = qx1(v0[2 * qy + 1]), pn0 = qx1(n0[2 * qy]), pn1 = qx1(n0[2 * qy + 1]);
    const f3 va = even ? v0[2 * qy] : pv0, vb = even ? pv0 : v0[2 * qy], vc = even ? v0[2 * qy + 1] : pv1, vd = even ? pv1 : v0[2 * qy + 1];
    const f3 na_ = even ? n0[2 * qy] : pn0, nb = even ? pn0 : n0[2 * qy], nc = even ? n0[2 * qy + 1] : pn1, nd = even ? pn1 : n0[2 * qy + 1];
    const bool oka = !(va.z == 0), okb = !(vb.z == 0), okc = !(vc.z == 0), okd = !(vd.z == 0);
    const bool vok = oka && okb && okc && okd && !isnan(va.x) && !isnan(vb.x) && !isnan(vc.x) && !isnan(vd.x);
    const bool nok = oka && okb && okc && okd && !isnan(na_.x) && !isnan(nb.x) && !isnan(nc.x) && !isnan(nd.x);
    const f3 vavg = box4(va, vb, vc, vd);
    const f3 navg = normalized(box4(na_, nb, nc, nd));
    v1[qy] = vavg; n1[qy] = navg;
    v1ok[qy] = vok; n1ok[qy] = nok;
    if (even) {
      const int x1 = bx * 2 + (j >> 1), y1 = by * 2 + qy;
      if (cf) {
        store_planar<false>(A.vmap[1], c1, r1, x1, y1, vok, vavg);
        store_planar<false>(A.nmap[1], c1, r1, x1, y1, nok, navg);
      } else {
        store_planar<false>(A.vmap[1], c1, r1, x1, y1, vok && !isnan(vavg.x), mul(R, vavg) + t);
        store_planar<false>(A.nmap[1], c1, r1, x1, y1, nok && !isnan(navg.x), mul(R, navg));
      }
    }
  }
  const f3 ov0 = qx2(v1[0]), ov1 = qx2(v1[1]), on0 = qx2(n1[0]), on1 = qx2(n1[1]);
  const bool ovok0 = qx2(v1ok[0] ? 1.0f : 0.0f) != 0.0f, ovok1 = qx2(v1ok[1] ? 1.0f : 0.0f) != 0.0f;
  const bool onok0 = qx2(n1ok[0] ? 1.0f : 0.0f) != 0.0f, onok1 = qx2(n1ok[1] ? 1.0f : 0.0f) != 0.0f;
  const f3 v00 = leftpair ? v1[0] : ov0, v01 = leftpair ? ov0 : v1[0], v10 = leftpair ? v1[1] : ov1, v11 = leftpair ? ov1 : v1[1];
  const f3 n00 = leftpair ? n1[0] : on0, n01 = leftpair ? on0 : n1[0], n10 = leftpair ? n1[1] : on1, n11 = leftpair ? on1 : n1[1];
  const bool vok2 = v1ok[0] && ovok0 && v1ok[1] && ovok1 && !isnan(v00.x) && !isnan(v01.x) && !isnan(v10.x) && !isnan(v11.x);
  const bool nok2 = n1ok[0] && onok0 && n1ok[1] && onok1 && !isnan(n00.x) && !isnan(n01.x) && !isnan(n10.x) && !isnan(n11.x);
  const f3 va = box4(v00, v01, v10, v11);
  const f3 na = normalized(box4(n00, n01, n10, n11));
  if (j == 0) {
    if (cf) {
      store_planar<false>(A.vmap[2], c2, r2, bx, by, vok2, va);
      store_planar<false>(A.nmap[2], c2, r2, bx, by, nok2, na);
    } else {
      store_planar<false>(A.vmap[2], c2, r2, bx, by, vok2 && !isnan(va.x), mul(R, va) + t);
      store_planar<false>(A.nmap[2], c2, r2, bx, by, nok2 && !isnan(na.x), mul(R, na));
    }
  }
}
__global__ void __launch_bounds__(256) k_model_maps(const ModelMapsArgs A, const TrackState* __restrict__ st) {
  const bool fill = model_maps_use_fill(A, st, blockIdx.x == 0 && blockIdx.y == 0);
  model_maps_lane(A, st, (int)(blockIdx.x * blockDim.x + threadIdx.x), (int)(blockIdx.y * blockDim.y + threadIdx.y), fill);
}
struct IcpView {
  const float* vmap_curr;
  const float* nmap_curr;
  const float* vmap_g_prev;
  const float* nmap_g_prev;
  int cols, rows;
  Intr k;
  float distThres, angleThres;
  float dist2Max, sine2Max;
};
struct IcpPose { m33 Rcurr; f3 tcurr; m33 Rprev_inv; f3 tprev; };
__device__ __forceinline__ float uniform_f(float x) { return __uint_as_float(__builtin_amdgcn_readfirstlane(__float_as_uint(x))); }
__device__ __forceinline__ f3 uniform_f3(f3 a) { return f3{uniform_f(a.x), uniform_f(a.y), uniform_f(a.z)}; }
__device__ __forceinline__ m33 uniform_m33(const m33& m) { return m33{{uniform_f3(m.r[0]), uniform_f3(m.r[1]), uniform_f3(m.r[2])}}; }
__device__ __forceinline__ IcpPose icp_pose_uniform(const IcpPose& P) {
  return IcpPose{uniform_m33(P.Rcurr), uniform_f3(P.tcurr), uniform_m33(P.Rprev_inv), uniform_f3(P.tprev)};
}

__device__ __forceinline__ bool icp_row(const IcpView& V, const IcpPose& P, int x, int y, float (&row)[7]) {
  const int cols = V.cols, rows = V.rows;
  const int plane = cols * rows, idx = y * cols + x;
  const f3 vcurr{V.vmap_curr[idx], V.vmap_curr[idx + plane], V.vmap_curr[idx + 2 * plane]};
  const f3 vcurr_g = mul(P.Rcurr, vcurr) + P.tcurr;
  const f3 vcurr_cp = mul(P.Rprev_inv, vcurr_g - P.tprev);
  const int ux = f2i_rn(vcurr_cp.x * V.k.fx / vcurr_cp.z + V.k.cx);
  const int uy = f2i_rn(vcurr_cp.y * V.k.fy / vcurr_cp.z + V.k.cy);
  if (ux < 0 || uy < 0 || ux >= cols || uy >= rows || vcurr_cp.z < 0) return false;
  const int pidx = uy * cols + ux;
  const f3 vprev_g{V.vmap_g_prev[pidx], V.vmap_g_prev[pidx + plane], V.vmap_g_prev[pidx + 2 * plane]};
  const f3 ncurr{V.nmap_curr[idx], V.nmap_curr[idx + plane], V.nmap_curr[idx + 2 * plane]};
  const f3 ncurr_g = mul(P.Rcurr, ncurr);
  const f3 nprev_g{V.nmap_g_prev[pidx], V.nmap_g_prev[pidx + plane], V.nmap_g_prev[pidx + 2 * plane]};
  const float dist = norm(vprev_g - vcurr_g);
  const float sine = norm(cross(ncurr_g, nprev_g));
  if (!(sine < V.angleThres && dist <= V.distThres && !isnan(ncurr.x) && !isnan(nprev_g.x))) return false;
  const f3 s_cp = mul(P.Rprev_inv, vcurr_g - P.tprev);
  const f3 d_cp = mul(P.Rprev_inv, vprev_g - P.tprev);
  const f3 n_cp = mul(P.Rprev_inv, nprev_g);
  const f3 c = cross(s_cp, n_cp);
  row[0] = n_cp.x; row[1] = n_cp.y; row[2] = n_cp.z;
  row[3] = c.x; row[4] = c.y; row[5] = c.z;
  row[6] = dot(n_cp, s_cp - d_cp);
  return true;
}

struct RgbView {
  const void* corres;
  const float* lastDepth;
  const float* cloud;
  const int16_t* dIdx;
  const int16_t* dIdy;
  int cols, rows;
  Intr k;
  float sobelScale;
};
template <bool PACKED>
__device__ __forceinline__ bool rgb_row(const RgbView& V, float sigma, int i, float (&row)[7]) {
  int zx, zy, oi;
  float diff;
  if (PACKED) {
    const uint32_t c = ((const uint32_t*)V.corres)[i];
    if (!(c & 0x80000000u)) return false;
    zx = (int)(c & 0x7FFu); zy = (int)((c >> 11) & 0x7FFu);
    diff = (float)((int)((c >> 22) & 0x1FFu) - 255);
    oi = i;
  } else {
    const DataTerm c = ((const DataTerm*)V.corres)[i];
    if (!c.valid) return false;
    zx = c.zero_x; zy = c.zero_y;
    diff = c.diff;
    oi = c.one_y * V.cols + c.one_x;
  }
  float w = sigma + fabsf(diff);
  w = w > 1.19209290E-07F ? 1.0f / w : 1.0f;
  if (sigma == -1) w = 1;
  row[6] = -w * diff;
  f3 p;
  const int zi = zy * V.cols + zx;
  if (V.cloud) {
    p = {V.cloud[(size_t)zi * 3], V.cloud[(size_t)zi * 3 + 1], V.cloud[(size_t)zi * 3 + 2]};
  } else {
    p = project_point(zx, zy, V.lastDepth[zi], 1.0f / V.k.fx, 1.0f / V.k.fy, V.k.cx, V.k.cy);
  }
  const float invz = (float)(1.0 / (double)p.z);
  const float dI_dx_val = w * V.sobelScale * V.dIdx[oi];
// ... 1985 lines not shown
```

include/ef_hip.h:

```cpp
#ifndef EF_HIP_H_
#define EF_HIP_H_
#include <stddef.h>
#include <stdint.h>
#ifdef __cplusplus
extern "C" {
#endif

#define EF_OK 0
#define EF_EINVAL (-1)
#define EF_EHIP (-2)
#define EF_ENOMEM (-3)
#define EF_ESTATE (-4)
#define EF_ECAPACITY (-5)

typedef struct ef_ctx ef_ctx;

typedef struct ef_config {
  int width, height;
  float fx, fy, cx, cy;
  int time_delta;
  float confidence;
  float depth_cut;
  float icp_weight;
  int fast_odom;
// ... 362 lines not shown
typedef struct ef_outlier_result {
  double sum, sum_sq;
  uint32_t participants, measured, sparse, outliers, count_after;
  float threshold;
} ef_outlier_result;
int ef_default_outlier_params(ef_ctx* ctx, ef_outlier_params* params);
int ef_map_neighbor_stats(ef_ctx* ctx, const ef_outlier_params* params, const ef_map_selection* among_or_null, float* mean_dist_or_null,
                          uint32_t* count_or_null, uint32_t max_rows);
int ef_map_neighbor_stats_dev(ef_ctx* ctx, const ef_outlier_params* params, const ef_map_selection* among_or_null, float* mean_dist_dev_or_null,
                              uint32_t* count_dev_or_null, uint32_t max_rows);
int ef_map_outliers_select(ef_ctx* ctx, const ef_outlier_params* params, const ef_map_selection* among_or_null, uint32_t* rows, uint32_t max_rows,
                           uint32_t* count, ef_outlier_result* result_or_null);
int ef_map_outliers_select_dev(ef_ctx* ctx, const ef_outlier_params* params, const ef_map_selection* among_or_null, uint32_t* rows_dev,
                               uint32_t max_rows, uint32_t* count_dev, ef_outlier_result* result_dev_or_null);
int ef_map_remove_outliers(ef_ctx* ctx, const ef_outlier_params* params, const ef_map_selection* among_or_null, ef_outlier_result* result);

#define EF_COMPONENT_NONE 0xFFFFFFFFu
#define EF_COMPONENTS_REJECTED 0
#define EF_COMPONENTS_ACCEPTED 1
typedef struct ef_component_params {
  float radius; float cell; float min_conf;
  uint32_t min_size; uint32_t max_size;
} ef_component_params;
typedef struct ef_component_result {
  uint32_t nodes, components, largest, rejected_rows, rejected_components, count_after, status;
} ef_component_result;
int ef_default_component_params(ef_ctx* ctx, ef_component_params* params);
int ef_map_components(ef_ctx* ctx, const ef_component_params* params, const ef_map_selection* among_or_null, uint32_t* label_or_null,
                      uint32_t* size_or_null, uint32_t max_rows, ef_component_result* result_or_null);
int ef_map_components_dev(ef_ctx* ctx, const ef_component_params* params, const ef_map_selection* among_or_null, uint32_t* label_dev_or_null,
                          uint32_t* size_dev_or_null, uint32_t max_rows, ef_component_result* result_dev_or_null);
int ef_map_components_select(ef_ctx* ctx, const ef_component_params* params, const ef_map_selection* among_or_null, int what, uint32_t* rows,
                             uint32_t max_rows, uint32_t* count, ef_component_result* result_or_null);
int ef_map_components_select_dev(ef_ctx* ctx, const ef_component_params* params, const ef_map_selection* among_or_null, int what,
                                 uint32_t* rows_dev, uint32_t max_rows, uint32_t* count_dev, ef_component_result* result_dev_or_null);
int ef_map_remove_components(ef_ctx* ctx, const ef_component_params* params, const ef_map_selection* among_or_null, ef_component_result* result);

enum ef_image {
  EF_IMG_DEPTH_FILTERED = 0,
  EF_IMG_DEPTH_METRIC,
  EF_IMG_DEPTH_METRIC_FILTERED,
  EF_IMG_PREDICT_IMAGE,
  EF_IMG_PREDICT_VERTEX,
  EF_IMG_PREDICT_NORMAL,
  EF_IMG_PREDICT_TIME,
  EF_IMG_FILL_IMAGE,
  EF_IMG_FILL_VERTEX,
  EF_IMG_FILL_NORMAL,
  EF_IMG_INDEX,
  EF_IMG_VERT_CONF,
  EF_IMG_COLOR_TIME,
  EF_IMG_NORM_RAD,
  EF_IMG_OLD_IMAGE,
  EF_IMG_OLD_VERTEX,
  EF_IMG_OLD_NORMAL,
  EF_IMG_OLD_TIME
};
int ef_get_image(ef_ctx* ctx, int which, void* host_dst, size_t bytes);
int ef_get_image_resized(ef_ctx* ctx, int which, int factor, void* host_dst, size_t bytes);
int ef_get_tracker_buffer(ef_ctx* ctx, int which, int level, void* host_dst, size_t bytes);
int ef_get_tracker_buffer_of(ef_ctx* ctx, int tracker, int which, int level, void* host_dst, size_t bytes);

typedef struct ef_timing { const char* name; float ms; } ef_timing;
int ef_enable_timing(ef_ctx* ctx, int on);
int ef_get_timings(ef_ctx* ctx, ef_timing* out, int max, int* n);

typedef struct ef_kernel_time {
  const char* name; float avg_us; int launches; double bytes_per_launch; double bytes_per_launch_survey;
} ef_kernel_time;
int ef_kernel_timing(ef_ctx* ctx, int every_n_frames);
int ef_get_kernel_timing(ef_ctx* ctx, ef_kernel_time* out);
int ef_get_splat_timing(ef_ctx* ctx, ef_kernel_time* out);
int ef_get_tracker_timing(ef_ctx* ctx, ef_kernel_time* out);

int ef_get_tracker_fallbacks(ef_ctx* ctx, int* count);
typedef struct ef_tracker_plan {
  int script, n_small, n_iter;
  unsigned long long levels;
  unsigned res_bytes, res_budget;
} ef_tracker_plan;
int ef_get_tracker_plan(ef_ctx* ctx, ef_tracker_plan* out);
int ef_debug_occupy(ef_ctx* ctx, int workgroups, int microseconds);
int ef_debug_query_lanes(ef_ctx* ctx, int lanes);
int ef_debug_inject_tracker_abort(ef_ctx* ctx);

int ef_debug_clocks(ef_ctx* ctx, unsigned long long* out16);
int ef_debug_small_clocks(ef_ctx* ctx, unsigned long long* out32);

int ef_dev_alloc(void** dev, size_t bytes);
int ef_dev_free(void* dev);
int ef_dev_upload(void* dev, const void* host, size_t bytes);
int ef_dev_download(void* host, const void* dev, size_t bytes);
int ef_dev_memset(void* dev, int value, size_t bytes);
int ef_dev_sync(void);
int ef_dev_calibrate(void* stream, float* empty_us, float* stream16mb_us);
int ef_device_count(int* n);
int ef_set_device(int device);

typedef struct ef_intr { float fx, fy, cx, cy; } ef_intr;

int ef_op_pyr_down(const uint16_t* src, int src_cols, int src_rows, uint16_t* dst, void* stream);
int ef_op_create_vmap(const ef_intr* intr, const uint16_t* depth, int cols, int rows, float depth_cutoff,
                      float* vmap, void* stream);
int ef_op_create_nmap(const float* vmap, int cols, int rows, float* nmap, void* stream);
int ef_op_transform_maps(const float* vmap_src, const float* nmap_src, int cols, int rows, const float* R9,
                         const float* t3, float* vmap_dst, float* nmap_dst, void* stream);
int ef_op_copy_maps(const float* vmap_src_f4, const float* nmap_src_f4, int cols, int rows, float* vmaps_tmp,
                    float* vmap_dst, float* nmap_dst, void* stream);
int ef_op_resize_vmap(const float* in, int src_cols, int src_rows, float* out, void* stream);
int ef_op_resize_nmap(const float* in, int src_cols, int src_rows, float* out, void* stream);
int ef_op_pyr_down_gauss_f(const float* src, int src_cols, int src_rows, float* dst, void* stream);
int ef_op_pyr_down_uchar_gauss(const uint8_t* src, int src_cols, int src_rows, uint8_t* dst, void* stream);
int ef_op_vertices_to_depth(const float* vmaps_tmp, int cols, int rows, float cutoff, float* dst, void* stream);
int ef_op_image_bgr_to_intensity(const uint8_t* rgba, int cols, int rows, uint8_t* dst, void* stream);
int ef_op_compute_derivative_images(const uint8_t* src, int cols, int rows, int16_t* dx, int16_t* dy, void* stream);
int ef_op_project_to_point_cloud(const float* depth, int cols, int rows, const ef_intr* intr_level0, int level,
                                 float* cloud_f3, void* stream);
int ef_op_icp_step(const float* Rcurr9, const float* tcurr3, const float* vmap_curr, const float* nmap_curr,
                   const float* Rprev_inv9, const float* tprev3, const ef_intr* intr, const float* vmap_g_prev,
                   const float* nmap_g_prev, float dist_thres, float angle_thres, int cols, int rows,
                   float* A_host36, float* b_host6, float* residual_host2, void* stream);
int ef_op_compute_rgb_residual(float min_scale, const int16_t* dIdx, const int16_t* dIdy, const float* last_depth,
                               const float* next_depth, const uint8_t* last_image, const uint8_t* next_image,
                               void* corres_img, float max_depth_delta, const float* kt3, const float* krkinv9,
                               int cols, int rows, int* sigma_sum_host, int* count_host, void* stream);
int ef_op_rgb_step(const void* corres_img, float sigma, const float* cloud_f3, float fx, float fy,
                   const int16_t* dIdx, const int16_t* dIdy, float sobel_scale, int cols, int rows,
                   float* A_host36, float* b_host6, void* stream);
int ef_op_so3_step(const uint8_t* last_image, const uint8_t* next_image, const float* image_basis9,
                   const float* kinv9, const float* krlr9, int cols, int rows, float* A_host9, float* b_host3,
                   float* residual_host2, void* stream);

typedef struct ef_model_maps_op {
  int cols, rows;
  const float *pred_vertex, *pred_normal, *fill_vertex, *fill_normal;
  const uint8_t *pred_image, *fill_image;
  float R[9], t[3];
  float max_depth_rgb;
  int camera_frame, force_fill_image, tally;
  unsigned dense_count;
  int dense_samples;
  float* vmap[3];
  float* nmap[3];
  float* depth0;
  uint8_t* last0;
  int joint;
  const uint16_t* raw;
  const uint8_t* rgb3;
  float depth_cut;
  uint16_t* filtered;
  float* metric;
  float* metric_filtered;
  uint8_t* next0;
} ef_model_maps_op;
int ef_op_model_maps(const ef_model_maps_op* args, unsigned* dense_count_left, void* stream);
int ef_op_sobel_mask(const uint8_t* const* next_image3, const float* const* next_depth3, int cols, int rows, int16_t* const* dIdx3,
                     int16_t* const* dIdy3, uint8_t* const* mask3, uint32_t* const* corres3, void* stream);

enum ef_linalg_op {
  EF_LINALG_LDLT6 = 0,
  EF_LINALG_LDLT3F,
  EF_LINALG_POLAR3,
  EF_LINALG_RODRIGUES,
  EF_LINALG_SE3_INVERSE,
  EF_LINALG_SE3_LOG_NORM,
  EF_LINALG_SCALAR,
  EF_LINALG_LDLT6_WAVE,
  EF_LINALG_LDLT6_EVERY_LANE,
  EF_LINALG_MAT_TO_QUAT,
  EF_LINALG_SE3_MUL,
  EF_LINALG_SE3_CASTF,
  EF_LINALG_SE3_INVERSE_F,
  EF_LINALG_M4_AFFINE_INVERSE,
  EF_LINALG_LDLT_PIVOTS,
  EF_LINALG_LU_INVERSE6
};
int ef_op_linalg(int which, const double* in_host, int n_in, double* out_host, int n_out);

typedef struct ef_gn_state {
  float Rcurr[9], tcurr[3];
  double resultRt[16];
  float krkinv[9], kt[3];
  float lastRGBErrorLevel;
  int rgb_broken;
} ef_gn_state;
typedef struct ef_gn_update_args {
  float sums[58];
  ef_gn_state prev;
  float Rprev[9], tprev[3];
  int count, sigma;
  int icp, rgb, rgb_only;
  float icp_weight;
  ef_intr knext;
  int level_changes;
  int split_tail;
} ef_gn_update_args;
int ef_op_gn_update(const ef_gn_update_args* in, ef_gn_state* next, double* lastA36, double* lastb6, float* stats4);
typedef struct ef_track_end_out {
  double q[4], t[3];
  double logged[16];
  float T_cw[16], pose_f[16], R_wc_f[9], t_wc_f[3];
  float weighting;
} ef_track_end_out;
int ef_op_track_end_tail(const float* Rcurr9, const float* tcurr3, const float* Rprev9, const float* tprev3, const double* q_prev4,
                         const double* t_prev3, int rgb, float weight_multiplier, ef_track_end_out* out);

typedef struct ef_cam { int cols, rows; float fx, fy, cx, cy; } ef_cam;

int ef_op_filter_depth(const uint16_t* raw, int cols, int rows, float max_d, uint16_t* filtered, void* stream);
int ef_op_metricise_depth(const uint16_t* in, int cols, int rows, float max_d, float* out, void* stream);
int ef_op_seed_map(const ef_cam* cam, const uint8_t* rgb, const float* depth_metric, const float* depth_metric_filtered,
                   int time, float max_depth, float* surfels_aos, uint32_t* count_host, void* stream);
int ef_op_predict_indices(const ef_cam* cam, const double* T_wc16, int time, const float* surfels_aos, uint32_t count,
                          float max_depth, int time_delta, uint32_t* index_map, float* vert_conf, float* color_time,
                          float* norm_rad, void* stream);
int ef_op_combined_predict(const ef_cam* cam, const double* T_wc16, const float* surfels_aos, uint32_t count,
                           float max_depth, float conf_threshold, int time, int max_time, int time_delta,
                           uint8_t* image_rgba, float* vertex, float* normal, uint16_t* time_map, void* stream);
int ef_op_synthesize_depth(const ef_cam* cam, const double* T_wc16, const float* surfels_aos, uint32_t count,
                           float max_depth, float conf_threshold, int time, int max_time, int time_delta,
                           float* depth, void* stream);
int ef_op_fill_in(const ef_cam* cam, const uint8_t* image_rgba, const float* vertex, const float* normal,
                  const uint16_t* depth_filtered, const uint8_t* rgb, int passthrough, int passthrough_image,
                  uint8_t* fill_image, float* fill_vertex, float* fill_normal, void* stream);
int ef_op_dense_enough(const ef_cam* cam, const uint8_t* image_rgba, int* dense_host, void* stream);
int ef_op_fuse(const ef_cam* cam, const double* T_wc16, int time, const uint8_t* rgb, const float* depth_metric,
               const float* depth_metric_filtered, const uint32_t* index_map, const float* vert_conf,
               const float* color_time, const float* norm_rad, float max_depth, float weighting, float* surfels_aos,
               uint32_t count, float* new_unstable_aos, uint32_t* new_count_host, void* stream);
int ef_op_clean(const ef_cam* cam, const double* T_wc16, int time, const uint32_t* index_map, const float* vert_conf,
                const float* color_time, const float* norm_rad, float conf_threshold, int time_delta, float max_depth,
                const float* surfels_aos, uint32_t count, const float* new_unstable_aos, uint32_t new_count,
                float* surfels_out_aos, uint32_t* out_count_host, void* stream);
int ef_op_clean_deform(const ef_cam* cam, const double* T_wc16, int time, const uint32_t* index_map, const float* vert_conf,
                       const float* color_time, const float* norm_rad, float conf_threshold, int time_delta, float max_depth,
                       const float* surfels_aos, uint32_t count, const float* new_unstable_aos, uint32_t new_count,
                       const float* graph, int nodes, const float* depth, int is_fern, float* surfels_out_aos,
                       uint32_t* out_count_host, void* stream);

#ifdef __cplusplus
}
#endif
#endif
```

Baseline: 2172.

## Defer fill-in maps and compute them on demand inside tracking model maps

Stops the predict pass from writing the fill-in vertex/normal/image maps when tracking will consume them next. The model-maps kernel instead reconstructs fill-in texels directly from the filtered depth and RGB. Materialisation happens lazily only when something else needs the buffers, which saves a full-frame write and read of three maps. It also reuses a stored depth from the z-buffer key rather than re-rasterising each sprite, and takes the normal from a helper. The cost is extra lazy-state bookkeeping and a possible synchronisation when the image buffers swap.

```diff
diff --git a/elasticfusion_amd/api.py b/elasticfusion_amd/api.py
--- a/elasticfusion_amd/api.py
+++ b/elasticfusion_amd/api.py
@@ -47,7 +47,8 @@
     _fields_ = [("cols", c_i), ("rows", c_i), ("pred_vertex", P), ("pred_normal", P), ("fill_vertex", P), ("fill_normal", P), ("pred_image", P),
                 ("fill_image", P), ("R", c_f * 9), ("t", c_f * 3), ("max_depth_rgb", c_f), ("camera_frame", c_i), ("force_fill_image", c_i),
                 ("tally", c_i), ("dense_count", C.c_uint), ("dense_samples", c_i), ("vmap", P * 3), ("nmap", P * 3), ("depth0", P), ("last0", P),
-                ("joint", c_i), ("raw", P), ("rgb3", P), ("depth_cut", c_f), ("filtered", P), ("metric", P), ("metric_filtered", P), ("next0", P)]
+                ("joint", c_i), ("raw", P), ("rgb3", P), ("depth_cut", c_f), ("filtered", P), ("metric", P), ("metric_filtered", P), ("next0", P),
+                ("fill_depth_filtered", P), ("fill_rgb3", P), ("fill_fx", c_f), ("fill_fy", c_f), ("fill_cx", c_f), ("fill_cy", c_f)]
 
 
 class ef_track_end_out(C.Structure):
@@ -1543,7 +1544,8 @@
 
     @staticmethod
     def model_maps(pred_vertex, pred_normal, fill_vertex, fill_normal, R, t, maxDepthRGB=6.0, pred_image=None, fill_image=None, camera_frame=False,
-                   force_fill_image=False, tally=False, dense_count=0, dense_samples=1, joint=False, raw=None, rgb=None, depth_cut=3.0, init=None):
+                   force_fill_image=False, tally=False, dense_count=0, dense_samples=1, joint=False, raw=None, rgb=None, depth_cut=3.0, init=None,
+                   fill_from=None):
         h, w, _ = pred_vertex.shape
         init = init or {}
         keep = [DevBuf.from_array(ops._f32(a)) for a in (pred_vertex, pred_normal, fill_vertex, fill_normal)]
@@ -1579,6 +1581,13 @@
             keep += fr
             a.joint, a.raw, a.rgb3, a.depth_cut = 1, fr[0].p, fr[1].p, float(depth_cut)
             a.filtered, a.metric, a.metric_filtered, a.next0 = (out[n].p for n in ("filtered", "metric", "metric_filtered", "next0"))
+        if fill_from is not None:
+            fd, frgb = np.ascontiguousarray(fill_from[0], np.uint16), np.ascontiguousarray(fill_from[1], np.uint8)
+            assert fd.shape == (h, w) and frgb.shape == (h, w, 3) and not force_fill_image
+            src = [DevBuf.from_array(fd), DevBuf.from_array(frgb)]
+            keep += src
+            a.fill_depth_filtered, a.fill_rgb3 = src[0].p, src[1].p
+            a.fill_fx, a.fill_fy, a.fill_cx, a.fill_cy = (float(v) for v in fill_from[2:6])
         left = C.c_uint(0)
         _chk(lib().ef_op_model_maps(C.byref(a), C.byref(left), None))
         res = {name: out[name].to_array(*spec[name]) for name in spec}
diff --git a/elasticfusion_amd/csrc/ef_context.hip b/elasticfusion_amd/csrc/ef_context.hip
--- a/elasticfusion_amd/csrc/ef_context.hip
+++ b/elasticfusion_amd/csrc/ef_context.hip
@@ -113,6 +113,9 @@
   efm::IndexMaps im{};
   efm::PredictMaps pm{};
   efm::FillMaps fm{};
+  bool fm_pending = false;
+  const uint16_t* fm_depth = nullptr;
+  const uint8_t* fm_rgb = nullptr;
   unsigned long long* zbuf = nullptr;
   unsigned long long* zbuf_assoc = nullptr;
   unsigned long long* zbuf_clean = nullptr;
diff --git a/elasticfusion_amd/csrc/ef_device.hpp b/elasticfusion_amd/csrc/ef_device.hpp
--- a/elasticfusion_amd/csrc/ef_device.hpp
+++ b/elasticfusion_amd/csrc/ef_device.hpp
@@ -83,6 +83,38 @@
 
 __device__ __forceinline__ int clampi(int v, int lo, int hi) { return v < lo ? lo : (v > hi ? hi : v); }
 
+struct FillSource {
+  const uint16_t* depth_filtered;
+  const uint8_t* rgb3;
+  int cols, rows;
+  float cx, cy, inv_fx, inv_fy;
+};
+__device__ __forceinline__ f3 fill_vertex_at(const FillSource& F, int sx, int sy, int x, int y) {
+  const float z = (float)F.depth_filtered[clampi(sy, 0, F.rows - 1) * F.cols + clampi(sx, 0, F.cols - 1)] / 1000.0f;
+  return {((float)x - F.cx) * z * F.inv_fx, ((float)y - F.cy) * z * F.inv_fy, z};
+}
+__device__ __forceinline__ float4 fill_texel_vertex(const FillSource& F, int x, int y, float4 sv, bool passthrough) {
+  if (!(sv.z == 0 || passthrough)) return sv;
+  const f3 v = fill_vertex_at(F, x, y, x, y);
+  float4 o; o.x = v.x; o.y = v.y; o.z = v.z; o.w = 1.f;
+  return o;
+}
+__device__ __forceinline__ float4 fill_texel_normal(const FillSource& F, int x, int y, float4 sn, bool passthrough) {
+  if (!(sn.z == 0 || passthrough)) return sn;
+  const f3 v = fill_vertex_at(F, x, y, x, y);
+  const f3 vx = fill_vertex_at(F, x + 1, y, x + 1, y);
+  const f3 vy = fill_vertex_at(F, x, y + 1, x, y + 1);
+  const f3 nn = normalized(cross(vx - v, vy - v));
+  float4 o; o.x = nn.x; o.y = nn.y; o.z = nn.z; o.w = 1.f;
+  return o;
+}
+__device__ __forceinline__ uchar4 fill_texel_image(const FillSource& F, int x, int y, uchar4 si, bool passthroughImage) {
+  if (!((si.x == 0 && si.y == 0 && si.z == 0) || passthroughImage)) return si;
+  const size_t pi = (size_t)(y * F.cols + x);
+  uchar4 o; o.x = F.rgb3[pi * 3]; o.y = F.rgb3[pi * 3 + 1]; o.z = F.rgb3[pi * 3 + 2]; o.w = 255;
+  return o;
+}
+
 struct DataTerm {
   short zero_x, zero_y;
   short one_x, one_y;
diff --git a/elasticfusion_amd/csrc/ef_host_frame.inc b/elasticfusion_amd/csrc/ef_host_frame.inc
--- a/elasticfusion_amd/csrc/ef_host_frame.inc
+++ b/elasticfusion_amd/csrc/ef_host_frame.inc
@@ -1,7 +1,17 @@
 namespace {
-int do_predict(ef_ctx* c, bool count_dense = true) {
+void fm_materialise(ef_ctx* c) {
+  if (!c->fm_pending) return;
+  efm::fill_in(c->cam, c->pm, c->fm_depth, c->fm_rgb, false, c->cfg.frame_to_frame_rgb != 0, c->fm, c->stream);
+  c->fm_pending = false;
+}
+int do_predict(ef_ctx* c, bool count_dense = true, bool tracked = false) {
+  const bool defer = tracked && count_dense && !c->cfg.close_loops && !c->timing && !c->lost && !c->cfg.frame_to_frame_rgb;
+  c->fm_pending = defer;
+  c->fm_depth = c->img.depth_filtered;
+  c->fm_rgb = c->img.rgb;
   efm::combined_predict(c->cam, c->st->T_cw, c->maps[c->cur], &c->st->map_counts[c->cur], c->maxDepthProcessed, c->cfg.confidence,
-                        c->last_frame_recovery ? 0 : c->tick, c->tick, c->cfg.time_delta, c->zbuf, c->pm, c->fm, c->img.depth_filtered, c->img.rgb,
+                        c->last_frame_recovery ? 0 : c->tick, c->tick, c->cfg.time_delta, c->zbuf, c->pm, defer ? efm::FillMaps{nullptr, nullptr, nullptr} : c->fm,
+                        c->img.depth_filtered, c->img.rgb,
                         c->cfg.frame_to_frame_rgb != 0, (count_dense && !c->tally_by_consumer) ? &c->st->dense_count : nullptr, c->stream, nullptr, 0u,
                         (count_dense && c->mark_value) ? c->d_consumed : nullptr, c->mark_value, c->rays);
   if (count_dense) c->mark_value = 0;
@@ -39,6 +49,10 @@
   const int W = c->cam.cols, H = c->cam.rows;
   hipStream_t sb = f.sb;
   if (f.overlap && !c->events_live) EF_HIP(c, hipStreamSynchronize(c->stream));
+  if (c->fm_pending && c->img_alt.depth_filtered == c->fm_depth) {
+    fm_materialise(c);
+    if (f.overlap) EF_HIP(c, hipStreamSynchronize(c->stream));
+  }
   std::swap(c->img, c->img_alt);
   c->frame_parity ^= 1;
   if (f.overlap) EF_HIP(c, hipStreamWaitEvent(sb, f.overlap_mode == 2 ? c->ev_frame_done[c->frame_parity] : c->ev_track_done, 0));
@@ -113,9 +127,11 @@
   tp.icpWeight = c->cfg.icp_weight;
   const bool rgb = tp.rgbOnly || tp.icpWeight < 100;
   timer_begin(c, "odomInit");
+  const eft::FillOnDemand on_demand{c->fm_depth, c->fm_rgb, c->cam.fx, c->cam.fy, c->cam.cx, c->cam.cy};
   eft::init_icp_model(c->pyr, (const float*)c->pm.vertex, (const float*)c->pm.normal, (const float*)c->fm.vertex,
                       (const float*)c->fm.normal, c->st, 6.0f , s, (const uint8_t*)c->pm.image,
-                      (const uint8_t*)c->fm.image, c->cfg.frame_to_frame_rgb != 0, f.joint_inputs ? &fp : nullptr, c->tally_pending);
+                      (const uint8_t*)c->fm.image, c->cfg.frame_to_frame_rgb != 0, f.joint_inputs ? &fp : nullptr, c->tally_pending,
+                      c->fm_pending ? &on_demand : nullptr);
   c->tally_pending = false;
   if (f.overlap) {
     eft::build_pyramids_model_side(c->pyr, s);
@@ -216,7 +232,7 @@
 }
 int end_of_frame(ef_ctx* c, const FramePlan& f) {
   timer_begin(c, "IndexMap::ACTIVE");
-  do_predict(c);
+  do_predict(c, true, f.track_this);
   timer_end(c, "IndexMap::ACTIVE");
   if (c->closure) {
     timer_begin(c, "ferns");
diff --git a/elasticfusion_amd/csrc/ef_host_inspect.inc b/elasticfusion_amd/csrc/ef_host_inspect.inc
--- a/elasticfusion_amd/csrc/ef_host_inspect.inc
+++ b/elasticfusion_amd/csrc/ef_host_inspect.inc
@@ -265,6 +265,7 @@
   DeviceGuard dg_(c);
   const size_t P = (size_t)c->cam.cols * c->cam.rows;
   if (which >= EF_IMG_INDEX && which <= EF_IMG_NORM_RAD) im_materialise(c);
+  if (which >= EF_IMG_FILL_IMAGE && which <= EF_IMG_FILL_NORMAL) fm_materialise(c);
   const ImageRef im = image_ref(c, which);
   if (!im.elem) { c->err = "ef_get_image: unknown image"; return EF_EINVAL; }
   const void* src = im.src;
diff --git a/elasticfusion_amd/csrc/ef_host_ops.inc b/elasticfusion_amd/csrc/ef_host_ops.inc
--- a/elasticfusion_amd/csrc/ef_host_ops.inc
+++ b/elasticfusion_amd/csrc/ef_host_ops.inc
@@ -199,6 +199,9 @@
   o.dense_count = a->dense_count; o.dense_samples = a->dense_samples;
   for (int i = 0; i < eft::NUM_PYRS; ++i) { o.vmap[i] = a->vmap[i]; o.nmap[i] = a->nmap[i]; }
   o.depth0 = a->depth0; o.last0 = a->last0;
+  if (a->fill_depth_filtered && (!a->fill_rgb3 || a->force_fill_image)) return EF_EINVAL;
+  eft::FillOnDemand od{a->fill_depth_filtered, a->fill_rgb3, a->fill_fx, a->fill_fy, a->fill_cx, a->fill_cy};
+  if (a->fill_depth_filtered) o.on_demand = &od;
   eft::FramePreprocess fp{};
   if (a->joint) {
     fp = eft::FramePreprocess{a->raw, a->depth_cut, efm::bilateral_table(), a->filtered, a->metric, a->metric_filtered, a->rgb3, nullptr};
diff --git a/elasticfusion_amd/csrc/ef_map_kernels.hip b/elasticfusion_amd/csrc/ef_map_kernels.hip
--- a/elasticfusion_amd/csrc/ef_map_kernels.hip
+++ b/elasticfusion_amd/csrc/ef_map_kernels.hip
@@ -448,36 +448,17 @@
   }
 }
 
-__device__ __forceinline__ f3 fill_vertex_at(const uint16_t* __restrict__ d, const Cam& cam, int sx, int sy, int x, int y, float inv_fx,
-                                             float inv_fy) {
-  const float z = (float)d[clampi(sy, 0, cam.rows - 1) * cam.cols + clampi(sx, 0, cam.cols - 1)] / 1000.0f;
-  return {((float)x - cam.cx) * z * inv_fx, ((float)y - cam.cy) * z * inv_fy, z};
+__device__ __forceinline__ FillSource fill_source(const Cam& cam, const uint16_t* __restrict__ depth_filtered, const uint8_t* __restrict__ rgb3) {
+  return FillSource{depth_filtered, rgb3, cam.cols, cam.rows, cam.cx, cam.cy, 1.0f / cam.fx, 1.0f / cam.fy};
 }
 __device__ __forceinline__ void fill_in_px(const Cam& cam, int x, int y, uchar4 si, float4 sv, float4 sn,
                                            const uint16_t* __restrict__ depth_filtered, const uint8_t* __restrict__ rgb3, bool passthrough,
                                            bool passthroughImage, FillMaps out) {
   const int pi = y * cam.cols + x;
-  const float inv_fx = 1.0f / cam.fx, inv_fy = 1.0f / cam.fy;
-  if (sv.z == 0 || passthrough) {
-    const f3 v = fill_vertex_at(depth_filtered, cam, x, y, x, y, inv_fx, inv_fy);
-    out.vertex[pi] = make_float4(v.x, v.y, v.z, 1.f);
-  } else {
-    out.vertex[pi] = sv;
-  }
-  if (sn.z == 0 || passthrough) {
-    const f3 v = fill_vertex_at(depth_filtered, cam, x, y, x, y, inv_fx, inv_fy);
-    const f3 vx = fill_vertex_at(depth_filtered, cam, x + 1, y, x + 1, y, inv_fx, inv_fy);
-    const f3 vy = fill_vertex_at(depth_filtered, cam, x, y + 1, x, y + 1, inv_fx, inv_fy);
-    const f3 nn = normalized(cross(vx - v, vy - v));
-    out.normal[pi] = make_float4(nn.x, nn.y, nn.z, 1.f);
-  } else {
-    out.normal[pi] = sn;
-  }
-  if ((si.x == 0 && si.y == 0 && si.z == 0) || passthroughImage) {
-    out.image[pi] = make_uchar4(rgb3[(size_t)pi * 3], rgb3[(size_t)pi * 3 + 1], rgb3[(size_t)pi * 3 + 2], 255);
-  } else {
-    out.image[pi] = si;
-  }
+  const FillSource F = fill_source(cam, depth_filtered, rgb3);
+  out.vertex[pi] = fill_texel_vertex(F, x, y, sv, passthrough);
+  out.normal[pi] = fill_texel_normal(F, x, y, sn, passthrough);
+  out.image[pi] = fill_texel_image(F, x, y, si, passthroughImage);
 }
 __device__ __forceinline__ void dense_sample(const Cam& cam, int x, int y, uchar4 si, unsigned* counter) {
   if (counter && x % 20 == 10 && y % 20 == 10 && x / 20 < cam.cols / 20 && y / 20 < cam.rows / 20)
@@ -505,24 +486,24 @@
     const uint32_t id = (uint32_t)key;
     const rt34 T = rt34_load16(T16);
     const float4 pc = map.pos_conf[id], ct = map.col_time[id], nr = map.nrm_rad[id];
-    const Sprite S = make_sprite(cam, T, pc, ct, nr, maxDepth, confThreshold, (float)time, (float)maxTime, (float)timeDelta);
-    float z = 0.f;
-    sprite_fragment(cam, S, px, py, z);
+    float z = depth_of_key((uint32_t)(key >> 32));
+    if (z == 0.f) {
+      const Sprite S = make_sprite(cam, T, pc, ct, nr, maxDepth, confThreshold, (float)time, (float)maxTime, (float)timeDelta);
+      sprite_fragment(cam, S, px, py, z);
+    }
     const f3 col = decodeColor(ct.x);
     im = make_uchar4((uint8_t)roundf(col.x * 255.0f), (uint8_t)roundf(col.y * 255.0f), (uint8_t)roundf(col.z * 255.0f), 255);
     const float fcx = (float)px + 0.5f, fcy = (float)py + 0.5f;
     vt = make_float4((fcx - cam.cx) * z * (1.f / cam.fx), (fcy - cam.cy) * z * (1.f / cam.fy), z, pc.w);
-    nm = make_float4(S.n.x, S.n.y, S.n.z, nr.w);
+    nm = index_texel_norm_rad(T, nr);
     tm = (uint16_t)(unsigned)ct.z;
   }
   out.image[pi] = im;
   out.vertex[pi] = vt;
   out.normal[pi] = nm;
   out.time[pi] = tm;
-  if (FUSE_FILL) {
-    fill_in_px(cam, px, py, im, vt, nm, depth_filtered, rgb3, false, passthroughImage, fill);
-    dense_sample(cam, px, py, im, dense_counter);
-  }
+  if (FUSE_FILL) fill_in_px(cam, px, py, im, vt, nm, depth_filtered, rgb3, false, passthroughImage, fill);
+  dense_sample(cam, px, py, im, dense_counter);
 }
 __global__ void __launch_bounds__(BLK) k_depth_resolve(const Cam cam, const float* __restrict__ T16, SurfelSoA map, float maxDepth,
                                                         float confThreshold, int time, int maxTime, int timeDelta, unsigned long long* zbuf,
diff --git a/elasticfusion_amd/csrc/ef_track.hpp b/elasticfusion_amd/csrc/ef_track.hpp
--- a/elasticfusion_amd/csrc/ef_track.hpp
+++ b/elasticfusion_amd/csrc/ef_track.hpp
@@ -177,10 +177,16 @@
   const uint8_t* rgb3;
   uint8_t* rgb_keep;
 };
+struct FillOnDemand {
+  const uint16_t* depth_filtered;
+  const uint8_t* rgb3;
+  float fx, fy, cx, cy;
+};
 void init_icp_model(const Pyramid& p, const float* pred_vertex, const float* pred_normal, const float* fill_vertex,
                     const float* fill_normal, const TrackState* st, float maxDepthRGB, hipStream_t s, const uint8_t* pred_image_rgba = nullptr,
                     const uint8_t* fill_image_rgba = nullptr, bool frameToFrameRGB = false, const FramePreprocess* with = nullptr,
-                    bool tally = false );
+                    bool tally = false ,
+                    const FillOnDemand* on_demand = nullptr);
 void init_icp_maps(const Pyramid& p, const float* vertex4, const float* normal4, const uint8_t* image_rgba, const TrackState* st,
                    float maxDepthRGB, hipStream_t s);
 void build_pyramids(const Pyramid& p, const uint16_t* depth_filtered, Intr k, float cutoff, hipStream_t s, bool with_sobel);
@@ -204,6 +210,7 @@
   uint8_t* last0;
   const FramePreprocess* with;
   uint8_t* next0;
+  const FillOnDemand* on_demand;
 };
 int model_maps_op(const ModelMapsOp& o, unsigned* dense_count_left, hipStream_t s);
 struct SobelMaskOp {
diff --git a/elasticfusion_amd/csrc/ef_track_host_inputs.inc b/elasticfusion_amd/csrc/ef_track_host_inputs.inc
--- a/elasticfusion_amd/csrc/ef_track_host_inputs.inc
+++ b/elasticfusion_amd/csrc/ef_track_host_inputs.inc
@@ -63,8 +63,10 @@
 }
 ModelMapsArgs model_maps_choice_args(const Pyramid& p, bool model_side, const float* pred_vertex, const float* pred_normal, const float* fill_vertex,
                                      const float* fill_normal, const TrackState* st, float maxDepthRGB, const uint8_t* pred_image_rgba,
-                                     const uint8_t* fill_image_rgba, bool frameToFrameRGB, bool tally) {
+                                     const uint8_t* fill_image_rgba, bool frameToFrameRGB, bool tally, const FillOnDemand* on_demand = nullptr) {
   ModelMapsArgs A = model_maps_args(p, model_side, pred_vertex, pred_normal, maxDepthRGB);
+  if (on_demand)
+    A.on_demand = FillSource{on_demand->depth_filtered, on_demand->rgb3, p.W(0), p.H(0), on_demand->cx, on_demand->cy, 1.0f / on_demand->fx, 1.0f / on_demand->fy};
   A.fill_vertex = (const float4*)fill_vertex; A.fill_normal = (const float4*)fill_normal;
   A.pred_image = pred_image_rgba; A.fill_image = fill_image_rgba; A.force_fill_image = frameToFrameRGB;
   A.tally_image = (tally && pred_image_rgba) ? pred_image_rgba : nullptr;
@@ -91,9 +93,9 @@
 
 void init_icp_model(const Pyramid& p, const float* pred_vertex, const float* pred_normal, const float* fill_vertex,
                     const float* fill_normal, const TrackState* st, float maxDepthRGB, hipStream_t s, const uint8_t* pred_image_rgba,
-                    const uint8_t* fill_image_rgba, bool frameToFrameRGB, const FramePreprocess* with, bool tally) {
+                    const uint8_t* fill_image_rgba, bool frameToFrameRGB, const FramePreprocess* with, bool tally, const FillOnDemand* on_demand) {
   launch_model_maps(p, model_maps_choice_args(p, true, pred_vertex, pred_normal, fill_vertex, fill_normal, st, maxDepthRGB, pred_image_rgba,
-                                               fill_image_rgba, frameToFrameRGB, tally), st, with, s);
+                                               fill_image_rgba, frameToFrameRGB, tally, on_demand), st, with, s);
 }
 int model_maps_op(const ModelMapsOp& o, unsigned* dense_count_left, hipStream_t s) {
   Pyramid p{};
@@ -115,7 +117,7 @@
   if (e == hipSuccess) e = hipMemcpy(st, h, sizeof(TrackState), hipMemcpyHostToDevice);
   if (e == hipSuccess) {
     launch_model_maps(p, model_maps_choice_args(p, !o.camera_frame, o.pred_vertex, o.pred_normal, o.fill_vertex, o.fill_normal, st, o.maxDepthRGB,
-                                                 o.pred_image, o.fill_image, o.force_fill_image, o.tally), st, o.with, s);
+                                                 o.pred_image, o.fill_image, o.force_fill_image, o.tally, o.on_demand), st, o.with, s);
     e = hipGetLastError();
   }
   if (e == hipSuccess) e = hipStreamSynchronize(s);
diff --git a/elasticfusion_amd/csrc/ef_track_kernels.hip b/elasticfusion_amd/csrc/ef_track_kernels.hip
--- a/elasticfusion_amd/csrc/ef_track_kernels.hip
+++ b/elasticfusion_amd/csrc/ef_track_kernels.hip
@@ -462,6 +462,7 @@
   uint8_t* last0;
   const uint8_t* tally_image;
   unsigned* tally_out;
+  FillSource on_demand;
 };
 __device__ __forceinline__ bool model_maps_use_fill(const ModelMapsArgs& A, const TrackState* __restrict__ st, bool first_wg) {
   if (!A.tally_image) return use_fill_in(st);
@@ -508,8 +509,9 @@
   if (gx >= cols || by * 4 >= rows) return;
   const int j = gx & 3, bx = gx >> 2;
   const bool even = (j & 1) == 0, leftpair = j < 2;
-  const float4* __restrict__ vsrc = fill ? A.fill_vertex : A.pred_vertex;
-  const float4* __restrict__ nsrc = fill ? A.fill_normal : A.pred_normal;
+  const bool on_demand = fill && A.on_demand.depth_filtered != nullptr;
+  const float4* __restrict__ vsrc = (fill && !on_demand) ? A.fill_vertex : A.pred_vertex;
+  const float4* __restrict__ nsrc = (fill && !on_demand) ? A.fill_normal : A.pred_normal;
   const m33 R = m33_load(st->R_wc_f);
   const f3 t{st->t_wc_f[0], st->t_wc_f[1], st->t_wc_f[2]};
   const bool cf = A.camera_frame;
@@ -520,11 +522,22 @@
     vs[r] = vsrc[(by * 4 + r) * cols + gx];
     ns[r] = nsrc[(by * 4 + r) * cols + gx];
   }
+  if (on_demand) {
+#pragma unroll
+    for (int r = 0; r < 4; ++r) {
+      vs[r] = fill_texel_vertex(A.on_demand, gx, by * 4 + r, vs[r], false);
+      ns[r] = fill_texel_normal(A.on_demand, gx, by * 4 + r, ns[r], false);
+    }
+  }
   if (A.last0) {
-    const uchar4* __restrict__ isrc = (const uchar4*)((A.force_fill_image || fill) ? A.fill_image : A.pred_image);
+    const uchar4* __restrict__ isrc = (const uchar4*)(((A.force_fill_image || fill) && !on_demand) ? A.fill_image : A.pred_image);
     uchar4 cs[4];
 #pragma unroll
     for (int r = 0; r < 4; ++r) cs[r] = isrc[(by * 4 + r) * cols + gx];
+    if (on_demand) {
+#pragma unroll
+      for (int r = 0; r < 4; ++r) cs[r] = fill_texel_image(A.on_demand, gx, by * 4 + r, cs[r], false);
+    }
 #pragma unroll
     for (int r = 0; r < 4; ++r) A.last0[(by * 4 + r) * cols + gx] = intensity_of((float)cs[r].x, (float)cs[r].y, (float)cs[r].z);
   }
diff --git a/include/ef_hip.h b/include/ef_hip.h
--- a/include/ef_hip.h
+++ b/include/ef_hip.h
@@ -538,6 +538,9 @@
   float* metric;
   float* metric_filtered;
   uint8_t* next0;
+  const uint16_t* fill_depth_filtered;
+  const uint8_t* fill_rgb3;
+  float fill_fx, fill_fy, fill_cx, fill_cy;
 } ef_model_maps_op;
 int ef_op_model_maps(const ef_model_maps_op* args, unsigned* dense_count_left, void* stream);
 int ef_op_sobel_mask(const uint8_t* const* next_image3, const float* const* next_depth3, int cols, int rows, int16_t* const* dIdx3,
```

Result: no change. 2185 (median of 6 runs) (+0.6%).
